# hila-chefer/Transformer-Explainability

Hardware: AMD Instinct MI355X
Metric: relevance maps/sec (ViT-B/16 224^2, batch 64 per GPU, generate_LRP transformer_attribution) (higher is better)
Workload: dtype f32 (3xbf16 split operands, 6 products, fp32 accumulate)

## Files before the change

include/te_relprop.h:

```cpp
#ifndef TE_RELPROP_H
#define TE_RELPROP_H

#include <stddef.h>
#include <stdint.h>

#ifdef __cplusplus
extern "C" {
#endif

typedef void* te_stream_t;
typedef uint16_t te_bf16_t;

enum {
  TE_OK = 0,
  TE_ERR_INVALID_ARG = -1,
  TE_ERR_WORKSPACE = -2,
  TE_ERR_UNSUPPORTED = -3,
  TE_ERR_NO_DEVICE = -4
};

enum { TE_VARIANT_OURS = 0, TE_VARIANT_LRP = 1, TE_IMPL_SIMPLE = 0x100 };

enum { TE_ROLLOUT_NORMALISE = 1, TE_ROLLOUT_CLS_FIXUP = 2, TE_ROLLOUT_ROW0 = 4 };

int te_version(void);
const char* te_status_string(int status);
int te_device_check(void);
const char* te_build_id(void);

size_t te_linear_relprop_workspace_bytes(int64_t T, int64_t in_f, int64_t out_f, int variant);
int te_linear_relprop_f32(const float* R, const float* X, const float* W, float* out,
                          int64_t T, int64_t in_f, int64_t out_f, float alpha, int variant,
                          void* ws, size_t ws_bytes, te_stream_t stream);

int te_linear_zpass_f32(const float* R, const float* X, const float* W, float* S,
                        int64_t T, int64_t in_f, int64_t out_f, te_stream_t stream);
int te_linear_cpass_f32(const float* S, const float* X, const float* W, float* out,
                        int64_t T, int64_t in_f, int64_t out_f, te_stream_t stream);

int te_linear_zpass_fwd_f32(const float* R, const float* r_scale, int64_t r_scale_stride,
                            int64_t rows_per_sample, const float* X, const float* W, const float* Y,
                            const float* bias, float* S, int64_t T, int64_t in_f, int64_t out_f,
                            te_stream_t stream);
int te_linear_relprop_fwd_f32(const float* R, const float* r_scale, int64_t r_scale_stride,
                              int64_t rows_per_sample, const float* X, const float* W, const float* Y,
                              const float* bias, float* out, int64_t T, int64_t in_f, int64_t out_f,
                              void* ws, size_t ws_bytes, te_stream_t stream);

size_t te_matmul_relprop_av_workspace_bytes(int64_t B, int64_t H, int64_t N, int64_t D);
int te_matmul_relprop_av_f32(const float* R, int64_t r_sb, int64_t r_sh, int64_t r_sn,
                             const float* attn,
                             const float* v, int64_t v_sb, int64_t v_sh, int64_t v_sn,
                             const float* Z, int64_t z_sb, int64_t z_sh, int64_t z_sn,
                             float* cam_attn,
                             float* cam_v, int64_t cv_sb, int64_t cv_sh, int64_t cv_sn,
                             int64_t B, int64_t H, int64_t N, int64_t D, float out_scale, int variant,
                             void* ws, size_t ws_bytes, te_stream_t stream);
size_t te_matmul_relprop_qk_workspace_bytes(int64_t B, int64_t H, int64_t N, int64_t D);
int te_matmul_relprop_qk_f32(const float* R_nn, const float* r_scale, int64_t r_scale_stride,
                             const float* q, int64_t q_sb, int64_t q_sh, int64_t q_sn,
                             const float* k, int64_t k_sb, int64_t k_sh, int64_t k_sn,
                             const float* Z,
                             float* cam_q, int64_t cq_sb, int64_t cq_sh, int64_t cq_sn,
                             float* cam_k, int64_t ck_sb, int64_t ck_sh, int64_t ck_sn,
                             int64_t B, int64_t H, int64_t N, int64_t D, float out_scale, int variant,
                             void* ws, size_t ws_bytes, te_stream_t stream);

size_t te_add_relprop_workspace_bytes(int64_t B, int64_t n);
int te_add_relprop_f32(const float* R, const float* X0, const float* X1, float* out0, float* out1,
                       int64_t B, int64_t n, int64_t x1_batch_stride, int variant,
                       void* ws, size_t ws_bytes, te_stream_t stream);

size_t te_add_relprop_deferred_workspace_bytes(int64_t B, int64_t n);
int te_add_relprop_deferred_f32(const float* R, const float* X0, const float* X1, float* a, float* b, float* fac,
                                int64_t B, int64_t n, int64_t x1_batch_stride,
                                void* ws, size_t ws_bytes, te_stream_t stream);

size_t te_add_bcast_relprop_workspace_bytes(int64_t B, int64_t H, int64_t N);
int te_add_bcast_relprop_f32(const float* R, const float* X0, const float* mask, float* out0,
                             float* out1, int64_t B, int64_t H, int64_t N, int variant,
                             void* ws, size_t ws_bytes, te_stream_t stream);

int te_add_bcast_relprop_deferred_f32(const float* R, const float* X0, const float* mask, float* a, float* out1,
                                      float* fac, int64_t B, int64_t H, int64_t N,
                                      void* ws, size_t ws_bytes, te_stream_t stream);

int te_clone_relprop_f32(const float* R0, const float* R1, const float* R2, const float* X,
                         float* out, int64_t n, te_stream_t stream);

int te_clone_relprop_scaled_f32(const float* R0, const float* s0, int64_t s0_stride,
                                const float* R1, const float* s1, int64_t s1_stride,
                                const float* R2, const float* s2, int64_t s2_stride,
                                const float* X, float* out, int64_t B, int64_t n, te_stream_t stream);

int te_index_select_relprop_f32(const float* R, const float* X, float* out,
                                int64_t B, int64_t N, int64_t C, int64_t index, te_stream_t stream);

int te_gradcam_headmean_f32(const float* grad, const float* cam, float* out,
                            int64_t B, int64_t H, int64_t N, te_stream_t stream);

size_t te_rollout_workspace_bytes(int64_t L, int64_t B, int64_t N);
size_t te_rollout_row0_workspace_bytes(int64_t B, int64_t N);
int te_rollout_f32(const float* cams, int64_t L, int64_t start_layer, int64_t B, int64_t N,
                   int flags, float* joint, void* ws, size_t ws_bytes, te_stream_t stream);

#define TE_X6_TILE_AUTO 0
#define TE_X6_TILE_128 1
#define TE_X6_TILE_256 2
#define TE_X6_TILE_128x128 3
#define TE_X6_TEST_DROP_HANDOVER 0x200
#define TE_X6_WHOLE_TILES 0x10000
#define TE_X6_TEST_SMALL_GRID 0x4000
#define TE_X6_X_PLANES_SIGNED 0x20000
#define TE_X6_TILE_Z_SHIFT 10
#define TE_X6_TILE_C_SHIFT 12
#define TE_X6_PHASE_SPLIT 4
#define TE_X6_PHASE_Z 8
#define TE_X6_PHASE_C 16
#define TE_X6_PHASE_MASK 28
int te_linear_relprop_x6_supported(int64_t T, int64_t in_f, int64_t out_f);
size_t te_linear_relprop_x6_workspace_bytes(int64_t T, int64_t in_f, int64_t out_f);
size_t te_linear_x6_weight_planes_bytes(int64_t in_f, int64_t out_f);
size_t te_linear_x6_planes_bytes(int64_t rows, int64_t K);
int te_linear_x6_prepare_weights_f32(const float* W, int64_t in_f, int64_t out_f, void* planes, size_t planes_bytes,
                                     te_stream_t stream);
int te_linear_x6_split_abs_f32(const float* X, int64_t rows, int64_t K, void* planes, size_t planes_bytes,
                               te_stream_t stream);
int te_linear_relprop_x6_f32(const float* R, const float* r_scale, int64_t r_scale_stride, int64_t rows_per_sample,
                             const float* X, const float* W, const void* w_planes, const void* x_planes,
                             const float* Y, const float* bias, float* out,
                             int64_t T, int64_t in_f, int64_t out_f, int flags, unsigned* status, void* ws,
                             size_t ws_bytes, te_stream_t stream);
int te_linear_relprop_x6_check(const void* ws, int64_t T, int64_t in_f, int64_t out_f, te_stream_t stream);

int te_linear_relprop_x6_general_supported(int64_t T, int64_t in_f, int64_t out_f, int variant);
size_t te_linear_x6_weight_planes_lrp_bytes(int64_t in_f, int64_t out_f);
int te_linear_x6_prepare_weights_lrp_f32(const float* W, int64_t in_f, int64_t out_f, void* planes, size_t planes_bytes,
                                         te_stream_t stream);
size_t te_linear_relprop_x6_general_workspace_bytes(int64_t T, int64_t in_f, int64_t out_f, int variant);
int te_linear_relprop_x6_general_f32(const float* R, const float* r_scale, int64_t r_scale_stride, int64_t rows_per_sample,
                                     const float* X, const float* W, const void* w_planes, const void* w_planes_lrp,
                                     const void* x_abs_planes, const float* Y, const float* bias, float* out,
                                     int64_t T, int64_t in_f, int64_t out_f, float alpha, int variant, int flags,
                                     unsigned* status, void* ws, size_t ws_bytes, te_stream_t stream);

int te_gemm_x6_supported(int64_t T, int64_t K, int64_t M);
size_t te_gemm_x6_workspace_bytes(int64_t T, int64_t K, int64_t M);
int te_linear_x6_split_matrix_f32(const float* A, int64_t rows, int64_t K, int transposed, void* planes,
                                  size_t planes_bytes, te_stream_t stream);
int te_gemm_x6_f32(const float* X, const void* x_planes, const void* w_planes, const float* bias, float* out,
                   int64_t T, int64_t K, int64_t M, int flags, unsigned* status, void* ws, size_t ws_bytes,
                   te_stream_t stream);
int te_linear_x6_split_dual_f32(const float* A, int64_t rows, int64_t K, void* planes, void* planes_abs,
                                size_t planes_bytes, te_stream_t stream);
int te_gelu_backward_x6_planes_f32(const float* dy, const float* x, int64_t rows, int64_t K, void* planes,
                                   size_t planes_bytes, te_stream_t stream);
int te_gelu_forward_x6_planes_f32(const float* x, float* y, int64_t rows, int64_t K, void* planes, void* planes_abs,
                                  size_t planes_bytes, te_stream_t stream);

int te_attention_forward_supported(int64_t N, int64_t D);
int te_attention_forward_f32(const float* qkv, float* z_qk, float* attn, float* out, void* out_planes,
                             void* out_abs_planes, size_t planes_bytes, int64_t B, int64_t H, int64_t N, int64_t D,
                             float scale, te_stream_t stream);
int te_attention_backward_f32(const float* d_out, const float* out, const float* qkv, const float* attn, float* d_attn,
                              float* d_qkv, int64_t B, int64_t H, int64_t N, int64_t D, float scale, int need_qk,
                              te_stream_t stream);

int te_attention_strided_supported(int64_t N, int64_t D);
size_t te_attention_backward_strided_workspace_bytes(int64_t B, int64_t H, int64_t N);
int te_attention_forward_strided_f32(const float* q, int64_t q_sb, int64_t q_sh, int64_t q_sn,
                                     const float* k, int64_t k_sb, int64_t k_sh, int64_t k_sn,
                                     const float* v, int64_t v_sb, int64_t v_sh, int64_t v_sn,
                                     const float* mask, float* z_qk, float* x_scaled, float* attn,
                                     float* out, int64_t o_sb, int64_t o_sh, int64_t o_sn,
                                     int64_t B, int64_t H, int64_t N, int64_t D, float scale, te_stream_t stream);
int te_attention_backward_strided_f32(const float* d_out, int64_t do_sb, int64_t do_sh, int64_t do_sn,
                                      const float* out, int64_t o_sb, int64_t o_sh, int64_t o_sn,
                                      const float* q, int64_t q_sb, int64_t q_sh, int64_t q_sn,
                                      const float* k, int64_t k_sb, int64_t k_sh, int64_t k_sn,
                                      const float* v, int64_t v_sb, int64_t v_sh, int64_t v_sn,
                                      const float* attn, float* d_attn,
                                      float* d_q, int64_t dq_sb, int64_t dq_sh, int64_t dq_sn,
                                      float* d_k, int64_t dk_sb, int64_t dk_sh, int64_t dk_sn,
                                      float* d_v, int64_t dv_sb, int64_t dv_sh, int64_t dv_sn,
                                      int64_t B, int64_t H, int64_t N, int64_t D, float scale, int need_qk,
                                      void* ws, size_t ws_bytes, te_stream_t stream);

int te_layernorm_supported(int64_t C);
int te_layernorm_forward_f32(const float* x, const float* weight, const float* bias, float* y, float* mean, float* rstd,
                             int64_t T, int64_t C, float eps, te_stream_t stream);
int te_layernorm_backward_f32(const float* dy, const float* x, const float* weight, const float* mean, const float* rstd,
                              const float* add, float* dx, int64_t T, int64_t C, te_stream_t stream);
int te_gelu_forward_f32(const float* x, float* y, int64_t n, te_stream_t stream);
int te_gelu_backward_f32(const float* dy, const float* x, float* dx, int64_t n, te_stream_t stream);

int te_heatmap_f32(const float* maps, float* heat, float* fg_mask, int64_t B, int64_t g, int64_t scale,
                   int normalise, te_stream_t stream);

size_t te_seg_metrics_workspace_bytes(int64_t B, int64_t H, int64_t W);
int te_seg_metrics_f32(const float* heat, const float* fg_mask, const int64_t* labels, int64_t* counts, double* ap,
                       double* f1, int64_t B, int64_t H, int64_t W, void* ws, size_t ws_bytes, te_stream_t stream);

#define TE_MAPSIM_SSIM 1
size_t te_map_similarity_workspace_bytes(int64_t B, int64_t n);
int te_map_similarity_f32(const float* a, const float* b, int64_t* rank_sums, double* sim, int64_t B, int64_t n, int64_t H,
                          int64_t W, int flags, double data_range, void* ws, size_t ws_bytes, te_stream_t stream);

#define TE_RATIONALE_MAX_KS 16
#define TE_RATIONALE_CLAMP 1
size_t te_rationale_metrics_workspace_bytes(int64_t B, int64_t N, int64_t Wmax);
int te_rationale_metrics_f32(const float* scores, const int32_t* word_ids, const uint8_t* truth, float* word_scores,
                             int32_t* n_words, int32_t* order, int32_t* counts, double* soft, int64_t B, int64_t N,
                             int64_t Wmax, const int64_t* ks, int64_t n_ks, int flags, void* ws, size_t ws_bytes,
                             te_stream_t stream);

#define TE_TOKEN_ERASE_MAX_FRACTIONS 8
int te_token_erase(const int64_t* input_ids, const int64_t* attention_mask, const int32_t* word_ids,
                   const int32_t* order, const int32_t* n_words, int64_t* ids_out, int64_t* mask_out,
                   int32_t* n_rationale, int64_t B, int64_t N, int64_t Wmax, const double* fractions, int64_t n_t,
                   int64_t pad_id, te_stream_t stream);

size_t te_conv2d_zb_relprop_workspace_bytes(int64_t B, int64_t C, int64_t H, int64_t W, int64_t E, int64_t p);
int te_conv2d_zb_relprop_f32(const float* R, int64_t r_bs, const float* X, const float* W, const float* Y,
                             const float* bias, float* out, int64_t B, int64_t C, int64_t H, int64_t W_, int64_t E,
                             int64_t p, int flags, void* ws, size_t ws_bytes, te_stream_t stream);

#define TE_PERTURB_MAX_STEPS 16
#define TE_PERTURB_MAX_CHANNELS 4
size_t te_perturb_workspace_bytes(int64_t B, int64_t n_steps);
int te_perturb_f32(const float* vis, const float* data, float* out, int64_t B, int64_t C, int64_t HW,
                   const int64_t* ks, int64_t n_steps, const float* mean, const float* std_, void* ws,
                   size_t ws_bytes, te_stream_t stream);

#define TE_BLUR_MAX_TAPS 63
int te_blur_normalised_f32(const float* data, float* out, int64_t B, int64_t C, int64_t H, int64_t W, const float* taps,
                           int64_t klen, const float* mean, const float* std_, te_stream_t stream);
size_t te_pixel_rank_workspace_bytes(int64_t B, int64_t n);
int te_pixel_rank_f32(const float* vis, int32_t* rank, int64_t B, int64_t n, void* ws, size_t ws_bytes, te_stream_t stream);
int te_curve_inputs_f32(const float* data, const float* substrate, const float* fill, const int32_t* rank, float* out,
                        int64_t B, int64_t C, int64_t HW, int64_t step, int64_t s0, int64_t n_s, int insertion,
                        const float* mean, const float* std_, te_stream_t stream);
int te_curve_inputs_bf16(const float* data, const float* substrate, const float* fill, const int32_t* rank, te_bf16_t* out,
                         int64_t B, int64_t C, int64_t HW, int64_t step, int64_t s0, int64_t n_s, int insertion,
                         const float* mean, const float* std_, te_stream_t stream);
int te_curve_scores_f32(const float* logits, const int64_t* target, double* prob, int64_t B, int64_t K, int64_t s0,
                        int64_t n_s, te_stream_t stream);
int te_curve_scores_bf16(const te_bf16_t* logits, const int64_t* target, double* prob, int64_t B, int64_t K, int64_t s0,
                         int64_t n_s, te_stream_t stream);
int te_curve_auc_f64(const double* prob, double* auc, int64_t S1, int64_t B, te_stream_t stream);

size_t te_localisation_workspace_bytes(int64_t P, int64_t H, int64_t W);
int te_localisation_f32(const float* heat, const int64_t* labels, const int64_t* image_index, const int64_t* target_id,
                        const int64_t* boxes, int64_t M, int64_t* stats, double* energy, int64_t P, int64_t B, int64_t H,
                        int64_t W, void* ws, size_t ws_bytes, te_stream_t stream);

int te_noise_inputs_f32(const float* x, float* out, int64_t B, int64_t n, int64_t d0, int64_t n_d, float radius, int64_t seed,
                        int64_t id0, te_stream_t stream);
int te_noise_inputs_bf16(const float* x, te_bf16_t* out, int64_t B, int64_t n, int64_t d0, int64_t n_d, float radius,
                         int64_t seed, int64_t id0, te_stream_t stream);
int te_map_distance_f32(const float* a, const float* b, double* sums, int64_t B, int64_t D, int64_t n, te_stream_t stream);
int te_map_distance_bf16(const float* a, const te_bf16_t* b, double* sums, int64_t B, int64_t D, int64_t n,
                         te_stream_t stream);
size_t te_map_complexity_workspace_bytes(int64_t B, int64_t n);
int te_map_complexity_f32(const float* maps, double* out, int64_t* counts, int64_t B, int64_t n, double eps, void* ws,
                          size_t ws_bytes, te_stream_t stream);

#define TE_SUBSET_MAX_CELLS 4096
int te_subset_inputs_f32(const float* x, const float* substrate, const float* fill, const float* attr, float* out,
                         uint8_t* member, double* attr_sum, int64_t B, int64_t C, int64_t g_h, int64_t g_w, int64_t p,
                         int64_t k, int64_t d0, int64_t n_d, int64_t seed, int64_t id0, te_stream_t stream);
int te_subset_inputs_bf16(const float* x, const float* substrate, const float* fill, const float* attr, te_bf16_t* out,
                          uint8_t* member, double* attr_sum, int64_t B, int64_t C, int64_t g_h, int64_t g_w, int64_t p,
                          int64_t k, int64_t d0, int64_t n_d, int64_t seed, int64_t id0, te_stream_t stream);
int te_perturbation_dot_f32(const float* x, const float* y, const float* w, double* sums, int64_t B, int64_t D, int64_t n,
                            int64_t m, te_stream_t stream);
int te_perturbation_dot_bf16(const float* x, const te_bf16_t* y, const float* w, double* sums, int64_t B, int64_t D, int64_t n,
                             int64_t m, te_stream_t stream);

int te_linear_relprop_bf16_supported(int64_t T, int64_t in_f, int64_t out_f);
size_t te_linear_relprop_bf16_workspace_bytes(int64_t T, int64_t in_f, int64_t out_f);
size_t te_linear_bf16_weight_planes_bytes(int64_t in_f, int64_t out_f);
int te_linear_bf16_prepare_weights(const te_bf16_t* W, int64_t in_f, int64_t out_f, void* planes, size_t planes_bytes,
                                   te_stream_t stream);
int te_linear_relprop_bf16(const float* R, int64_t r_ld, const float* r_scale, int64_t r_scale_stride,
                           int64_t rows_per_scale, const te_bf16_t* X, int64_t x_ld, const void* w_planes, float* out,
                           int64_t T, int64_t in_f, int64_t out_f, void* ws, size_t ws_bytes, te_stream_t stream);
int te_matmul_relprop_bf16_supported(int64_t N, int64_t D);
size_t te_matmul_relprop_av_bf16_workspace_bytes(int64_t B, int64_t H, int64_t N, int64_t D);
size_t te_matmul_relprop_qk_bf16_workspace_bytes(int64_t B, int64_t H, int64_t N, int64_t D);
int te_matmul_relprop_av_bf16(const float* R, int64_t r_sb, int64_t r_sh, int64_t r_sn,
                              const te_bf16_t* attn,
                              const te_bf16_t* v, int64_t v_sb, int64_t v_sh, int64_t v_sn,
                              const te_bf16_t* Z, int64_t z_sb, int64_t z_sh, int64_t z_sn,
                              float* cam_attn,
                              float* cam_v, int64_t cv_sb, int64_t cv_sh, int64_t cv_sn,
                              int64_t B, int64_t H, int64_t N, int64_t D, float out_scale, int variant,
                              void* ws, size_t ws_bytes, te_stream_t stream);
int te_matmul_relprop_qk_bf16(const float* R_nn, const float* r_scale, int64_t r_scale_stride,
                              const te_bf16_t* q, int64_t q_sb, int64_t q_sh, int64_t q_sn,
                              const te_bf16_t* k, int64_t k_sb, int64_t k_sh, int64_t k_sn,
                              const te_bf16_t* Z,
                              float* cam_q, int64_t cq_sb, int64_t cq_sh, int64_t cq_sn,
                              float* cam_k, int64_t ck_sb, int64_t ck_sh, int64_t ck_sn,
                              int64_t B, int64_t H, int64_t N, int64_t D, float out_scale, int variant,
                              void* ws, size_t ws_bytes, te_stream_t stream);
// ... 120 lines not shown
```

transformer-explainability_amd/bert.py:

```python
from __future__ import annotations

import math
from types import SimpleNamespace

import torch
import torch.nn as nn

from . import ops
from . import rules as R_ours

__all__ = ["BertConfigLite", "make_bert_module", "BertModel", "BertForSequenceClassification"]


def BertConfigLite(**kw):
    d = dict(vocab_size=30522, hidden_size=768, num_hidden_layers=12, num_attention_heads=12,
             intermediate_size=3072, hidden_act="gelu", hidden_dropout_prob=0.1,
             attention_probs_dropout_prob=0.1, max_position_embeddings=512, type_vocab_size=2,
             layer_norm_eps=1e-12, pad_token_id=0, num_labels=2)
    d.update(kw)
    return SimpleNamespace(**d)


class _FusedSelfAttention(torch.autograd.Function):

# ... 113 lines not shown
            if attention_mask is not None:
                scores = self.add([scores, attention_mask])
            probs = self.softmax(scores)
            self.save_attn(probs)
            if probs.requires_grad:
                probs.register_hook(self.save_attn_gradients)
            probs = self.dropout(probs)
            if head_mask is not None:
                probs = self.mul([probs, head_mask])
            ctx = self.matmul2([probs, v])
            ctx = ctx.permute(0, 2, 1, 3).contiguous()
            return (ctx.view(*ctx.shape[:-2], self.all_head_size),)

        def _forward_fused(self, h1, h2, h3, attention_mask):
            B, N, C = h1.shape
            H, D = self.num_attention_heads, self.attention_head_size
            ql, kl, vl = self.query(h1), self.key(h2), self.value(h3)
            ctx, probs, zqk, xsc = _FusedSelfAttention.apply(ql, kl, vl, attention_mask, H, 1.0 / math.sqrt(D), self)
            self._fused_anchor = ql if ql.requires_grad else None
            heads = lambda t: t.detach().view(B, N, H, D).permute(0, 2, 1, 3)
            q, k, v = heads(ql), heads(kl), heads(vl)
            self.save_attn(probs)
            caches = [(self.matmul1, [q, k.transpose(-1, -2)], zqk), (self.matmul2, [probs, v], heads(ctx))]
            if attention_mask is not None:
                caches.append((self.add, [xsc, attention_mask], None))
            for mod, X, Y in caches:
                mod.X, mod.Y = X, Y
                mod._y_version = Y._version if Y is not None else None
                mod._w_version = (None, None)
            return (ctx,)

        def relprop(self, cam, **kwargs):
            B, N, C = cam.shape
            H, D = self.num_attention_heads, self.attention_head_size
            var = self.matmul2.variant
            probs, v = self.matmul2.X
            q, kt = self.matmul1.X
            rq = torch.empty((B, N, C), dtype=cam.dtype, device=cam.device)
            rk, rv = torch.empty_like(rq), torch.empty_like(rq)
            as_heads = lambda t: t.view(B, N, H, D).permute(0, 2, 1, 3)
            if self.save_head_relevance:
                self.head_relevance = ops.head_relevance(as_heads(cam))
            cam1, _ = ops.matmul_relprop_av(as_heads(cam), probs, v, out_scale=0.5, cam_v_out=as_heads(rv), variant=var,
                                            z=R_ours._cached_y(self.matmul2))
            if self.head_mask is not None:
                cam1, _ = self.mul.relprop(cam1, **kwargs)
            self.save_attn_cam(cam1)
            if getattr(self, "_stop_after_attn_cam", False):
                raise L.StopRelprop()
            if self.attention_mask is not None:
                cam1, _ = self.add.relprop(cam1, deferred=True, **kwargs)
            ops.matmul_relprop_qk(cam1, q, kt.transpose(-1, -2), out_scale=0.5, cam_q_out=as_heads(rq),
                                  cam_k_out=as_heads(rk), variant=var, z=R_ours._cached_y(self.matmul1))
            rq = self.query.relprop(rq, **kwargs)
            rk = self.key.relprop(rk, **kwargs)
            rv = self.value.relprop(rv, **kwargs)
            return self.clone.relprop((rq, rk, rv), **kwargs)

        def attnlrp(self, G_o, eps):
            if self.head_mask is not None:
                raise ops._lib.TeError("BertSelfAttention.attnlrp: head_mask is not implemented for AttnLRP")
            q, k, v = self.query.Y.detach(), self.key.Y.detach(), self.value.Y.detach()
            d_q, d_k, d_v = torch.empty_like(q), torch.empty_like(k), torch.empty_like(v)
            R_ours.attention_attnlrp(G_o, q, k, v, self.get_attn().detach(), self.num_attention_heads,
                                     1.0 / math.sqrt(self.attention_head_size), d_q, d_k, d_v)
            ops.alrp_scale3(d_q, d_k, d_v)
            return self.clone.attnlrp((self.query.attnlrp(d_q, eps), self.key.attnlrp(d_k, eps),
                                       self.value.attnlrp(d_v, eps)), eps)

    class BertSelfOutput(nn.Module):
        def __init__(self, config):
            super().__init__()
            self.dense = L.Linear(config.hidden_size, config.hidden_size)
            self.LayerNorm = L.LayerNorm(config.hidden_size, eps=config.layer_norm_eps)
            self.dropout = L.Dropout(config.hidden_dropout_prob)
            self.add = L.Add()

        def forward(self, hidden_states, input_tensor):
            return self.LayerNorm(self.add([self.dropout(self.dense(hidden_states)), input_tensor]))

        def relprop(self, cam, **kwargs):
            cam1, cam2 = self.add.relprop(cam, deferred=True, **kwargs)
            return self.dense.relprop(cam1, **kwargs), cam2

        def attnlrp(self, G, eps):
            Gd = self.add.attnlrp(self.LayerNorm.attnlrp(G, eps), eps)
            return self.dense.attnlrp(Gd, eps), Gd

    class BertAttention(nn.Module):
        def __init__(self, config):
            super().__init__()
            self.self = BertSelfAttention(config)
            self.output = BertSelfOutput(config)
            self.clone = L.Clone()

        def forward(self, hidden_states, attention_mask=None, head_mask=None, **unused):
            h1, h2 = self.clone(hidden_states, 2)
            return (self.output(self.self(h1, attention_mask, head_mask)[0], h2),)

        def relprop(self, cam, **kwargs):
            cam1, cam2 = self.output.relprop(cam, **kwargs)
            cam1 = self.self.relprop(cam1, **kwargs)
            return self.clone.relprop((cam1, cam2), **kwargs)

        def attnlrp(self, G, eps):
            G1, G2 = self.output.attnlrp(G, eps)
            return self.clone.attnlrp((self.self.attnlrp(G1, eps), G2), eps)

    class BertIntermediate(nn.Module):
        def __init__(self, config):
            super().__init__()
            self.dense = L.Linear(config.hidden_size, config.intermediate_size)
            act = config.hidden_act
            self.intermediate_act_fn = ACT[act]() if isinstance(act, str) else act

        def forward(self, hidden_states):
            return self.intermediate_act_fn(self.dense(hidden_states))

        def relprop(self, cam, **kwargs):
            return self.dense.relprop(cam, **kwargs)

        def attnlrp(self, G, eps):
            return self.dense.attnlrp(self.intermediate_act_fn.attnlrp(G, eps), eps)

    class BertOutput(nn.Module):
        def __init__(self, config):
            super().__init__()
            self.dense = L.Linear(config.intermediate_size, config.hidden_size)
            self.LayerNorm = L.LayerNorm(config.hidden_size, eps=config.layer_norm_eps)
            self.dropout = L.Dropout(config.hidden_dropout_prob)
            self.add = L.Add()

        def forward(self, hidden_states, input_tensor):
            return self.LayerNorm(self.add([self.dropout(self.dense(hidden_states)), input_tensor]))

        def relprop(self, cam, **kwargs):
            cam1, cam2 = self.add.relprop(cam, deferred=True, **kwargs)
            return self.dense.relprop(cam1, **kwargs), cam2

        def attnlrp(self, G, eps):
            Gd = self.add.attnlrp(self.LayerNorm.attnlrp(G, eps), eps)
            return self.dense.attnlrp(Gd, eps), Gd

    class BertLayer(nn.Module):
        def __init__(self, config):
            super().__init__()
            self.attention = BertAttention(config)
            self.intermediate = BertIntermediate(config)
            self.output = BertOutput(config)
            self.clone = L.Clone()
            act = self.intermediate.intermediate_act_fn
            if hasattr(act, "feeds"):
                act.feeds(self.output.dense)

        def forward(self, hidden_states, attention_mask=None, head_mask=None, **unused):
            att = self.attention(hidden_states, attention_mask, head_mask)[0]
            a1, a2 = self.clone(att, 2)
            return (self.output(self.intermediate(a1), a2),)

        def relprop(self, cam, **kwargs):
            cam1, cam2 = self.output.relprop(cam, **kwargs)
            cam1 = self.intermediate.relprop(cam1, **kwargs)
            cam = self.clone.relprop((cam1, cam2), **kwargs)
            return self.attention.relprop(cam, **kwargs)

        def attnlrp(self, G, eps):
            G1, G2 = self.output.attnlrp(G, eps)
            G = self.clone.attnlrp((self.intermediate.attnlrp(G1, eps), G2), eps)
            return self.attention.attnlrp(G, eps)

        def relprop_cls_only(self, cam_cls, **kwargs):
            alpha = kwargs.get("alpha", 1)
            var = self.clone.variant
            cls = lambda t: t[:, :1]
            dfr = ops.USE_DEFERRED_ADD
            c1, c2 = ops.add_relprop(cam_cls, cls(self.output.add.X[0]), cls(self.output.add.X[1]), variant=var,
                                     deferred=dfr)
            c1 = R_ours.linear_rule(self.output.dense, c1, alpha, cls, var)
            c1 = R_ours.linear_rule(self.intermediate.dense, c1, alpha, cls, var)
            cam = ops.clone_relprop((c1, c2), cls(self.clone.X))
            att = self.attention
            a1, a2 = ops.add_relprop(cam, cls(att.output.add.X[0]), cls(att.output.add.X[1]), variant=var, deferred=dfr)
            a1 = R_ours.linear_rule(att.output.dense, a1, alpha, cls, var)
            B, N, C = att.clone.X.shape
            dense = torch.zeros((2, B, N, C), dtype=a1.dtype, device=a1.device)
            dense[0, :, 0] = a1[:, 0]
            if isinstance(a2, ops.Deferred):
                a2 = a2.materialise()
            dense[1, :, 0] = a2[:, 0]
            cam1 = att.self.relprop(dense[0], **kwargs)
            return att.clone.relprop((cam1, dense[1]), **kwargs)

    class BertEncoder(nn.Module):
        def __init__(self, config):
            super().__init__()
            self.config = config
            self.layer = nn.ModuleList([BertLayer(config) for _ in range(config.num_hidden_layers)])

        def forward(self, hidden_states, attention_mask=None, head_mask=None, **unused):
            for i, layer in enumerate(self.layer):
                hidden_states = layer(hidden_states, attention_mask, None if head_mask is None else head_mask[i])[0]
            return (hidden_states,)

        def relprop(self, cam, **kwargs):
            for layer in reversed(self.layer):
                cam = layer.relprop(cam, **kwargs)
            return cam

        def attnlrp(self, G, eps):
            for layer in reversed(self.layer):
                G = layer.attnlrp(G, eps)
            return G

    class BertPooler(nn.Module):
        def __init__(self, config):
            super().__init__()
            self.dense = L.Linear(config.hidden_size, config.hidden_size)
            self.activation = L.Tanh()
            self.pool = L.IndexSelect()
            self.register_buffer("_cls_index", torch.zeros((), dtype=torch.long), persistent=False)

        def forward(self, hidden_states):
            first = self.pool(hidden_states, 1, self._cls_index).squeeze(1)
            return self.activation(self.dense(first))

        def relprop(self, cam, **kwargs):
            cam = self.dense.relprop(cam, **kwargs)
            return self.pool.relprop(cam.unsqueeze(1), **kwargs)

        def attnlrp(self, G, eps):
            G = self.dense.attnlrp(self.activation.attnlrp(G, eps), eps)
            return self.pool.attnlrp(G, eps)

    class BertModel(nn.Module):
        def __init__(self, config):
            super().__init__()
            self.config = config
            self.embeddings = BertEmbeddings(config)
            self.encoder = BertEncoder(config)
            self.pooler = BertPooler(config)

        def get_input_embeddings(self):
            return self.embeddings.word_embeddings

        def get_head_mask(self, head_mask, num_hidden_layers, is_attention_chunked=False, batch_size=None):
            par = next(self.parameters())
            return R_ours.expand_head_mask(head_mask, num_hidden_layers, self.config.num_attention_heads, par.dtype,
                                           batch_size, par.device)

        def forward(self, input_ids=None, attention_mask=None, token_type_ids=None, position_ids=None,
                    head_mask=None, inputs_embeds=None, **unused):
            shape = input_ids.size() if input_ids is not None else inputs_embeds.size()[:-1]
            device = input_ids.device if input_ids is not None else inputs_embeds.device
            head_mask = self.get_head_mask(head_mask, self.config.num_hidden_layers, batch_size=shape[0])
            if attention_mask is None:
                attention_mask = torch.ones(shape, device=device)
            ext = (1.0 - attention_mask[:, None, None, :].to(next(self.parameters()).dtype)) * -10000.0
            with (ops.stock_forward() if torch.is_tensor(head_mask) else ops._NULL):
                emb = self.embeddings(input_ids=input_ids, position_ids=position_ids, token_type_ids=token_type_ids,
                                      inputs_embeds=inputs_embeds)
                seq = self.encoder(emb, attention_mask=ext, head_mask=head_mask)[0]
                return (seq, self.pooler(seq))

        exploit_cls_sparsity = True

        def relprop(self, cam, **kwargs):
            if not self.exploit_cls_sparsity:
                return self.encoder.relprop(self.pooler.relprop(cam, **kwargs), **kwargs)
            cam = self.pooler.dense.relprop(cam, **kwargs)
            cam = ops.index_select_relprop(cam.unsqueeze(1), self.pooler.pool.X[:, :1], 0)
            layers = list(self.encoder.layer)
            cam = layers[-1].relprop_cls_only(cam, **kwargs)
            for layer in reversed(layers[:-1]):
                cam = layer.relprop(cam, **kwargs)
            return cam

        def attnlrp(self, G, eps):
            G = self.encoder.attnlrp(self.pooler.attnlrp(G, eps), eps)
            norm = self.embeddings.LayerNorm
            return ops.alrp_token_relevance(norm.X, norm.attnlrp(G, eps), skip_first=False)

    class BertForSequenceClassification(nn.Module):
        def __init__(self, config):
            super().__init__()
            self.config = config
            self.num_labels = config.num_labels
            self.bert = BertModel(config)
            self.dropout = L.Dropout(config.hidden_dropout_prob)
            self.classifier = L.Linear(config.hidden_size, config.num_labels)
            self.apply(self._init_weights)

        def _init_weights(self, m):
            if isinstance(m, (nn.Linear, nn.Embedding)):
                m.weight.data.normal_(mean=0.0, std=getattr(self.config, "initializer_range", 0.02))
            elif isinstance(m, nn.LayerNorm):
                m.bias.data.zero_()
                m.weight.data.fill_(1.0)
            if isinstance(m, nn.Linear) and m.bias is not None:
                m.bias.data.zero_()

        def forward(self, input_ids=None, attention_mask=None, token_type_ids=None, position_ids=None,
                    head_mask=None, inputs_embeds=None, labels=None, **unused):
            pooled = self.bert(input_ids, attention_mask=attention_mask, token_type_ids=token_type_ids,
                               position_ids=position_ids, head_mask=head_mask, inputs_embeds=inputs_embeds)[1]
            logits = self.classifier(self.dropout(pooled))
            if labels is not None:
# ... 24 lines not shown
```

transformer-explainability_amd/csrc/te_api.hip:

```cpp
#include "te_common.h"

#include <string.h>

extern "C" int te_version(void) { return 800;  }

#ifndef TE_BUILD_ID
#define TE_BUILD_ID "unstamped"
#endif
extern "C" const char* te_build_id(void) { return TE_BUILD_ID; }

extern "C" const char* te_status_string(int status) {
  switch (status) {
    case TE_OK: return "ok";
    case TE_ERR_INVALID_ARG: return "invalid argument";
    case TE_ERR_WORKSPACE: return "workspace missing, misaligned or too small";
    case TE_ERR_UNSUPPORTED: return "shape not supported by the gfx950 kernels";
    case TE_ERR_NO_DEVICE: return "no gfx950 device visible";
    default: break;
  }
  if (status > 0) return hipGetErrorString((hipError_t)status);
  return "unknown status";
}

extern "C" int te_device_check(void) {
  int n = 0;
  if (hipGetDeviceCount(&n) != hipSuccess || n <= 0) return TE_ERR_NO_DEVICE;
  for (int d = 0; d < n; ++d) {
    hipDeviceProp_t p;
    if (hipGetDeviceProperties(&p, d) != hipSuccess) continue;
    if (strncmp(p.gcnArchName, "gfx950", 6) == 0) return TE_OK;
  }
  return TE_ERR_NO_DEVICE;
}
```

transformer-explainability_amd/csrc/te_linear_x6.hip:

```cpp
#include <algorithm>
#include <cmath>
#include <type_traits>

#include "te_x6.h"

namespace {

constexpr int kRB = 3 * kFrag;
constexpr int kMinFrag = 4;
constexpr int kSpinMillis = 250;
constexpr int kErrWord = 1023;


enum { MODE_Z = 0, MODE_C = 1, MODE_G = 2, MODE_ZI = 3, MODE_Z1 = 4, MODE_CI = 5, MODE_X = 6, MODE_ZS = 7 };

__device__ __forceinline__ float bf16_f32(unsigned b) { return __uint_as_float(b << 16); }

enum { OP_ABS = 0, OP_POS = 1, OP_NEG = 2, OP_ID = 3 };
template <int OP>
__device__ __forceinline__ float apply_op(float x) {
  if constexpr (OP == OP_ID) return x;
  if constexpr (OP == OP_ABS) return __int_as_float(__float_as_int(x) & 0x7fffffff);
  const int b = __float_as_int(x);
  if constexpr (OP == OP_POS) return __int_as_float(b > 0 ? b : 0);
  return __int_as_float(b < 0 ? b : 0);
}

template <int OP, bool TRANSPOSE>
__global__ __launch_bounds__(256) void split_kernel(const float* __restrict__ src, unsigned char* __restrict__ dst,
                                                    int64_t R, int64_t K, int group, int sign,
                                                    unsigned char* __restrict__ dst_abs = nullptr) {
  const int r = threadIdx.x & 31, sl = threadIdx.x >> 5;
  const int64_t rb = blockIdx.x;
  const int64_t ks = (int64_t)blockIdx.y * 8 + sl;
  const int64_t nks = K >> 4;
  if (ks >= nks) return;
  const int64_t row = rb * 32 + r;
  float v[16];
  if (row < R) {
    if constexpr (!TRANSPOSE) {
      const float* s = src + row * K + ks * 16;
#pragma unroll
      for (int c = 0; c < 4; ++c) {
        const f32x4 q = *reinterpret_cast<const f32x4*>(s + 4 * c);
#pragma unroll
        for (int e = 0; e < 4; ++e) v[4 * c + e] = q[e];
      }
    } else {
#pragma unroll
      for (int e = 0; e < 16; ++e) v[e] = src[(ks * 16 + e) * R + row];
    }
  } else {
#pragma unroll
    for (int e = 0; e < 16; ++e) v[e] = 0.0f;
  }
  unsigned p[8][3];
#pragma unroll
  for (int e = 0; e < 8; ++e) split3_pk(apply_op<OP>(v[2 * e]), apply_op<OP>(v[2 * e + 1]), p[e]);
  unsigned char* d = dst + ((rb * nks + ks) * group + sign * 3) * kFrag + r * 16;
#pragma unroll
  for (int q = 0; q < 3; ++q)
#pragma unroll
    for (int kh = 0; kh < 2; ++kh) {
      u32x4 w;
#pragma unroll
      for (int e = 0; e < 4; ++e) w[e] = p[4 * kh + e][q];
      *reinterpret_cast<u32x4*>(d + q * kFrag + kh * 512) = w;
    }
  if constexpr (OP == OP_ID) {
    if (dst_abs) {
#pragma unroll
      for (int e = 0; e < 8; ++e) {
        const unsigned m = p[e][0] & 0x80008000u;
        p[e][0] &= 0x7fff7fffu;
        p[e][1] ^= m & (((p[e][1] & 0x7fff7fffu) + 0x7fff7fffu) & 0x80008000u);
        p[e][2] ^= m & (((p[e][2] & 0x7fff7fffu) + 0x7fff7fffu) & 0x80008000u);
      }
      unsigned char* da = dst_abs + ((rb * nks + ks) * 3) * kFrag + r * 16;
#pragma unroll
      for (int q = 0; q < 3; ++q)
#pragma unroll
        for (int kh = 0; kh < 2; ++kh) {
          u32x4 w;
#pragma unroll
          for (int e = 0; e < 4; ++e) w[e] = p[4 * kh + e][q];
          *reinterpret_cast<u32x4*>(da + q * kFrag + kh * 512) = w;
        }
    }
  }
}

enum { SRC_GELU_BWD = 0, SRC_GELU_FWD = 1 };
constexpr int kGsPitch = 132;
template <int SRC>
__global__ __launch_bounds__(256) void gelu_split_lds_kernel(const float* __restrict__ g, const float* __restrict__ x,
                                                             float* __restrict__ y, unsigned char* __restrict__ dst,
                                                             unsigned char* __restrict__ dst_abs, int64_t R, int64_t K) {
  __shared__ __attribute__((aligned(16))) float tile[32 * kGsPitch];
  const int64_t rb = blockIdx.x;
  const int64_t k0 = (int64_t)blockIdx.y * 128;
#pragma unroll
  for (int j = 0; j < 4; ++j) {
    const int i = threadIdx.x + 256 * j;
    const int tr = i >> 5, c4 = i & 31;
    const int64_t row = rb * 32 + tr, col = k0 + 4 * c4;
    f32x4 o = {0.0f, 0.0f, 0.0f, 0.0f};
    if (row < R && col < K) {
      const int64_t at = row * K + col;
      const f32x4 xv = __builtin_nontemporal_load(reinterpret_cast<const f32x4*>(x + at));
      if constexpr (SRC == SRC_GELU_BWD) {
        const f32x4 gv = __builtin_nontemporal_load(reinterpret_cast<const f32x4*>(g + at));
#pragma unroll
        for (int e = 0; e < 4; ++e) o[e] = te_gelu_grad(gv[e], xv[e]);
      } else {
#pragma unroll
        for (int e = 0; e < 4; ++e) o[e] = te_gelu(xv[e]);
        *reinterpret_cast<f32x4*>(y + at) = o;
      }
    }
    *reinterpret_cast<f32x4*>(&tile[tr * kGsPitch + 4 * c4]) = o;
  }
  __syncthreads();
  const int r = threadIdx.x & 31, sl = threadIdx.x >> 5;
  const int64_t ks = (int64_t)blockIdx.y * 8 + sl;
  const int64_t nks = K >> 4;
  if (ks >= nks) return;
  float v[16];
#pragma unroll
  for (int c = 0; c < 4; ++c) {
    const f32x4 q = *reinterpret_cast<const f32x4*>(&tile[r * kGsPitch + sl * 16 + 4 * c]);
#pragma unroll
    for (int e = 0; e < 4; ++e) v[4 * c + e] = q[e];
  }
  unsigned p[8][3];
#pragma unroll
  for (int e = 0; e < 8; ++e) split3_pk(v[2 * e], v[2 * e + 1], p[e]);
  auto store = [&](unsigned char* d) __attribute__((always_inline)) {
#pragma unroll
    for (int q = 0; q < 3; ++q)
#pragma unroll
      for (int kh = 0; kh < 2; ++kh) {
        u32x4 w;
#pragma unroll
        for (int e = 0; e < 4; ++e) w[e] = p[4 * kh + e][q];
        *reinterpret_cast<u32x4*>(d + q * kFrag + kh * 512) = w;
      }
  };
  store(dst + ((rb * nks + ks) * 3) * kFrag + r * 16);
  if (SRC == SRC_GELU_FWD && dst_abs) {
#pragma unroll
    for (int e = 0; e < 8; ++e) {
      const unsigned m = p[e][0] & 0x80008000u;
      p[e][0] &= 0x7fff7fffu;
      p[e][1] ^= m & (((p[e][1] & 0x7fff7fffu) + 0x7fff7fffu) & 0x80008000u);
      p[e][2] ^= m & (((p[e][2] & 0x7fff7fffu) + 0x7fff7fffu) & 0x80008000u);
    }
    store(dst_abs + ((rb * nks + ks) * 3) * kFrag + r * 16);
  }
}

__global__ __launch_bounds__(256) void zero_words_kernel(u32x4* __restrict__ p) {
  p[(size_t)blockIdx.x * 256 + threadIdx.x] = u32x4{0u, 0u, 0u, 0u};
}

__device__ __forceinline__ float exact_z(const float* __restrict__ x, const float* __restrict__ w, int64_t K) {
  float z1 = 0.0f, z2 = 0.0f;
  for (int64_t k = 0; k < K; ++k) {
    const float xv = x[k], wv = w[k];
    z1 = fmaf(fmaxf(xv, 0.0f), fmaxf(wv, 0.0f), z1);
    z2 = fmaf(fminf(xv, 0.0f), fminf(wv, 0.0f), z2);
  }
  return z1 + z2;
}

__device__ __forceinline__ float exact_zi(const float* __restrict__ x, const float* __restrict__ w, int64_t K) {
  float z1 = 0.0f, z2 = 0.0f;
  for (int64_t k = 0; k < K; ++k) {
    const float xv = x[k], wv = w[k];
    z1 = fmaf(fmaxf(xv, 0.0f), fminf(wv, 0.0f), z1);
    z2 = fmaf(fminf(xv, 0.0f), fmaxf(wv, 0.0f), z2);
  }
  return z1 + z2;
}

struct X6Params {
  const unsigned char* A;
  const unsigned char* B;
  int64_t a_group_stride;
  int64_t b_rb_stride;
  int nks;
  unsigned char pad0_[20];
  int ntm, ntn;
  int rows_w;
  int t_fast;
  int whole_tiles;
  int pad1_;
  int ncb;
  int64_t T;
  int in_f, out_f;
  float* partial;
  unsigned* flags;
  unsigned* status;
  long long spin_ticks;
  int drop_handover;
  int small_grid;
  int prefer_whole;
  const float* R;
  const float* Y;
  const float* bias;
  const float* X;
  const float* W;
  unsigned char* S;
  const float* rs;
  int64_t rs_stride;
  int rps;
  float* out;
  float scale;
  int accum;
  int x_sign;
};

#if defined(__HIP_DEVICE_COMPILE__)
#define X6_PASS4(a, b, c, d) asm volatile("" : "+v"(a), "+v"(b), "+v"(c), "+v"(d))
#else
#define X6_PASS4(a, b, c, d) (void)0
#endif

__device__ __forceinline__ void glds16(const unsigned char* src, unsigned char* lds_wave_base) {
  __builtin_amdgcn_global_load_lds((const __attribute__((address_space(1))) void*)src,
                                   (__attribute__((address_space(3))) void*)lds_wave_base, 16, 0, 0);
}

constexpr int kStages = 2;
template <int WM>
struct X6Geo {
  static constexpr int NWM = (WM == 1) ? 1 : 2, NWN = (WM == 0) ? 2 : 4, MI = (WM == 0) ? 2 : 4;
  static constexpr int NW = NWM * NWN, THREADS = 64 * NW, WPS = (WM == 0) ? 3 : 2;
  static constexpr int TM = NWM * MI * 32, TT = NWN * 64;
  static constexpr int NPA = 3 * NWM * MI, NPB = 3 * NWN * 2;
  static constexpr int ACC = MI * 2 * 16;
  static constexpr int MAX_SPX = (WM == 2) ? 32 : (WM == 1) ? 64 : 96;
};

template <int WM, int MODE>
struct X6Lds {
  using GEO = X6Geo<WM>;
  static constexpr bool STAGED = (MODE == MODE_Z || MODE == MODE_ZS || MODE == MODE_ZI || MODE == MODE_Z1) && GEO::MI == 4;
  static constexpr int STAGES = kStages * (GEO::NPA + GEO::NPB) * kFrag;
  static constexpr int MAIN = (STAGED && GEO::NW * 16384 > STAGES) ? GEO::NW * 16384 : STAGES;
  static constexpr int TOTAL = MAIN + GEO::NW * 512 + 16;
};

template <int WM, int MODE>
__global__ __launch_bounds__(X6Geo<WM>::THREADS, X6Geo<WM>::WPS) void x6_kernel(const X6Params p) {
  using GEO = X6Geo<WM>;
  constexpr int NW = GEO::NW, NWM = GEO::NWM, NWN = GEO::NWN, MI = GEO::MI;
  constexpr bool SGN = MODE == MODE_ZS;
  constexpr bool Z_ABS = MODE == MODE_Z || SGN;
  constexpr bool IS_Z = (Z_ABS || MODE == MODE_ZI || MODE == MODE_Z1);
  constexpr bool IS_C = (MODE == MODE_C || MODE == MODE_CI);
  constexpr int G = IS_C ? 6 : 3;
  constexpr int NPA = GEO::NPA, NPB = GEO::NPB;
  constexpr int NP = NPA + NPB;
  static_assert(NPA / 3 == NW, "each wave stages one weight-side block");
  constexpr int PBW = NPB / 3 / NW;
  constexpr int STAGE = NP * kFrag;
  constexpr int GROUPS = NPA / G;
  constexpr int LDS_MAIN = X6Lds<WM, MODE>::MAIN;
  extern __shared__ __attribute__((aligned(16))) unsigned char smem[];

  const int lane = threadIdx.x & 63;
  const int wave = __builtin_amdgcn_readfirstlane(threadIdx.x >> 6);
  const int wm = wave / NWN, wn = wave % NWN;
  const int lane16 = lane * 16;

  const int bid = blockIdx.x, spx = gridDim.x >> 3;
  const int xcd = bid & 7, slot = bid >> 3;
  const int nks = p.nks;
  const int tiles = p.ntm * p.ntn;
  const int tx0 = (int)((int64_t)tiles * xcd / 8), tx1 = (int)((int64_t)tiles * (xcd + 1) / 8);
  const int ntx = tx1 - tx0;
  const int64_t iters = (int64_t)ntx * nks;
  auto cut = [&](int s) -> int64_t {
    int64_t b = iters * s / spx;
    const int r = (int)(b % nks);
    if (p.whole_tiles) return (2 * r < nks) ? b - r : b + (nks - r);
    if (r < kMinFrag) b -= r;
    else if (nks - r < kMinFrag) b += nks - r;
    return b;
  };
  const int64_t ib = cut(slot), ie = cut(slot + 1);
  if (ib >= ie) return;
  const int f_tile = (int)(ib / nks), kb = (int)(ib - (int64_t)f_tile * nks);
  const int l_tile = (int)((ie - 1) / nks), ke = (int)(ie - (int64_t)l_tile * nks);
  const bool tail = kb > 0;
  const bool head = (ke < nks) && !(f_tile == l_tile && tail);
  const int full0 = tail ? f_tile + 1 : f_tile, full1 = (ke < nks) ? l_tile - 1 : l_tile;
  const int nseq = (head ? 1 : 0) + (full1 >= full0 ? full1 - full0 + 1 : 0) + (tail ? 1 : 0);

  float* my_part = p.partial + (size_t)bid * GEO::THREADS * GEO::ACC;
  const float* in_part = p.partial + (size_t)(bid - 8) * GEO::THREADS * GEO::ACC;

  for (int seq = 0; seq < nseq; ++seq) {
    int tile, k0, k1;
    if (head && seq == 0) {
      tile = l_tile, k0 = 0, k1 = ke;
    } else if (tail && seq == nseq - 1) {
      tile = f_tile, k0 = kb, k1 = (f_tile == l_tile) ? ke : nks;
    } else {
      tile = full0 + seq - (head ? 1 : 0), k0 = 0, k1 = nks;
    }
    tile += tx0;
    int tn, tm;
    if (p.t_fast) {
      tm = tile / p.ntn, tn = tile - tm * p.ntn;
    } else {
      tn = tile / p.ntm, tm = tile - tn * p.ntm;
    }

    const unsigned char* srcA;
    if constexpr (!IS_C)
      srcA = p.A + (int64_t)(tm * GROUPS + wave) * p.a_group_stride + (int64_t)k0 * kRB;
    else
      srcA = p.A + (int64_t)(tm * GROUPS + (wave >> 1)) * p.a_group_stride + (int64_t)k0 * (2 * kRB) + (wave & 1) * kRB;
    const unsigned char* srcB[PBW];
#pragma unroll
    for (int u = 0; u < PBW; ++u) {
      const int cb = min(tn * (GEO::TT / 32) + wave * PBW + u, p.ncb - 1);
      srcB[u] = p.B + (int64_t)cb * p.b_rb_stride + (int64_t)k0 * kRB;
    }
    unsigned char* const ldsA = smem + wave * kRB;
    unsigned char* const ldsB = smem + NPA * kFrag + wave * (PBW * kRB);
    u32x4 breg[SGN ? PBW : 1][3];
    auto stage_in = [&](int stg, int adv) __attribute__((always_inline)) {
      srcA += adv * (G * kFrag);
#pragma unroll
      for (int u = 0; u < PBW; ++u) srcB[u] += adv * kRB;
#pragma unroll
      for (int q = 0; q < 3; ++q) glds16(srcA + q * kFrag + lane16, ldsA + stg * STAGE + q * kFrag);
#pragma unroll
      for (int u = 0; u < PBW; ++u)
#pragma unroll
        for (int q = 0; q < 3; ++q) {
          if constexpr (SGN) breg[u][q] = *reinterpret_cast<const u32x4*>(srcB[u] + q * kFrag + lane16);
          else glds16(srcB[u] + q * kFrag + lane16, ldsB + stg * STAGE + (u * 3 + q) * kFrag);
        }
    };
    auto sign_and_store = [&](int stg) __attribute__((always_inline)) {
#pragma unroll
      for (int u = 0; u < (SGN ? PBW : 0); ++u) {
#pragma unroll
        for (int e = 0; e < 4; ++e) {
          const unsigned m = breg[u][0][e] & 0x80008000u;
          breg[u][0][e] &= 0x7fff7fffu;
          breg[u][1][e] ^= m;
          breg[u][2][e] ^= m;
        }
#pragma unroll
        for (int q = 0; q < 3; ++q) *reinterpret_cast<u32x4*>(ldsB + stg * STAGE + (u * 3 + q) * kFrag + lane16) = breg[u][q];
      }
    };

    auto wait_for = [&](unsigned* flag) -> bool {
      unsigned* const ok_word = reinterpret_cast<unsigned*>(smem + LDS_MAIN + NW * 512);
      if (threadIdx.x == 0) {
        unsigned spins = 0, ok = 1u;
        const long long t_begin = wall_clock64();
        while (__hip_atomic_load(flag, __ATOMIC_RELAXED, __HIP_MEMORY_SCOPE_AGENT) == 0u) {
          __builtin_amdgcn_s_sleep(8);
          if ((++spins & 63u) == 0u &&
              (__hip_atomic_load(p.status, __ATOMIC_RELAXED, __HIP_MEMORY_SCOPE_AGENT) != 0u ||
               wall_clock64() - t_begin > p.spin_ticks)) {
            ok = 0u;
            break;
          }
        }
        if (!ok) {
          __hip_atomic_fetch_or(p.status, 1u, __ATOMIC_RELAXED, __HIP_MEMORY_SCOPE_AGENT);
          __hip_atomic_store(p.flags + kErrWord, 1u, __ATOMIC_RELAXED, __HIP_MEMORY_SCOPE_AGENT);
        }
        __builtin_amdgcn_fence(__ATOMIC_ACQUIRE, "agent");
        __hip_atomic_store(flag, 0u, __ATOMIC_RELAXED, __HIP_MEMORY_SCOPE_AGENT);
        *ok_word = ok;
// ... 62 lines not shown
        X6_WAIT(5); X6_MM(1, 0, 1);
        X6_WAIT(4); X6_MM(1, 1, 1); X6_MM(0, 1, 1);
        X6_WAIT(2); X6_MM(0, 0, 2);
        X6_WAIT(1); X6_MM(1, 0, 2);
        X6_WAIT(0); X6_MM(1, 1, 2); X6_MM(0, 1, 2);
        X6_SB;
#pragma unroll
        for (int q6 = 3; q6 < 6; ++q6) {
          X6_MM(0, 0, q6); X6_MM(1, 0, q6); X6_MM(1, 1, q6); X6_MM(0, 1, q6);
          X6_SB;
        }
#undef X6_RD4
      } else {
      X6_RD_HEAD(0);
      X6_RD_TAIL(0);
      stage_in((st + 1) % kStages, (ks + 1 < k1) ? 1 : 0);
      X6_WAIT(4); X6_MM(0, 0, 0);
      X6_WAIT(3); X6_MM(1, 0, 0);
      X6_WAIT(2); X6_MM(1, 1, 0); X6_MM(0, 1, 0);
      X6_RD_HEAD(1);
      X6_WAIT(4); X6_MM(2, 1, 0); X6_MM(2, 0, 0);
      X6_WAIT(3); X6_MM(3, 0, 0); X6_MM(3, 1, 0);
      X6_RD_TAIL(1);
      X6_WAIT(4); X6_MM(0, 0, 1);
      X6_WAIT(3); X6_MM(1, 0, 1);
      X6_WAIT(2); X6_MM(1, 1, 1); X6_MM(0, 1, 1);
      X6_RD_HEAD(2);
      X6_WAIT(4); X6_MM(2, 1, 1); X6_MM(2, 0, 1);
      X6_WAIT(3); X6_MM(3, 0, 1); X6_MM(3, 1, 1);
      X6_RD_TAIL(2);
      X6_WAIT(4); X6_MM(0, 0, 2);
      X6_WAIT(3); X6_MM(1, 0, 2);
      X6_WAIT(2); X6_MM(1, 1, 2); X6_MM(0, 1, 2);
      X6_WAIT(1); X6_MM(2, 1, 2); X6_MM(2, 0, 2);
      X6_WAIT(0); X6_MM(3, 0, 2); X6_MM(3, 1, 2);
      X6_SB;
#pragma unroll
      for (int q6 = 3; q6 < 6; ++q6) {
        X6_MM(0, 0, q6); X6_MM(1, 0, q6); X6_MM(1, 1, q6); X6_MM(0, 1, q6);
        X6_MM(2, 1, q6); X6_MM(2, 0, q6); X6_MM(3, 0, q6); X6_MM(3, 1, q6);
        X6_SB;
      }
      }
#undef X6_SB
#undef X6_RDB
#undef X6_RDA
#undef X6_WAIT
#undef X6_MM
#undef X6_RD_HEAD
#undef X6_RD_TAIL
      if constexpr (SGN) sign_and_store((st + 1) % kStages);
      st = (st + 1 == kStages) ? 0 : st + 1;
    }
    if constexpr (SGN) asm volatile("s_waitcnt lgkmcnt(0)" ::: "memory");

    auto publish = [&](float* dst, unsigned* flag) __attribute__((always_inline)) {
      f32x4* op = reinterpret_cast<f32x4*>(dst) + (size_t)wave * (GEO::ACC / 4) * 64 + lane;
#pragma unroll
      for (int mi = 0; mi < MI; ++mi)
#pragma unroll
        for (int ni = 0; ni < 2; ++ni) {
#pragma unroll
          for (int c = 0; c < 4; ++c) {
            f32x4 v;
#pragma unroll
            for (int e = 0; e < 4; ++e) v[e] = acc[mi][ni][4 * c + e];
            op[c * 64] = v;
          }
          op += 4 * 64;
          asm volatile("" : "+v"(op));
        }
      asm volatile("s_waitcnt vmcnt(0)" ::: "memory");
      __syncthreads();
      if (threadIdx.x == 0) {
        __builtin_amdgcn_fence(__ATOMIC_RELEASE, "agent");
        asm volatile("s_waitcnt vmcnt(0)" ::: "memory");
        if (!p.drop_handover) __hip_atomic_store(flag, 1u, __ATOMIC_RELAXED, __HIP_MEMORY_SCOPE_AGENT);
      }
    };
    if (k1 < nks) {
      publish(my_part, p.flags + bid);
      continue;
    }
    const int tc = lane & 31, h = lane >> 5;
    if constexpr (IS_Z) {
      const int nksS = p.out_f >> 4;
      int64_t tl[2];
      bool live[2], blk[2];
      float f[2];
#pragma unroll
      for (int ni = 0; ni < 2; ++ni) {
        const int cb = tn * (GEO::TT / 32) + wn * 2 + ni;
        const int64_t t = (int64_t)cb * 32 + tc;
        blk[ni] = cb < p.ncb;
        live[ni] = t < p.T;
        tl[ni] = live[ni] ? t : p.T - 1;
        f[ni] = p.rs ? p.rs[(tl[ni] / p.rps) * p.rs_stride] : 1.0f;
      }
      float* const bias_lds = reinterpret_cast<float*>(smem + LDS_MAIN) + wave * 128;
      if (lane < MI * 8) {
        f32x4 bv = {0.0f, 0.0f, 0.0f, 0.0f};
        if (p.bias) bv = *reinterpret_cast<const f32x4*>(p.bias + (tm * (NWM * MI) + wm * MI) * 32 + lane * 4);
        *reinterpret_cast<f32x4*>(bias_lds + lane * 4) = bv;
      }
      if constexpr (X6Lds<WM, MODE>::STAGED) {
        constexpr int NL = (MODE == MODE_Z1) ? 4 : 8;
        __builtin_amdgcn_s_barrier();
        unsigned char* const stg = smem + wave * 16384;
        unsigned rda[4];
#pragma unroll
        for (int g = 0; g < 4; ++g)
          rda[g] = (unsigned)(uintptr_t)stg + tc * 128 + (((2 * g + h) ^ ((tc >> 1) & 7)) << 4);
        const unsigned bia = (unsigned)(uintptr_t)bias_lds + h * 16;
        const int r8 = lane >> 3;
        auto request = [&](int bi, int buf) __attribute__((always_inline)) {
          const int ni = bi / MI, mi = bi % MI;
          const int cb = tn * (GEO::TT / 32) + wn * 2 + ni;
          const int j0 = (tm * (NWM * MI) + wm * MI + mi) * 32;
#pragma unroll
          for (int i = 0; i < 4; ++i) {
            const int row = 8 * i + r8;
            const int64_t t = min((int64_t)cb * 32 + row, p.T - 1);
            const int64_t off = t * p.out_f + j0 + (((lane & 7) ^ ((row >> 1) & 7)) << 2);
            glds16(reinterpret_cast<const unsigned char*>(p.R + off), stg + buf * 8192 + i * 1024);
            if constexpr (MODE != MODE_Z1)
              glds16(reinterpret_cast<const unsigned char*>(p.Y + off), stg + buf * 8192 + 4096 + i * 1024);
          }
        };
        const bool all_blk = blk[0] && blk[1];
        request(0, 0);
        request(1, 1);
#pragma unroll
        for (int bi = 0; bi < 2 * MI; ++bi) {
          const int ni = bi / MI, mi = bi % MI, buf = bi & 1;
          const int cb = tn * (GEO::TT / 32) + wn * 2 + ni;
          const int j0 = (tm * (NWM * MI) + wm * MI + mi) * 32;
          constexpr int kStore = 6;
          const int yl = (bi + 1 < 2 * MI) ? NL : 0, ys = (bi >= 2 ? kStore : 0) + (bi >= 1 ? kStore : 0);
          if (all_blk) asm volatile("s_waitcnt vmcnt(%0)" ::"n"(yl + ys) : "memory");
          else asm volatile("s_waitcnt vmcnt(%0)" ::"n"(yl) : "memory");
          f32x4 r4[4], y4[4], b4[4];
#pragma unroll
          for (int g = 0; g < 4; ++g) {
            asm volatile("ds_read_b128 %0, %1 offset:%2" : "=v"(r4[g]) : "v"(rda[g]), "i"(buf * 8192));
            if constexpr (MODE != MODE_Z1)
              asm volatile("ds_read_b128 %0, %1 offset:%2" : "=v"(y4[g]) : "v"(rda[g]), "i"(buf * 8192 + 4096));
            asm volatile("ds_read_b128 %0, %1 offset:%2" : "=v"(b4[g]) : "v"(bia), "i"((mi * 32 + 8 * g) * 4));
          }
          asm volatile("s_waitcnt lgkmcnt(0)" ::: "memory");
          if (bi + 2 < 2 * MI) request(bi + 2, buf);
          X6_PASS4(r4[0], r4[1], r4[2], r4[3]);
          if constexpr (MODE != MODE_Z1) X6_PASS4(y4[0], y4[1], y4[2], y4[3]);
          X6_PASS4(b4[0], b4[1], b4[2], b4[3]);
          unsigned w[4][3][2];
          unsigned long long any_cancel = 0;
          auto z_of = [&](int g, int c0, f32x2& z2, f32x2& a2) __attribute__((always_inline)) {
            a2 = f32x2{acc[mi][ni][4 * g + c0], acc[mi][ni][4 * g + c0 + 1]};
            if constexpr (Z_ABS)
              z2 = f32x2{0.5f, 0.5f} * ((f32x2{y4[g][c0], y4[g][c0 + 1]} - f32x2{b4[g][c0], b4[g][c0 + 1]}) + a2);
            else if constexpr (MODE == MODE_ZI)
              z2 = f32x2{0.5f, 0.5f} * ((f32x2{y4[g][c0], y4[g][c0 + 1]} - f32x2{b4[g][c0], b4[g][c0 + 1]}) - a2);
            else
              z2 = a2;
          };
          auto cancels = [&](float z, float a_abs, float b) __attribute__((always_inline)) -> bool {
            if constexpr (Z_ABS) return te_z_cancels(z, a_abs, b);
            else if constexpr (MODE == MODE_ZI) return te_z_cancels(-z, a_abs, b);
            else return false;
          };
#pragma unroll
          for (int g = 0; g < 4; ++g) {
            float sv4[4];
#pragma unroll
            for (int c0 = 0; c0 < 4; c0 += 2) {
              f32x2 z2, a2;
              z_of(g, c0, z2, a2);
              f32x2 rr = {r4[g][c0], r4[g][c0 + 1]};
              if (p.rs) rr = rr * f32x2{f[ni], f[ni]};
              const f32x2 sv = sd2(rr, z2);
#pragma unroll
              for (int e = 0; e < 2; ++e) {
                const bool cancel = cancels(z2[e], a2[e], b4[g][c0 + e]);
                if constexpr (MODE != MODE_Z1) any_cancel |= __builtin_amdgcn_ballot_w64(cancel);
                sv4[c0 + e] = (live[ni] && !cancel) ? sv[e] : 0.0f;
              }
            }
            unsigned lo[3], hi[3];
            split3_pk(sv4[0], sv4[1], lo);
            split3_pk(sv4[2], sv4[3], hi);
#pragma unroll
            for (int q = 0; q < 3; ++q) {
              w[g][q][0] = lo[q];
              w[g][q][1] = hi[q];
            }
          }
          unsigned bad = 0;
          if (any_cancel != 0) {
#pragma unroll
            for (int g = 0; g < 4; ++g)
#pragma unroll
              for (int c0 = 0; c0 < 4; c0 += 2) {
                f32x2 z2, a2;
                z_of(g, c0, z2, a2);
                bad |= (cancels(z2[0], a2[0], b4[g][c0]) ? 1u : 0u) << (4 * g + c0);
                bad |= (cancels(z2[1], a2[1], b4[g][c0 + 1]) ? 1u : 0u) << (4 * g + c0 + 1);
              }
          }
#pragma unroll
          for (int g = 0; g < 2; ++g)
#pragma unroll
            for (int q = 0; q < 3; ++q)
#pragma unroll
              for (int d = 0; d < 2; ++d) swap_halves(w[g][q][d], w[g + 2][q][d]);
          if (blk[ni]) {
            unsigned char* Srow = p.S + (int64_t)cb * nksS * kRB + tc * 16;
            unsigned char* sp = Srow + (int64_t)((j0 >> 4) + h) * kRB;
#pragma unroll
            for (int q = 0; q < 3; ++q)
#pragma unroll
              for (int c = 0; c < 2; ++c) {
                u32x4 v = {w[c][q][0], w[c][q][1], w[c + 2][q][0], w[c + 2][q][1]};
                *reinterpret_cast<u32x4*>(sp + q * kFrag + c * 512) = v;
              }
            if (!live[ni]) bad = 0;
            if (__builtin_amdgcn_ballot_w64(bad != 0) != 0) {
              asm volatile("s_waitcnt vmcnt(0)" ::: "memory");
              const float* Rrow = p.R + tl[ni] * p.out_f;
#pragma clang loop unroll(disable)
              for (int e = 0; e < 16; ++e) {
                if ((bad >> e) & 1u) {
                  const int jj = j0 + 8 * (e >> 2) + 4 * h + (e & 3);
                  const float z = (MODE == MODE_ZI) ? exact_zi(p.X + tl[ni] * p.in_f, p.W + (int64_t)jj * p.in_f, p.in_f)
                                                    : exact_z(p.X + tl[ni] * p.in_f, p.W + (int64_t)jj * p.in_f, p.in_f);
                  float rr = Rrow[jj];
                  if (p.rs) rr = rr * f[ni];
                  unsigned pl[3];
                  split3(te_sd(rr, z), pl);
                  unsigned short* d = reinterpret_cast<unsigned short*>(Srow + (int64_t)(jj >> 4) * kRB + ((jj >> 3) & 1) * 512) + (jj & 7);
                  d[0] = (unsigned short)pl[0];
                  d[kFrag / 2] = (unsigned short)pl[1];
                  d[kFrag] = (unsigned short)pl[2];
                }
              }
            }
          }
        }
      } else {
      constexpr int NBUF = (MI == 4) ? 2 : 1;
      f32x4 r4[NBUF][4], y4[NBUF][4];
      auto load_block = [&](int bi, int buf) __attribute__((always_inline)) {
        const int ni = bi / MI, mi = bi % MI;
        const int j0 = (tm * (NWM * MI) + wm * MI + mi) * 32;
        const float* Rrow = p.R + tl[ni] * p.out_f + j0 + 4 * h;
#pragma unroll
        for (int g = 0; g < 4; ++g) r4[buf][g] = *reinterpret_cast<const f32x4*>(Rrow + 8 * g);
        if constexpr (MODE != MODE_Z1) {
          const float* Yrow = p.Y + tl[ni] * p.out_f + j0 + 4 * h;
#pragma unroll
          for (int g = 0; g < 4; ++g) y4[buf][g] = *reinterpret_cast<const f32x4*>(Yrow + 8 * g);
        }
      };
      if constexpr (NBUF == 2) load_block(0, 0);
#pragma unroll
      for (int bi = 0; bi < 2 * MI; ++bi) {
        const int ni = bi / MI, mi = bi % MI, buf = bi % NBUF;
        const int cb = tn * (GEO::TT / 32) + wn * 2 + ni;
        const int j0 = (tm * (NWM * MI) + wm * MI + mi) * 32;
        if constexpr (NBUF == 2) {
          if (bi + 1 < 2 * MI) load_block(bi + 1, buf ^ 1);
        } else {
          load_block(bi, 0);
        }
        unsigned w[4][3][2];
        unsigned bad = 0;
#pragma unroll
        for (int g = 0; g < 4; ++g) {
          const f32x4 b4 = *reinterpret_cast<const f32x4*>(bias_lds + mi * 32 + 8 * g + 4 * h);
          float sv4[4];
#pragma unroll
          for (int c = 0; c < 4; ++c) {
            const float a_abs = acc[mi][ni][4 * g + c];
            float z;
            bool cancel;
            if constexpr (Z_ABS) {
              z = 0.5f * ((y4[buf][g][c] - b4[c]) + a_abs);
              cancel = te_z_cancels(z, a_abs, b4[c]);
            } else if constexpr (MODE == MODE_ZI) {
              z = 0.5f * ((y4[buf][g][c] - b4[c]) - a_abs);
              cancel = te_z_cancels(-z, a_abs, b4[c]);
            } else {
              z = a_abs;
              cancel = false;
            }
            bad |= (cancel ? 1u : 0u) << (4 * g + c);
            float rr = r4[buf][g][c];
            if (p.rs) rr = rr * f[ni];
            float sv = te_sd(rr, z);
            asm volatile("" : "+v"(sv));
            sv4[c] = (live[ni] && !cancel) ? sv : 0.0f;
          }
          unsigned lo[3], hi[3];
          split3_pk(sv4[0], sv4[1], lo);
          split3_pk(sv4[2], sv4[3], hi);
#pragma unroll
          for (int q = 0; q < 3; ++q) {
            w[g][q][0] = lo[q];
            w[g][q][1] = hi[q];
          }
        }
#pragma unroll
        for (int g = 0; g < 2; ++g)
#pragma unroll
          for (int q = 0; q < 3; ++q)
#pragma unroll
            for (int d = 0; d < 2; ++d) swap_halves(w[g][q][d], w[g + 2][q][d]);
        if (blk[ni]) {
          unsigned char* Srow = p.S + (int64_t)cb * nksS * kRB + tc * 16;
          unsigned char* sp = Srow + (int64_t)((j0 >> 4) + h) * kRB;
#pragma unroll
          for (int q = 0; q < 3; ++q)
#pragma unroll
            for (int c = 0; c < 2; ++c) {
              u32x4 v = {w[c][q][0], w[c][q][1], w[c + 2][q][0], w[c + 2][q][1]};
              *reinterpret_cast<u32x4*>(sp + q * kFrag + c * 512) = v;
            }
          if (!live[ni]) bad = 0;
          if (__builtin_amdgcn_ballot_w64(bad != 0) != 0) {
            asm volatile("s_waitcnt vmcnt(0)" ::: "memory");
            const float* Rrow = p.R + tl[ni] * p.out_f;
#pragma clang loop unroll(disable)
            for (int e = 0; e < 16; ++e) {
              if ((bad >> e) & 1u) {
                const int jj = j0 + 8 * (e >> 2) + 4 * h + (e & 3);
                const float z = (MODE == MODE_ZI) ? exact_zi(p.X + tl[ni] * p.in_f, p.W + (int64_t)jj * p.in_f, p.in_f)
                                                  : exact_z(p.X + tl[ni] * p.in_f, p.W + (int64_t)jj * p.in_f, p.in_f);
                float rr = Rrow[jj];
                if (p.rs) rr = rr * f[ni];
                unsigned pl[3];
                split3(te_sd(rr, z), pl);
                unsigned short* d = reinterpret_cast<unsigned short*>(Srow + (int64_t)(jj >> 4) * kRB + ((jj >> 3) & 1) * 512) + (jj & 7);
                d[0] = (unsigned short)pl[0];
                d[kFrag / 2] = (unsigned short)pl[1];
                d[kFrag] = (unsigned short)pl[2];
              }
            }
          }
        }
      }
      }
    } else if constexpr (MODE == MODE_G) {
      float* const bias_lds = reinterpret_cast<float*>(smem + LDS_MAIN) + wave * 128;
      if (lane < MI * 8) {
        f32x4 bv = {0.0f, 0.0f, 0.0f, 0.0f};
        if (p.bias) bv = *reinterpret_cast<const f32x4*>(p.bias + (tm * (NWM * MI) + wm * MI) * 32 + lane * 4);
        *reinterpret_cast<f32x4*>(bias_lds + lane * 4) = bv;
      }
#pragma unroll
      for (int ni = 0; ni < 2; ++ni) {
        const int64_t t = ((int64_t)tn * (GEO::TT / 32) + wn * 2 + ni) * 32 + tc;
        float* orow = p.out + (t < p.T ? t : 0) * p.out_f + (tm * (NWM * MI) + wm * MI) * 32 + 4 * h;
#pragma unroll
        for (int mi = 0; mi < MI; ++mi)
#pragma unroll
          for (int g = 0; g < 4; ++g) {
            const f32x4 b4 = *reinterpret_cast<const f32x4*>(bias_lds + mi * 32 + 8 * g + 4 * h);
            f32x4 o;
#pragma unroll
            for (int c = 0; c < 4; ++c) o[c] = acc[mi][ni][4 * g + c] + b4[c];
            if (t < p.T) *reinterpret_cast<f32x4*>(orow + mi * 32 + 8 * g) = o;
          }
      }
    } else if constexpr (MODE == MODE_X) {
#pragma unroll
      for (int ni = 0; ni < 2; ++ni) {
        const int64_t t = ((int64_t)tn * (GEO::TT / 32) + wn * 2 + ni) * 32 + tc;
        const int64_t off = (t < p.T ? t : 0) * p.out_f + (tm * (NWM * MI) + wm * MI) * 32 + 4 * h;
#pragma unroll
        for (int mi = 0; mi < MI; ++mi) {
          f32x4 xv[4], pv[4];
#pragma unroll
          for (int g = 0; g < 4; ++g) {
            xv[g] = *reinterpret_cast<const f32x4*>(p.X + off + mi * 32 + 8 * g);
            pv[g] = p.accum ? *reinterpret_cast<const f32x4*>(p.out + off + mi * 32 + 8 * g) : f32x4{0.0f, 0.0f, 0.0f, 0.0f};
          }
#pragma unroll
          for (int g = 0; g < 4; ++g) {
            f32x4 o;
#pragma unroll
            for (int c = 0; c < 4; ++c) {
              const float xm = (p.x_sign > 0) ? fmaxf(xv[g][c], 0.0f) : fminf(xv[g][c], 0.0f);
              const float v = p.scale * (xm * acc[mi][ni][4 * g + c]);
              o[c] = p.accum ? pv[g][c] + v : v;
            }
            if (t < p.T) *reinterpret_cast<f32x4*>(p.out + off + mi * 32 + 8 * g) = o;
          }
        }
      }
    } else {
      f32x4 x4[2][MI / 2][4];
      int64_t tt[2];
      bool live[2];
#pragma unroll
      for (int ni = 0; ni < 2; ++ni) {
        const int64_t t = ((int64_t)tn * (GEO::TT / 32) + wn * 2 + ni) * 32 + tc;
        live[ni] = t < p.T;
        tt[ni] = live[ni] ? t : p.T - 1;
#pragma unroll
        for (int il = 0; il < MI / 2; ++il) {
          const float* xr = p.X + tt[ni] * p.in_f + (tm * (NWM * MI / 2) + wm * (MI / 2) + il) * 32 + 4 * h;
#pragma unroll
          for (int g = 0; g < 4; ++g) x4[ni][il][g] = *reinterpret_cast<const f32x4*>(xr + 8 * g);
        }
      }
#pragma unroll
      for (int ni = 0; ni < 2; ++ni)
#pragma unroll
        for (int il = 0; il < MI / 2; ++il) {
          float* orow = p.out + tt[ni] * p.in_f + (tm * (NWM * MI / 2) + wm * (MI / 2) + il) * 32 + 4 * h;
#pragma unroll
          for (int g = 0; g < 4; ++g) {
            f32x4 o;
#pragma unroll
            for (int c = 0; c < 4; ++c) {
              const float xv = x4[ni][il][g][c];
              const float xp = fmaxf(xv, 0.0f), xn = fminf(xv, 0.0f);
              if constexpr (MODE == MODE_C)
                o[c] = p.scale * (xp * acc[2 * il][ni][4 * g + c] + xn * acc[2 * il + 1][ni][4 * g + c]);
              else
                o[c] = p.scale * (xp * acc[2 * il + 1][ni][4 * g + c] + xn * acc[2 * il][ni][4 * g + c]);
            }
            if constexpr (MODE == MODE_CI) {
              const f32x4 prev = *reinterpret_cast<const f32x4*>(orow + 8 * g);
#pragma unroll
              for (int c = 0; c < 4; ++c) o[c] = prev[c] + o[c];
            }
            if (live[ni]) *reinterpret_cast<f32x4*>(orow + 8 * g) = o;
          }
        }
    }
    __syncthreads();
  }
}

static_assert(sizeof(X6Params) == 248, "X6Params is the kernel-argument block of x6_kernel");
static_assert(offsetof(X6Params, ntm) == 56 && offsetof(X6Params, ncb) == 80 && offsetof(X6Params, T) == 88 &&
              offsetof(X6Params, partial) == 104 && offsetof(X6Params, R) == 152 && offsetof(X6Params, out) == 224,
              "a field of X6Params moved in the kernel arguments");

inline size_t planes_bytes(int64_t rows, int64_t K) {
  return (size_t)te_ceil_div(rows, 32) * 32 * (size_t)K * 6;
}
inline bool bad_k(int64_t K) { return K < 16 || K % 16; }
constexpr size_t kPartialBytes = (size_t)512 * 256 * 128 * 4;
constexpr double kWholeTileSlack = 1.15;
constexpr size_t kFlagBytes = 65536;
constexpr int kFlagWords = kFlagBytes / 4;
constexpr int kUsedFlagWords = kErrWord + 1;
constexpr int kRulePasses = 2;
constexpr int kGeneralPasses = 8;

struct X6Workspace {
  size_t x_stride, s, s_stride, partial, flags, total;
  unsigned char* x(void* ws, int set) const { return (unsigned char*)ws + set * x_stride; }
  unsigned char* sp(void* ws, int set) const { return (unsigned char*)ws + s + set * s_stride; }
  float* acc(void* ws) const { return (float*)((unsigned char*)ws + partial); }
  unsigned* flag_region(const void* ws, int pass) const { return (unsigned*)((unsigned char*)ws + flags) + (size_t)pass * kFlagWords; }
};
inline X6Workspace x6_workspace(int64_t T, int64_t K, int64_t M, int xsets, int ssets, int passes) {
  X6Workspace l;
  l.x_stride = te_align_up(planes_bytes(T, K), 256);
  l.s_stride = te_align_up(planes_bytes(T, M), 256);
  l.s = xsets * l.x_stride;
  l.partial = l.s + ssets * l.s_stride;
  l.flags = l.partial + kPartialBytes;
  l.total = l.flags + passes * kFlagBytes;
  return l;
}
inline X6Workspace gemm_workspace(int64_t T, int64_t K, int64_t M) { return x6_workspace(T, K, M, 1, 0, 1); }
inline X6Workspace rule_workspace(int64_t T, int64_t in_f, int64_t out_f) { return x6_workspace(T, in_f, out_f, 1, 1, kRulePasses); }
inline X6Workspace general_workspace(int64_t T, int64_t in_f, int64_t out_f) { return x6_workspace(T, in_f, out_f, 2, 2, kGeneralPasses); }

struct X6WeightPlanes { size_t c, total; };
inline X6WeightPlanes weight_planes(int64_t in_f, int64_t out_f) {
  const size_t c = te_align_up(planes_bytes(out_f, in_f), 256);
  return {c, c + te_align_up(2 * planes_bytes(in_f, out_f), 256)};
}
struct X6WeightPlanesLrp { size_t wn, wpT, wnT, total; };
inline X6WeightPlanesLrp weight_planes_lrp(int64_t in_f, int64_t out_f) {
  const size_t za = te_align_up(planes_bytes(out_f, in_f), 256), ca = te_align_up(planes_bytes(in_f, out_f), 256);
  return {za, 2 * za, 2 * za + ca, 2 * za + 2 * ca};
}

constexpr int kTileMask = TE_X6_TILE_128 | TE_X6_TILE_256 | TE_X6_TILE_128x128;
constexpr int kProductFlags = kTileMask | TE_X6_WHOLE_TILES | TE_X6_TEST_DROP_HANDOVER | TE_X6_TEST_SMALL_GRID;
constexpr int kRuleFlags = kProductFlags | TE_X6_PHASE_MASK | TE_X6_X_PLANES_SIGNED | (kTileMask << TE_X6_TILE_Z_SHIFT) | (kTileMask << TE_X6_TILE_C_SHIFT);

inline int pick_wm(int64_t in_f, int64_t out_f) {
  if (out_f % 256 == 0 && in_f % 128 == 0) return 2;
  if (out_f % 128 == 0 && in_f % 64 == 0) return 1;
  return 0;
}

inline long long spin_ticks_for_current_device() {
  static long long cached[64] = {};
  int dev = 0;
  if (hipGetDevice(&dev) != hipSuccess || dev < 0 || dev >= 64) dev = 0;
  if (cached[dev] == 0) {
    int khz = 0;
    if (hipDeviceGetAttribute(&khz, hipDeviceAttributeWallClockRate, dev) != hipSuccess || khz <= 0) khz = 100000;
    cached[dev] = (long long)khz * kSpinMillis;
  }
  return cached[dev];
}

template <int WM, int MODE>
int launch_x6(const X6Params& p, hipStream_t stream) {
  using GEO = X6Geo<WM>;
  constexpr int lds = X6Lds<WM, MODE>::TOTAL;
  static_assert(lds * (WM == 0 ? 3 : WM == 1 ? 2 : 1) <= 160 * 1024, "LDS of the workgroups of one CU");
  static_assert((size_t)8 * GEO::MAX_SPX * GEO::THREADS * GEO::ACC * 4 <= kPartialBytes && 8 * GEO::MAX_SPX < kErrWord, "workspace");
  auto kern = x6_kernel<WM, MODE>;
  hipError_t e = hipFuncSetAttribute(reinterpret_cast<const void*>(kern), hipFuncAttributeMaxDynamicSharedMemorySize, lds);
  if (e != hipSuccess) return (int)e;
  X6Params q = p;
  q.ntm = p.rows_w / GEO::TM;
  q.ntn = (int)te_ceil_div(p.T, GEO::TT);
  const int64_t tiles = (int64_t)q.ntm * q.ntn;
  const int max_spx = p.small_grid ? 2 : GEO::MAX_SPX;
  const int spx = (int)std::min<int64_t>(max_spx, std::max<int64_t>(1, te_ceil_div(tiles, 8)));
  const double r = (double)tiles / (8.0 * spx);
  q.whole_tiles = ((p.prefer_whole || std::ceil(r) <= kWholeTileSlack * r) && !p.small_grid) ? 1 : 0;
  if (!q.status) q.status = q.flags + kErrWord;
  q.spin_ticks = spin_ticks_for_current_device();
  kern<<<dim3(8 * spx), dim3(GEO::THREADS), lds, stream>>>(q);
  return TE_OK;
}

template <int MODE>
int launch_x6_mode(int wm, const X6Params& p, hipStream_t stream) {
  if (wm == 2) return launch_x6<2, MODE>(p, stream);
  if (wm == 1) return launch_x6<1, MODE>(p, stream);
  return launch_x6<0, MODE>(p, stream);
}

inline int choose_geo(int wm_max, int64_t T, int64_t rows_w, int pin, int min_tiles_256 = 256, bool small_ok = false) {
  if (pin == TE_X6_TILE_128) return 1;
  if (pin == TE_X6_TILE_256) return wm_max;
  if (pin == TE_X6_TILE_128x128) return 0;
  const int64_t t256 = te_ceil_div(T, 256);
  if (wm_max == 2 && t256 * (rows_w / 256) >= min_tiles_256) return 2;
  if (small_ok && t256 * (rows_w / 128) < 448) return 0;
  return 1;
}

inline X6Params call_params(int64_t T, float* partial, const float* bias, float* out, unsigned* status, int flags) {
  X6Params p{};
  p.T = T;
  p.ncb = (int)te_ceil_div(T, 32);
  p.partial = partial;
  p.bias = bias;
  p.out = out;
  p.status = status;
  p.drop_handover = (flags & TE_X6_TEST_DROP_HANDOVER) ? 1 : 0;
  p.small_grid = (flags & TE_X6_TEST_SMALL_GRID) ? 1 : 0;
  p.prefer_whole = (flags & TE_X6_WHOLE_TILES) ? 1 : 0;
  return p;
}
inline X6Params rule_params(X6Params p, const float* R, const float* r_scale, int64_t r_scale_stride, int64_t rows_per_sample,
                            const float* X, const float* W, const float* Y) {
  p.R = R;
  p.Y = Y;
  p.X = X;
  p.W = W;
  p.rs = r_scale;
  p.rs_stride = r_scale_stride;
  p.rps = (int)(r_scale ? rows_per_sample : 1);
  return p;
}
inline bool bad_r_scale(const float* r_scale, int64_t rows_per_sample, int64_t T) {
  return r_scale && (rows_per_sample <= 0 || rows_per_sample > 0x7fffffff || T % rows_per_sample);
}

template <int MODE>
int launch_pass(X6Params p, int wm, const unsigned char* A, const unsigned char* B, unsigned char* S, int64_t in_f,
                int64_t out_f, unsigned* flag_region, hipStream_t stream, float scale = 0.0f, int accum = 0, int x_sign = 0) {
  constexpr bool c_like = MODE == MODE_C || MODE == MODE_CI;
  constexpr bool over_out = c_like || MODE == MODE_X;
  p.A = A, p.B = B, p.S = S;
  p.nks = (int)((over_out ? out_f : in_f) / 16);
  p.a_group_stride = (int64_t)p.nks * (c_like ? 2 : 1) * kRB;
  p.b_rb_stride = (int64_t)p.nks * kRB;
  p.rows_w = (int)(c_like ? 2 * in_f : MODE == MODE_X ? in_f : out_f);
  p.in_f = (int)(MODE == MODE_X ? out_f : in_f);
  p.out_f = (int)(MODE == MODE_X ? in_f : out_f);
  p.scale = scale, p.accum = accum, p.x_sign = x_sign;
  p.flags = flag_region;
  return launch_x6_mode<MODE>(wm, p, stream);
}

inline void zero_flag_regions(unsigned* flag_words, int passes, hipStream_t stream) {
  zero_words_kernel<<<dim3(passes * kFlagBytes / 16 / 256), dim3(256), 0, stream>>>(reinterpret_cast<u32x4*>(flag_words));
}

inline int check_producer(bool have_all, bool f32_aligned, bool planes_aligned, int64_t rows, int64_t K, size_t planes_bytes_) {
  if (!have_all || rows < 1) return TE_ERR_INVALID_ARG;
  if (bad_k(K) || !f32_aligned || rows > ((int64_t)1 << 26)) return TE_ERR_UNSUPPORTED;
  if (planes_bytes_ < planes_bytes(rows, K) || !planes_aligned) return TE_ERR_WORKSPACE;
  return TE_OK;
}
inline dim3 producer_grid(int64_t rows, int64_t K) { return dim3((unsigned)te_ceil_div(rows, 32), (unsigned)te_ceil_div(K / 16, 8)); }

}

extern "C" int te_linear_relprop_x6_supported(int64_t T, int64_t in_f, int64_t out_f) {
  return (T >= 1 && in_f >= 128 && out_f >= 128 && pick_wm(in_f, out_f) != 0 && in_f <= (1 << 20) && out_f <= (1 << 20) &&
          T <= (int64_t)1 << 26) ? 1 : 0;
}

extern "C" size_t te_linear_x6_weight_planes_bytes(int64_t in_f, int64_t out_f) {
  return te_linear_relprop_x6_supported(1, in_f, out_f) ? weight_planes(in_f, out_f).total : 0;
}

extern "C" int te_linear_x6_prepare_weights_f32(const float* W, int64_t in_f, int64_t out_f, void* planes,
                                                size_t planes_bytes_, te_stream_t stream_) {
  if (!W || !planes) return TE_ERR_INVALID_ARG;
  if (!te_linear_relprop_x6_supported(1, in_f, out_f) || !te_aligned16(W)) return TE_ERR_UNSUPPORTED;
  if (planes_bytes_ < te_linear_x6_weight_planes_bytes(in_f, out_f) || !te_aligned16(planes)) return TE_ERR_WORKSPACE;
  hipStream_t stream = (hipStream_t)stream_;
  unsigned char* pz = (unsigned char*)planes;
  unsigned char* pc = pz + weight_planes(in_f, out_f).c;
  split_kernel<OP_ABS, false><<<producer_grid(out_f, in_f), dim3(256), 0, stream>>>(W, pz, out_f, in_f, 3, 0);
  const dim3 gc = producer_grid(in_f, out_f);
  split_kernel<OP_POS, true><<<gc, dim3(256), 0, stream>>>(W, pc, in_f, out_f, 6, 0);
  split_kernel<OP_NEG, true><<<gc, dim3(256), 0, stream>>>(W, pc, in_f, out_f, 6, 1);
  TE_RETURN_IF_LAUNCH_FAILED();
  return TE_OK;
}

extern "C" size_t te_linear_x6_planes_bytes(int64_t rows, int64_t K) {
  return (rows < 1 || bad_k(K)) ? 0 : planes_bytes(rows, K);
}

extern "C" int te_linear_x6_split_abs_f32(const float* X, int64_t rows, int64_t K, void* planes, size_t planes_bytes_,
                                          te_stream_t stream_) {
  const int rc = check_producer(X && planes, te_aligned16(X), te_aligned16(planes), rows, K, planes_bytes_);
  if (rc != TE_OK) return rc;
  split_kernel<OP_ABS, false><<<producer_grid(rows, K), dim3(256), 0, (hipStream_t)stream_>>>(X, (unsigned char*)planes, rows, K, 3, 0);
  TE_RETURN_IF_LAUNCH_FAILED();
  return TE_OK;
}

extern "C" int te_gemm_x6_supported(int64_t T, int64_t K, int64_t M) {
  return (T >= 1 && K >= 128 && M >= 128 && K % 16 == 0 && M % 128 == 0 && K <= (1 << 20) && M <= (1 << 20) &&
          T <= (int64_t)1 << 26) ? 1 : 0;
}

extern "C" int te_linear_x6_split_matrix_f32(const float* A, int64_t rows, int64_t K, int transposed, void* planes,
                                             size_t planes_bytes_, te_stream_t stream_) {
  const int rc = check_producer(A && planes, te_aligned16(A), te_aligned16(planes), rows, K, planes_bytes_);
  if (rc != TE_OK) return rc;
  const dim3 grid = producer_grid(rows, K);
  if (transposed)
    split_kernel<OP_ID, true><<<grid, dim3(256), 0, (hipStream_t)stream_>>>(A, (unsigned char*)planes, rows, K, 3, 0);
  else
    split_kernel<OP_ID, false><<<grid, dim3(256), 0, (hipStream_t)stream_>>>(A, (unsigned char*)planes, rows, K, 3, 0);
  TE_RETURN_IF_LAUNCH_FAILED();
  return TE_OK;
}

extern "C" int te_linear_x6_split_dual_f32(const float* A, int64_t rows, int64_t K, void* planes, void* planes_abs,
                                           size_t planes_bytes_, te_stream_t stream_) {
  const int rc = check_producer(A && planes && planes_abs, te_aligned16(A), te_aligned16(planes) && te_aligned16(planes_abs), rows, K, planes_bytes_);
  if (rc != TE_OK) return rc;
  split_kernel<OP_ID, false><<<producer_grid(rows, K), dim3(256), 0, (hipStream_t)stream_>>>(A, (unsigned char*)planes, rows, K, 3, 0,
                                                                                           (unsigned char*)planes_abs);
  TE_RETURN_IF_LAUNCH_FAILED();
  return TE_OK;
}

extern "C" int te_gelu_backward_x6_planes_f32(const float* dy, const float* x, int64_t rows, int64_t K, void* planes,
                                              size_t planes_bytes_, te_stream_t stream_) {
  const int rc = check_producer(dy && x && planes, te_aligned16(dy) && te_aligned16(x), te_aligned16(planes), rows, K, planes_bytes_);
  if (rc != TE_OK) return rc;
  gelu_split_lds_kernel<SRC_GELU_BWD><<<producer_grid(rows, K), dim3(256), 0, (hipStream_t)stream_>>>(
      dy, x, nullptr, (unsigned char*)planes, nullptr, rows, K);
  TE_RETURN_IF_LAUNCH_FAILED();
  return TE_OK;
}

extern "C" int te_gelu_forward_x6_planes_f32(const float* x, float* y, int64_t rows, int64_t K, void* planes, void* planes_abs,
                                             size_t planes_bytes_, te_stream_t stream_) {
  const int rc = check_producer(x && y && planes, te_aligned16(x) && te_aligned16(y),
                                te_aligned16(planes) && (!planes_abs || te_aligned16(planes_abs)), rows, K, planes_bytes_);
  if (rc != TE_OK) return rc;
  gelu_split_lds_kernel<SRC_GELU_FWD><<<producer_grid(rows, K), dim3(256), 0, (hipStream_t)stream_>>>(
      nullptr, x, y, (unsigned char*)planes, (unsigned char*)planes_abs, rows, K);
  TE_RETURN_IF_LAUNCH_FAILED();
  return TE_OK;
}

extern "C" size_t te_gemm_x6_workspace_bytes(int64_t T, int64_t K, int64_t M) {
  return te_gemm_x6_supported(T, K, M) ? gemm_workspace(T, K, M).total : 0;
}

extern "C" int te_gemm_x6_f32(const float* X, const void* x_planes, const void* w_planes, const float* bias, float* out,
                              int64_t T, int64_t K, int64_t M, int flags, unsigned* status, void* ws, size_t ws_bytes,
                              te_stream_t stream_) {
  if ((!X && !x_planes) || !w_planes || !out) return TE_ERR_INVALID_ARG;
  if ((flags & ~kProductFlags) != 0) return TE_ERR_INVALID_ARG;
  if (!te_gemm_x6_supported(T, K, M)) return TE_ERR_UNSUPPORTED;
  if (!ws || ws_bytes < te_gemm_x6_workspace_bytes(T, K, M) || !te_aligned16(ws)) return TE_ERR_WORKSPACE;
  if ((X && !te_aligned16(X)) || !te_aligned16(out) || !te_aligned16(w_planes) || (bias && !te_aligned16(bias)) ||
      (x_planes && !te_aligned16(x_planes)))
    return TE_ERR_UNSUPPORTED;
  hipStream_t stream = (hipStream_t)stream_;
  const X6Workspace l = gemm_workspace(T, K, M);
  zero_flag_regions(l.flag_region(ws, 0), 1, stream);
  if (!x_planes) {
    int rc = te_linear_x6_split_matrix_f32(X, T, K, 0, l.x(ws, 0), planes_bytes(T, K), stream_);
    if (rc != TE_OK) return rc;
    x_planes = l.x(ws, 0);
  }
  const int wm = choose_geo((M % 256 == 0) ? 2 : 1, T, M, flags & kTileMask, 192, true);
  const int rc = launch_pass<MODE_G>(call_params(T, l.acc(ws), bias, out, status, flags), wm, (const unsigned char*)w_planes,
                                     (const unsigned char*)x_planes, nullptr, K, M, l.flag_region(ws, 0), stream);
  if (rc != TE_OK) return rc;
  TE_RETURN_IF_LAUNCH_FAILED();
  return TE_OK;
}

extern "C" size_t te_linear_relprop_x6_workspace_bytes(int64_t T, int64_t in_f, int64_t out_f) {
  return te_linear_relprop_x6_supported(T, in_f, out_f) ? rule_workspace(T, in_f, out_f).total : 0;
}

extern "C" int te_linear_relprop_x6_f32(const float* R, const float* r_scale, int64_t r_scale_stride,
                                        int64_t rows_per_sample, const float* X, const float* W, const void* w_planes,
                                        const void* x_planes, const float* Y, const float* bias, float* out, int64_t T,
                                        int64_t in_f, int64_t out_f, int flags, unsigned* status, void* ws,
                                        size_t ws_bytes, te_stream_t stream_) {
  if (!R || !X || !W || !w_planes || !Y || !out || T <= 0) return TE_ERR_INVALID_ARG;
  if (!te_linear_relprop_x6_supported(T, in_f, out_f)) return TE_ERR_UNSUPPORTED;
  if (!ws || ws_bytes < te_linear_relprop_x6_workspace_bytes(T, in_f, out_f) || !te_aligned16(ws)) return TE_ERR_WORKSPACE;
  if (!te_aligned16(X) || !te_aligned16(W) || !te_aligned16(R) || !te_aligned16(Y) || !te_aligned16(out) ||
      !te_aligned16(w_planes) || (bias && !te_aligned16(bias)) || (x_planes && !te_aligned16(x_planes)))
    return TE_ERR_UNSUPPORTED;
  if (bad_r_scale(r_scale, rows_per_sample, T)) return TE_ERR_INVALID_ARG;
  if ((flags & ~kRuleFlags) != 0) return TE_ERR_INVALID_ARG;
  const int phases = (flags & TE_X6_PHASE_MASK) ? (flags & TE_X6_PHASE_MASK) : TE_X6_PHASE_MASK;
  hipStream_t stream = (hipStream_t)stream_;
  const X6Workspace l = rule_workspace(T, in_f, out_f);
  unsigned char* Ss = l.sp(ws, 0);
  const unsigned char* wz = (const unsigned char*)w_planes;
  const unsigned char* wc = wz + weight_planes(in_f, out_f).c;

  if (phases & TE_X6_PHASE_SPLIT) zero_flag_regions(l.flag_region(ws, 0), kRulePasses, stream);
  const bool x_signed = (flags & TE_X6_X_PLANES_SIGNED) != 0;
  if (!x_planes) {
    if (phases & TE_X6_PHASE_SPLIT) {
      int rc = x_signed ? te_linear_x6_split_matrix_f32(X, T, in_f, 0, l.x(ws, 0), planes_bytes(T, in_f), stream_)
                        : te_linear_x6_split_abs_f32(X, T, in_f, l.x(ws, 0), planes_bytes(T, in_f), stream_);
      if (rc != TE_OK) return rc;
    }
    x_planes = l.x(ws, 0);
  }
  const int wm_max = pick_wm(in_f, out_f);
  const int pz = (flags >> TE_X6_TILE_Z_SHIFT) & kTileMask, pc = (flags >> TE_X6_TILE_C_SHIFT) & kTileMask;
  const int wm_z = choose_geo(wm_max, T, out_f, pz ? pz : (flags & kTileMask), 256, true);
  const int wm_c = choose_geo(wm_max, T, 2 * in_f, pc ? pc : (flags & kTileMask));
  const X6Params p = rule_params(call_params(T, l.acc(ws), bias, out, status, flags), R, r_scale, r_scale_stride, rows_per_sample,
                                 X, W, Y);
  int rc;
  if (phases & TE_X6_PHASE_Z) {
    rc = x_signed ? launch_pass<MODE_ZS>(p, wm_z, wz, (const unsigned char*)x_planes, Ss, in_f, out_f, l.flag_region(ws, 0), stream, 1.0f)
                  : launch_pass<MODE_Z>(p, wm_z, wz, (const unsigned char*)x_planes, Ss, in_f, out_f, l.flag_region(ws, 0), stream, 1.0f);
    if (rc != TE_OK) return rc;
  }
  if (phases & TE_X6_PHASE_C) {
    rc = launch_pass<MODE_C>(p, wm_c, wc, Ss, Ss, in_f, out_f, l.flag_region(ws, 1), stream, 1.0f);
    if (rc != TE_OK) return rc;
  }
  TE_RETURN_IF_LAUNCH_FAILED();
  return TE_OK;
}

extern "C" int te_linear_relprop_x6_general_supported(int64_t T, int64_t in_f, int64_t out_f, int variant) {
  if (!te_linear_relprop_x6_supported(T, in_f, out_f)) return 0;
  if (variant == TE_VARIANT_LRP) return (in_f % 128 == 0) ? 1 : 0;
  return variant == TE_VARIANT_OURS ? 1 : 0;
}

extern "C" size_t te_linear_x6_weight_planes_lrp_bytes(int64_t in_f, int64_t out_f) {
  return te_linear_relprop_x6_general_supported(1, in_f, out_f, TE_VARIANT_LRP) ? weight_planes_lrp(in_f, out_f).total : 0;
}

extern "C" int te_linear_x6_prepare_weights_lrp_f32(const float* W, int64_t in_f, int64_t out_f, void* planes,
                                                    size_t planes_bytes_, te_stream_t stream_) {
  if (!W || !planes) return TE_ERR_INVALID_ARG;
  if (!te_linear_relprop_x6_general_supported(1, in_f, out_f, TE_VARIANT_LRP) || !te_aligned16(W)) return TE_ERR_UNSUPPORTED;
  if (planes_bytes_ < te_linear_x6_weight_planes_lrp_bytes(in_f, out_f) || !te_aligned16(planes)) return TE_ERR_WORKSPACE;
  hipStream_t stream = (hipStream_t)stream_;
  unsigned char* q = (unsigned char*)planes;
  const X6WeightPlanesLrp wl = weight_planes_lrp(in_f, out_f);
  const dim3 gz = producer_grid(out_f, in_f), gc = producer_grid(in_f, out_f);
  split_kernel<OP_POS, false><<<gz, dim3(256), 0, stream>>>(W, q, out_f, in_f, 3, 0);
  split_kernel<OP_NEG, false><<<gz, dim3(256), 0, stream>>>(W, q + wl.wn, out_f, in_f, 3, 0);
  split_kernel<OP_POS, true><<<gc, dim3(256), 0, stream>>>(W, q + wl.wpT, in_f, out_f, 3, 0);
  split_kernel<OP_NEG, true><<<gc, dim3(256), 0, stream>>>(W, q + wl.wnT, in_f, out_f, 3, 0);
  TE_RETURN_IF_LAUNCH_FAILED();
  return TE_OK;
}

extern "C" size_t te_linear_relprop_x6_general_workspace_bytes(int64_t T, int64_t in_f, int64_t out_f, int variant) {
  return te_linear_relprop_x6_general_supported(T, in_f, out_f, variant) ? general_workspace(T, in_f, out_f).total : 0;
}

extern "C" int te_linear_relprop_x6_general_f32(const float* R, const float* r_scale, int64_t r_scale_stride,
                                                int64_t rows_per_sample, const float* X, const float* W,
                                                const void* w_planes, const void* w_planes_lrp, const void* x_abs_planes,
                                                const float* Y, const float* bias, float* out, int64_t T, int64_t in_f,
                                                int64_t out_f, float alpha, int variant, int flags, unsigned* status,
                                                void* ws, size_t ws_bytes, te_stream_t stream_) {
  if (!R || !X || !W || !out || T <= 0) return TE_ERR_INVALID_ARG;
  if (!te_linear_relprop_x6_general_supported(T, in_f, out_f, variant)) return TE_ERR_UNSUPPORTED;
  const bool lrp = variant == TE_VARIANT_LRP;
  if (lrp ? !w_planes_lrp : (!w_planes || !Y)) return TE_ERR_INVALID_ARG;
  if (!ws || ws_bytes < te_linear_relprop_x6_general_workspace_bytes(T, in_f, out_f, variant) || !te_aligned16(ws))
    return TE_ERR_WORKSPACE;
  if (!te_aligned16(X) || !te_aligned16(W) || !te_aligned16(R) || (Y && !te_aligned16(Y)) || !te_aligned16(out) ||
      (w_planes && !te_aligned16(w_planes)) || (w_planes_lrp && !te_aligned16(w_planes_lrp)) ||
      (bias && !te_aligned16(bias)) || (x_abs_planes && !te_aligned16(x_abs_planes)))
    return TE_ERR_UNSUPPORTED;
  if (bad_r_scale(r_scale, rows_per_sample, T)) return TE_ERR_INVALID_ARG;
  if ((flags & ~kProductFlags) != 0) return TE_ERR_INVALID_ARG;
  hipStream_t stream = (hipStream_t)stream_;
  const float beta = alpha - 1.0f;
  const X6Workspace l = general_workspace(T, in_f, out_f);
  unsigned char* Xa = l.x(ws, 0), *Xb = l.x(ws, 1);
  unsigned char* Sa = l.sp(ws, 0), *Sb = l.sp(ws, 1);
  zero_flag_regions(l.flag_region(ws, 0), kGeneralPasses, stream);

  const X6Params p = rule_params(call_params(T, l.acc(ws), bias, out, status ? status : l.flag_region(ws, kGeneralPasses - 1) + kErrWord, flags),
                                 R, r_scale, r_scale_stride, rows_per_sample, X, W, Y);
  const int pin = flags & kTileMask;
  const int wm_z = choose_geo(pick_wm(in_f, out_f), T, out_f, pin, 256, true);
  int pass = 0;
  int rc;
  if (!lrp) {
    const unsigned char* wz = (const unsigned char*)w_planes;
    const unsigned char* wc = wz + weight_planes(in_f, out_f).c;
    if (!x_abs_planes) {
      rc = te_linear_x6_split_abs_f32(X, T, in_f, Xa, planes_bytes(T, in_f), stream_);
      if (rc != TE_OK) return rc;
      x_abs_planes = Xa;
    }
    const int wm_c = choose_geo(pick_wm(in_f, out_f), T, 2 * in_f, pin);
    rc = launch_pass<MODE_Z>(p, wm_z, wz, (const unsigned char*)x_abs_planes, Sa, in_f, out_f, l.flag_region(ws, pass++), stream);
    if (rc != TE_OK) return rc;
    rc = launch_pass<MODE_C>(p, wm_c, wc, Sa, nullptr, in_f, out_f, l.flag_region(ws, pass++), stream, alpha);
    if (rc != TE_OK) return rc;
    if (beta != 0.0f) {
      rc = launch_pass<MODE_ZI>(p, wm_z, wz, (const unsigned char*)x_abs_planes, Sa, in_f, out_f, l.flag_region(ws, pass++), stream);
      if (rc != TE_OK) return rc;
      rc = launch_pass<MODE_CI>(p, wm_c, wc, Sa, nullptr, in_f, out_f, l.flag_region(ws, pass++), stream, -beta);
      if (rc != TE_OK) return rc;
    }
  } else {
    const X6WeightPlanesLrp wl = weight_planes_lrp(in_f, out_f);
    const unsigned char* Wp = (const unsigned char*)w_planes_lrp;
    const unsigned char* Wn = Wp + wl.wn, *WpT = Wp + wl.wpT, *WnT = Wp + wl.wnT;
    split_kernel<OP_POS, false><<<producer_grid(T, in_f), dim3(256), 0, stream>>>(X, Xa, T, in_f, 3, 0);
    split_kernel<OP_NEG, false><<<producer_grid(T, in_f), dim3(256), 0, stream>>>(X, Xb, T, in_f, 3, 0);
    const int wm_x = choose_geo((in_f % 256 == 0) ? 2 : 1, T, in_f, pin, 192, true);
    auto x_pass = [&](const unsigned char* AT, const unsigned char* S, int sign, float scale, int accum) -> int {
      return launch_pass<MODE_X>(p, wm_x, AT, S, nullptr, in_f, out_f, l.flag_region(ws, pass++), stream, scale, accum, sign);
    };
    for (int half = 0; half < (beta != 0.0f ? 2 : 1); ++half) {
      const unsigned char* w1 = half ? Wn : Wp, *w2 = half ? Wp : Wn, *w1T = half ? WnT : WpT, *w2T = half ? WpT : WnT;
      const float sc = half ? -beta : alpha;
      if (half) {
        pass = 0;
        static_assert(kGeneralPasses >= 5, "four passes per half + the region of the per-call error word");
// ... 31 lines not shown
```

transformer-explainability_amd/ops.py:

```python
from __future__ import annotations

import contextlib
import os
from typing import Optional, Sequence, Tuple

import torch

from . import _lib
from ._lib import (TE_HEADMEAN_CLAMP, TE_HEADMEAN_ROW0, TE_IMPL_SIMPLE, TE_RATIONALE_CLAMP, TE_ROLLOUT_CLS_FIXUP,
                   TE_ROLLOUT_NORMALISE, TE_ROLLOUT_ROW0, TE_VARIANT_LRP, TE_VARIANT_OURS)
from ._lib import (TE_X6_PHASE_C, TE_X6_PHASE_SPLIT, TE_X6_PHASE_Z, TE_X6_TEST_DROP_HANDOVER,
                   TE_X6_TEST_SMALL_GRID, TE_X6_TILE_C_SHIFT, TE_X6_TILE_Z_SHIFT, TE_X6_WHOLE_TILES, TE_X6_X_PLANES_SIGNED)

Tensor = torch.Tensor
_VARIANTS = {"ours": TE_VARIANT_OURS, "lrp": TE_VARIANT_LRP}

FORCE_SIMPLE = False
KERNEL_TIMER = None
_NULL = contextlib.nullcontext()


def _timed(name: str, flops: float = 0.0, nbytes: float = 0.0):
    return _NULL if KERNEL_TIMER is None else KERNEL_TIMER(name, float(flops), float(nbytes))

# ... 160 lines not shown
    return bad


def x6_failed(device=None) -> bool:
    return bool(_x6_failed_words(device))


def x6_raise_if_failed(device=None, reset: bool = True):
    bad = _x6_failed_words(device)
    if bad:
        if reset:
            for t in bad:
                t.zero_()
        raise _lib.TeError("an x6 Linear kernel waited in vain for the accumulators of a tile it shares with another "
                           "workgroup (bounded stream-K hand-over expired): the affected outputs were poisoned with NaN and "
                           "every map computed since the last check is invalid.  Typical causes: several persistent x6 "
                           "launches competing for the CUs (more than one step in flight), a profiler or another process "
                           "holding CUs.  Re-run the step; set TE_LINEAR_X6=0 to use the fp32-MFMA kernels instead")


_x6_posted = {}


def x6_post(device):
    if not torch.cuda.is_available() or torch.cuda.is_current_stream_capturing():
        return
    idx = _x6_device_index(device)
    t = _x6_status.get(idx)
    if t is None:
        return
    ent = _x6_posted.get(idx)
    if ent is None:
        ent = _x6_posted[idx] = [torch.zeros(4, dtype=torch.int32).pin_memory(), torch.cuda.Event(), False]
    elif ent[2] and not ent[1].query():
        return
    with torch.cuda.device(idx):
        ent[0].copy_(t, non_blocking=True)
        ent[1].record()
    ent[2] = True


def x6_poll(device):
    if not _x6_posted or torch.cuda.is_current_stream_capturing():
        return
    ent = _x6_posted.get(_x6_device_index(device))
    if ent is None or not ent[2] or not ent[1].query():
        return
    ent[2] = False
    if int(ent[0][0]) != 0:
        x6_raise_if_failed(device)


def _weight_key(W: Tensor):
    return (W.data_ptr(), W._version, tuple(W.shape), tuple(W.stride()), str(W.device))


def x6_invalidate(obj) -> int:
    mods = obj.modules() if hasattr(obj, "modules") else [obj]
    n = 0
    for m in mods:
        c = getattr(m, "__dict__", {}).get("_te_cache")
        if c:
            c.clear()
            n += 1
    return n


def _cached_planes(W: Tensor, cache: Optional[dict], name: str, build) -> tuple:
    key = _weight_key(W)
    hit = None if cache is None else cache.get(name)
    if hit is None or hit[0] != key:
        hit = (key, *build(W.detach()))
        if cache is not None:
            cache[name] = hit
    return hit[1:]


def _prepare_planes(Wc: Tensor, bytes_fn: str, prepare_fn: str, dims: tuple, *extra) -> Tensor:
    with _on_device(Wc) as lib:
        planes = _ws(getattr(lib, bytes_fn)(*dims), Wc)
        _lib.check(getattr(lib, prepare_fn)(_ptr(Wc), *dims, *extra, _ptr(planes), planes.numel(), _stream(Wc)), prepare_fn)
    return planes


def x6_weight_planes(W: Tensor, cache: Optional[dict] = None) -> Tensor:
    out_f, in_f = W.shape
    return _cached_planes(W, cache, "x6_planes", lambda Wd: (_prepare_planes(
        _c(Wd), "te_linear_x6_weight_planes_bytes", "te_linear_x6_prepare_weights_f32", (in_f, out_f)),))[0]


X6_GEMM = {"": "all", "1": "all", "0": "off"}.get(os.environ.get("TE_X6_GEMM", "all"), os.environ.get("TE_X6_GEMM", "all"))
if X6_GEMM not in ("all", "auto", "off"):
    raise ValueError(f"TE_X6_GEMM={X6_GEMM!r}: expected all / auto / off (or 1 / 0)")


def gemm_x6_wanted(T: int, K: int, M: int) -> bool:
    if X6_GEMM == "off" or T < 256 or not gemm_x6_supported(T, K, M):
        return False
    return X6_GEMM == "all" or (K <= 1024 and M >= 2 * K)


def x6_weight_planes_lrp(W: Tensor, cache: Optional[dict] = None) -> Tensor:
    out_f, in_f = W.shape
    return _cached_planes(W, cache, "x6_planes_lrp", lambda Wd: (_prepare_planes(
        _c(Wd), "te_linear_x6_weight_planes_lrp_bytes", "te_linear_x6_prepare_weights_lrp_f32", (in_f, out_f)),))[0]


def x6_matrix_planes(W: Tensor, transposed: bool, cache: Optional[dict] = None) -> Tensor:
    out_f, in_f = W.shape
    dims = (in_f, out_f) if transposed else (out_f, in_f)
    return _cached_planes(W, cache, "x6_gemm_planes_T" if transposed else "x6_gemm_planes", lambda Wd: (_prepare_planes(
        _c(Wd), "te_linear_x6_planes_bytes", "te_linear_x6_split_matrix_f32", dims, int(transposed)),))[0]


def linear_relprop_x6_supported(T: int, in_f: int, out_f: int) -> bool:
    return bool(_lib.load().te_linear_relprop_x6_supported(int(T), int(in_f), int(out_f)))


def gemm_x6_supported(T: int, K: int, M: int) -> bool:
    return bool(_lib.load().te_gemm_x6_supported(int(T), int(K), int(M)))


X6_KEEP_ABS = os.environ.get("TE_X6_KEEP_ABS", "1") not in ("", "0")
X6_SIGNED_PLANES = True


def _signed(planes: Tensor) -> Tensor:
    planes._te_signed_planes = True
    return planes


def planes_are_signed(planes: Optional[Tensor]) -> bool:
    return planes is not None and getattr(planes, "_te_signed_planes", False)


def _x_abs_key(X: Tensor, T: int, K: int):
    return (X.data_ptr(), X._version, T, K, str(X.device))


def post_x_planes(cache: dict, X: Tensor, xs: Tensor, xa: Optional[Tensor] = None):
    K = X.shape[-1]
    cache["x_planes_from_producer"] = (_x_abs_key(X, X.numel() // K, K), xs, xa, X)


def take_x_planes(cache: dict, X: Tensor, T: int, K: int):
    hit = cache.pop("x_planes_from_producer", None)
    if hit is not None and hit[0] == _x_abs_key(X, T, K) and hit[3].data_ptr() == X.data_ptr():
        return hit[1], hit[2]
    return None


def drop_x_planes(cache: dict, with_abs: bool = False):
    cache.pop("x_planes_from_producer", None)
    if with_abs:
        cache.pop("x_abs_planes", None)


def post_x_abs_planes(cache: dict, X: Tensor, T: int, K: int, xa: Tensor):
    cache["x_abs_planes"] = (_x_abs_key(X, T, K), xa)


def take_x_abs_planes(cache: dict, X: Tensor, T: int, K: int) -> Optional[Tensor]:
    keep = _X_ABS_KEPT
    hit = cache.get("x_abs_planes") if keep is not None and not keep.last else cache.pop("x_abs_planes", None)
    return hit[1] if hit is not None and hit[0] == _x_abs_key(X, T, K) else None


_X_ABS_KEPT = None


class x_abs_planes_kept:

    def __init__(self, caches):
        self.caches, self.last = list(caches), False

    def __enter__(self):
        global _X_ABS_KEPT
        self._outer, _X_ABS_KEPT = _X_ABS_KEPT, self
        return self

    def __exit__(self, *exc):
        global _X_ABS_KEPT
        _X_ABS_KEPT = self._outer
        for c in self.caches:
            c.pop("x_abs_planes", None)
        return False


def post_dy_planes(cache: dict, planes: Tensor, like: Tensor) -> Tensor:
    base = torch.full((1,), float("nan"), dtype=like.dtype, device=like.device)
    cache["dy_planes_from_consumer"] = (base, tuple(like.shape), planes)
    return base.expand(like.shape)


def take_dy_planes(cache: dict, dy: Tensor) -> Optional[Tensor]:
    hit = cache.pop("dy_planes_from_consumer", None)
    if hit is not None and dy.data_ptr() == hit[0].data_ptr() and tuple(dy.shape) == hit[1] and not any(dy.stride()):
        return hit[2]
    return None


def rule_takes_abs_planes(T: int, in_f: int, out_f: int) -> bool:
    return bool(USE_LINEAR_X6 and X6_KEEP_ABS and linear_relprop_x6_supported(T, in_f, out_f))


def gemm_x6(X: Tensor, w_planes: Tensor, bias: Optional[Tensor], M: int, timer_name: str = "gemm_x6",
            keep_abs: Optional[dict] = None, x_planes: Optional[Tensor] = None) -> Tensor:
    K = X.shape[-1]
    lead = X.shape[:-1]
    T = X.numel() // K
    Xc = None if x_planes is not None else _c(X).reshape(-1, K)
    like = X if Xc is None else Xc
    out = torch.empty((T, M), dtype=torch.float32, device=X.device)
    bc = None if bias is None else _c(bias.detach())
    with _on_device(like) as lib:
        ws = _ws(lib.te_gemm_x6_workspace_bytes(T, K, M), like)
        x_bytes = (6.0 if x_planes is not None else 10.0) * T * K
        xs = x_planes
        if xs is None and keep_abs is not None:
            got = take_x_planes(keep_abs, X, T, K)
            if got is not None:
                xs, x_bytes = got[0], 6.0 * T * K
                post_x_abs_planes(keep_abs, X, T, K, got[1] if got[1] is not None else _signed(xs))
        if xs is not None and xs.numel() * xs.element_size() < lib.te_linear_x6_planes_bytes(T, K):
            raise _lib.TeError(f"gemm_x6: the operand planes handed in hold {xs.numel() * xs.element_size()} bytes, "
                               f"[{T}, {K}] needs {lib.te_linear_x6_planes_bytes(T, K)}")
        for_rule = xs is None and keep_abs is not None and rule_takes_abs_planes(T, K, M)
        if for_rule and not X6_SIGNED_PLANES:
            x_bytes += 6.0 * T * K
        with _timed(timer_name, 12.0 * T * K * M, x_bytes + 6.0 * K * M + 4.0 * T * M):
            if for_rule:
                nb = lib.te_linear_x6_planes_bytes(T, K)
                if X6_SIGNED_PLANES:
                    xs = _signed(_ws(nb, Xc))
                    _lib.check(lib.te_linear_x6_split_matrix_f32(_ptr(Xc), T, K, 0, _ptr(xs), nb, _stream(Xc)),
                               "te_linear_x6_split_matrix_f32")
                    post_x_abs_planes(keep_abs, X, T, K, xs)
                else:
                    xs, xa = _ws(nb, Xc), _ws(nb, Xc)
                    _lib.check(lib.te_linear_x6_split_dual_f32(_ptr(Xc), T, K, _ptr(xs), _ptr(xa), nb, _stream(Xc)),
                               "te_linear_x6_split_dual_f32")
                    post_x_abs_planes(keep_abs, X, T, K, xa)
            _lib.check(lib.te_gemm_x6_f32(_ptr(Xc) if Xc is not None else None, _ptr(xs), _ptr(w_planes), _ptr(bc), _ptr(out),
                                          T, K, M, (X6_TILE | X6_FLAGS) & ~0x3c00, _ptr(x6_status(X.device)), _ptr(ws),
                                          ws.numel(), _stream(like)), "te_gemm_x6_f32")
    return out.reshape(*lead, M)


def linear_relprop(R: Tensor, X: Tensor, W: Tensor, alpha: float = 1.0, variant="ours",
                   Y: Optional[Tensor] = None, bias: Optional[Tensor] = None, cache: Optional[dict] = None) -> Tensor:
    if _any_f64(R, X, W):
        return linear_relprop_f64(R, X, W, alpha=alpha, variant=variant)
    if _is_bf16(X) or _is_bf16(W):
        return linear_relprop_bf16(R, X, W, alpha=alpha, variant=variant, cache=cache)
    out_f, in_f = W.shape
    lead = X.shape[:-1]
    R, r_scale = _split_deferred(R)
    Rc, Xc, Wc = _c(R).reshape(-1, out_f), _c(X).reshape(-1, in_f), _c(W)
    T = Xc.shape[0]
    if Rc.shape[0] != T:
        raise _lib.TeError(f"Linear.relprop: R has {Rc.shape[0]} rows, X has {T}")
    out = torch.empty((T, in_f), dtype=torch.float32, device=X.device)
    var = _variant(variant)
    fast_ok = (var == TE_VARIANT_OURS and alpha == 1 and in_f % 4 == 0 and out_f % 4 == 0 and
               all(t.data_ptr() % 16 == 0 for t in (Rc, Xc, Wc)))
    fwd = fast_ok and USE_FORWARD_OUTPUT and Y is not None
    if r_scale is not None and not fwd:
        Rc = _c(Deferred(R, r_scale).materialise()).reshape(-1, out_f)
        r_scale = None
    rs_ptr, rs_stride, rps = None, 0, 1
    if r_scale is not None:
        rs_ptr, rs_stride, rps = r_scale.data_ptr(), r_scale.stride(0), T // r_scale.shape[0]
    var_code = var & 0xff
    general = (USE_LINEAR_X6 and not (var & TE_IMPL_SIMPLE) and not (var_code == TE_VARIANT_OURS and alpha == 1)
               and all(t.data_ptr() % 16 == 0 for t in (Rc, Xc, Wc))
               and (var_code == TE_VARIANT_LRP or (USE_FORWARD_OUTPUT and Y is not None))
               and bool(_lib.load().te_linear_relprop_x6_general_supported(T, in_f, out_f, var_code)))
    if general:
        Yg = bg = None
        if var_code == TE_VARIANT_OURS:
            Yg = _c(Y.detach()).reshape(-1, out_f)
            bg = None if bias is None else _c(bias.detach())
            general = Yg.shape[0] == T and Yg.data_ptr() % 16 == 0 and (bg is None or bg.data_ptr() % 16 == 0)
    if general:
        wp = x6_weight_planes(W, cache) if var_code == TE_VARIANT_OURS else None
        wpl = x6_weight_planes_lrp(W, cache) if var_code == TE_VARIANT_LRP else None
        xa = take_x_abs_planes(cache, X, T, in_f) if cache is not None and var_code == TE_VARIANT_OURS else None
        if planes_are_signed(xa):
            xa = None
        gemm = 2.0 * T * in_f * out_f
        halves = 2 if alpha != 1 else 1
        units = (18.0 if var_code == TE_VARIANT_OURS else 24.0) * halves
        with _on_device(Xc) as lib, _timed("linear_x6_general", units * gemm,
                                           halves * (6.0 * (2 * T * in_f + 3 * in_f * out_f + 2 * T * out_f) + 16.0 * T * in_f)):
            ws = _ws(lib.te_linear_relprop_x6_general_workspace_bytes(T, in_f, out_f, var_code), Xc)
            _lib.check(lib.te_linear_relprop_x6_general_f32(_ptr(Rc), rs_ptr, rs_stride, rps, _ptr(Xc), _ptr(Wc), _ptr(wp),
                                                            _ptr(wpl), _ptr(xa), _ptr(Yg), _ptr(bg), _ptr(out), T, in_f,
                                                            out_f, float(alpha), var_code, (X6_TILE | X6_FLAGS) & ~0x3c00,
                                                            _ptr(x6_status(Xc.device)), _ptr(ws), ws.numel(), _stream(Xc)),
                       "te_linear_relprop_x6_general_f32")
            if X6_CHECK:
                x6_raise_if_failed(Xc.device)
        return out.reshape(*lead, in_f)
    if fwd:
        Yc = _c(Y.detach()).reshape(-1, out_f)
        bc = None if bias is None else _c(bias.detach())
        if Yc.shape[0] != T:
            raise _lib.TeError(f"Linear.relprop: Y has {Yc.shape[0]} rows, X has {T}")
    if (fwd and USE_LINEAR_X6 and Yc.data_ptr() % 16 == 0 and (bc is None or bc.data_ptr() % 16 == 0)
            and _lib.load().te_linear_relprop_x6_supported(T, in_f, out_f)):
        planes = x6_weight_planes(W, cache)
        xa = take_x_abs_planes(cache, X, T, in_f) if cache is not None else None
        x_signed = TE_X6_X_PLANES_SIGNED if planes_are_signed(xa) else 0
        with _on_device(Xc) as lib:
            ws = _ws(lib.te_linear_relprop_x6_workspace_bytes(T, in_f, out_f), Xc)
            status = x6_status(Xc.device)

            def call(flags):
                _lib.check(lib.te_linear_relprop_x6_f32(_ptr(Rc), rs_ptr, rs_stride, rps, _ptr(Xc), _ptr(Wc), _ptr(planes),
                                                        _ptr(xa), _ptr(Yc), _ptr(bc), _ptr(out), T, in_f, out_f,
                                                        X6_TILE | X6_FLAGS | x_signed | flags, _ptr(status), _ptr(ws), ws.numel(),
                                                        _stream(Xc)),
                           "te_linear_relprop_x6_f32")
            if KERNEL_TIMER is None:
                call(0)
            else:
                gemm = 2.0 * T * in_f * out_f
                if xa is None:
                    with _timed("linear_x6_split", 0.0, 10.0 * T * in_f):
                        call(TE_X6_PHASE_SPLIT)
                else:
                    call(TE_X6_PHASE_SPLIT)
                with _timed("linear_x6_zpass", 6.0 * gemm, 6.0 * (T * in_f + in_f * out_f + T * out_f) + 8.0 * T * out_f):
                    call(TE_X6_PHASE_Z)
                with _timed("linear_x6_cpass", 12.0 * gemm, 6.0 * (T * out_f + 2 * in_f * out_f) + 8.0 * T * in_f):
                    call(TE_X6_PHASE_C)
            if X6_CHECK:
                rc = lib.te_linear_relprop_x6_check(_ptr(ws), T, in_f, out_f, _stream(Xc))
                if rc != 0:
                    status.zero_()
                    raise _lib.TeError(f"te_linear_relprop_x6_f32({T},{in_f},{out_f}): a workgroup waited in vain for the "
                                       f"accumulators of a shared tile (status {rc}); the result is invalid")
                x6_raise_if_failed(Xc.device)
        return out.reshape(*lead, in_f)
    if KERNEL_TIMER is not None and fast_ok:
        with _on_device(Xc) as lib:
            S = torch.empty((T, out_f), dtype=torch.float32, device=X.device)
            st = _stream(Xc)
            if fwd:
                with _timed("linear_zpass_fwd", 2.0 * T * in_f * out_f, 4.0 * (T * in_f + 3 * T * out_f + in_f * out_f)):
                    _lib.check(lib.te_linear_zpass_fwd_f32(_ptr(Rc), rs_ptr, rs_stride, rps, _ptr(Xc), _ptr(Wc),
                                                           _ptr(Yc), _ptr(bc), _ptr(S), T, in_f, out_f, st),
                               "te_linear_zpass_fwd_f32")
            else:
                with _timed("linear_zpass", 2.0 * T * (2 * in_f) * out_f, 4.0 * (T * in_f + 2 * T * out_f + in_f * out_f)):
                    _lib.check(lib.te_linear_zpass_f32(_ptr(Rc), _ptr(Xc), _ptr(Wc), _ptr(S), T, in_f, out_f, st),
                               "te_linear_zpass_f32")
            with _timed("linear_cpass", 2.0 * T * (2 * in_f) * out_f, 4.0 * (T * out_f + 2 * T * in_f + in_f * out_f)):
                _lib.check(lib.te_linear_cpass_f32(_ptr(S), _ptr(Xc), _ptr(Wc), _ptr(out), T, in_f, out_f, st),
                           "te_linear_cpass_f32")
        return out.reshape(*lead, in_f)
    with _on_device(Xc) as lib:
        ws = _ws(lib.te_linear_relprop_workspace_bytes(T, in_f, out_f, var), Xc)
        if fwd:
            _lib.check(lib.te_linear_relprop_fwd_f32(_ptr(Rc), rs_ptr, rs_stride, rps, _ptr(Xc), _ptr(Wc),
                                                     _ptr(Yc), _ptr(bc), _ptr(out), T, in_f, out_f, _ptr(ws),
                                                     ws.numel(), _stream(Xc)),
                       "te_linear_relprop_fwd_f32")
        else:
            _lib.check(lib.te_linear_relprop_f32(_ptr(Rc), _ptr(Xc), _ptr(Wc), _ptr(out), T, in_f, out_f, float(alpha),
                                                 var, _ptr(ws), ws.numel(), _stream(Xc)), "te_linear_relprop_f32")
    return out.reshape(*lead, in_f)


def _bhnd(t: Tensor) -> Tuple[Tensor, int, int, int]:
    t = _prep(t)
    if t.stride(-1) != 1 or min(t.stride()[:3]) < 0:
        t = t.contiguous()
    sb, sh, sn, _ = t.stride()
    return t, sb, sh, sn


def _cached_z(z: Optional[Tensor], shape) -> Optional[Tensor]:
    if z is None or not USE_FORWARD_PRODUCTS or tuple(z.shape) != tuple(shape):
        return None
    return _c(z.detach())


def matmul_relprop_av(R: Tensor, attn: Tensor, v: Tensor, out_scale: float = 1.0,
                      cam_v_out: Optional[Tensor] = None, variant="ours", z: Optional[Tensor] = None
                      ) -> Tuple[Tensor, Tensor]:
    if _any_f64(R, attn, v):
        return matmul_relprop_av_f64(R, attn, v, out_scale, cam_v_out, variant, z)
    if _is_bf16(attn) or _is_bf16(v):
        return matmul_relprop_av_bf16(R, attn, v, out_scale, cam_v_out, variant, z)
    B, H, N, D = v.shape
    zc = None
    z_str = (H * N * D, N * D, D)
# ... 164 lines not shown
    hd = lambda t: (None, 0, 0, 0) if t is None else _heads(_prep(t), H)
    (q, qb, qh, qn), (k, kb, kh, kn), (v, vb, vh, vn) = hd(q), hd(k), hd(v)
    (dq, dqb, dqh, dqn), (dk, dkb, dkh, dkn), (dv, dvb, dvh, dvn) = hd(d_q), hd(d_k), hd(d_v)
    with _on_device(d_out) as lib, _timed("attention_backward", (8.0 if need_qk else 4.0) * B * H * N * N * D,
                                          4.0 * B * ((4 if need_qk else 2) * H * N * N + 8 * N * C)):
        ws = _ws(lib.te_attention_backward_strided_workspace_bytes(B, H, N), d_out)
        if not (out is not None and tuple(out.shape) == (B, N, C) and out.dtype == d_out.dtype and out.stride(-1) == 1):
            out = None
        (o, ob, oh, on) = hd(out)
        _lib.check(lib.te_attention_backward_strided_f32(_ptr(d_out), N * C, 64, C, _ptr(o), ob, oh, on, _ptr(q), qb, qh, qn,
                                                         _ptr(k), kb, kh, kn, _ptr(v), vb, vh, vn, _ptr(attn), _ptr(d_attn),
                                                         _ptr(dq), dqb, dqh, dqn, _ptr(dk), dkb, dkh, dkn, _ptr(dv), dvb, dvh,
                                                         dvn, B, H, N, D, float(scale), int(bool(need_qk)), _ptr(ws),
                                                         ws.numel(), _stream(d_out)), "te_attention_backward_strided_f32")
    return d_attn


def attention_forward_planes_supported(qkv: Tensor, num_heads: int) -> bool:
    B, N, C3 = qkv.shape
    C = C3 // 3
    return (qkv.is_cuda and qkv.dtype == torch.float32 and C % num_heads == 0 and C // num_heads == 64 and N <= 224
            and bool(_lib.load().te_attention_forward_supported(N, 64)))


def attention_forward(qkv: Tensor, num_heads: int, scale: float, planes: bool = False, planes_abs: bool = True):
    if _is_bf16(qkv):
        if planes:
            raise _lib.TeError("attention_forward(planes=True): operand planes are emitted from float32 activations only")
        qkv = _c16(qkv)
        C = qkv.shape[-1] // 3
        out, attn, zqk, _ = attention_forward_qkv_bf16(qkv[..., :C], qkv[..., C:2 * C], qkv[..., 2 * C:], num_heads, scale)
        return out, attn, zqk
    qkv = _c(qkv)
    B, N, C3 = qkv.shape
    C = C3 // 3
    H, D = num_heads, C // num_heads
    if not _lib.load().te_attention_forward_supported(N, D):
        if planes:
            raise _lib.TeError("attention_forward(planes=True): shape not served by te_attention_forward_f32")
        out, attn, zqk, _ = attention_forward_qkv(qkv[..., :C], qkv[..., C:2 * C], qkv[..., 2 * C:], num_heads, scale)
        return out, attn, zqk
    out = torch.empty((B, N, C), dtype=torch.float32, device=qkv.device)
    attn = torch.empty((B, H, N, N), dtype=torch.float32, device=qkv.device)
    zqk = torch.empty((B, H, N, N), dtype=torch.float32, device=qkv.device)
    extra = (12.0 if planes_abs else 6.0) * B * N * C if planes else 0.0
    with _on_device(qkv) as lib, _timed("attention_forward", 4.0 * B * H * N * N * D, 4.0 * B * (2 * H * N * N + 4 * N * C) + extra):
        nb, xs, xa = 0, None, None
        if planes:
            nb = lib.te_linear_x6_planes_bytes(B * N, C)
            xs, xa = _ws(nb, qkv), _ws(nb, qkv) if planes_abs else None
        _lib.check(lib.te_attention_forward_f32(_ptr(qkv), _ptr(zqk), _ptr(attn), _ptr(out), _ptr(xs), _ptr(xa), nb, B, H, N,
                                                D, float(scale), _stream(qkv)), "te_attention_forward_f32")
    return (out, attn, zqk, xs, xa) if planes else (out, attn, zqk)


def attention_backward(d_out: Tensor, qkv: Tensor, attn: Tensor, num_heads: int, scale: float,
                       need_qk: bool = True, out: Optional[Tensor] = None) -> Tuple[Tensor, Optional[Tensor]]:
    if _is_bf16(d_out) or _is_bf16(qkv) or _is_bf16(attn):
        qkv = _c16(qkv)
        C = qkv.shape[-1] // 3
        d_qkv = torch.empty_like(qkv)
        th = lambda t, i: t[..., i * C:(i + 1) * C]
        d_attn = attention_backward_qkv_bf16(d_out, th(qkv, 0), th(qkv, 1), th(qkv, 2), attn, num_heads, scale,
                                             th(d_qkv, 0), th(d_qkv, 1), th(d_qkv, 2), need_qk=need_qk)
        return d_attn, d_qkv
    d_out, qkv, attn = _c(d_out), _c(qkv), _c(attn)
    B, N, C3 = qkv.shape
    C = C3 // 3
    H, D = num_heads, C // num_heads
    d_qkv = torch.empty_like(qkv)
    if not _lib.load().te_attention_forward_supported(N, D):
        th = lambda t, i: t[..., i * C:(i + 1) * C]
        d_attn = attention_backward_qkv(d_out, th(qkv, 0), th(qkv, 1), th(qkv, 2), attn, num_heads, scale,
                                        th(d_qkv, 0), th(d_qkv, 1), th(d_qkv, 2), need_qk=need_qk, out=out)
        return d_attn, d_qkv
    d_attn = torch.empty_like(attn)
    with _on_device(qkv) as lib, _timed("attention_backward", (8.0 if need_qk else 4.0) * B * H * N * N * D,
                                        4.0 * B * ((4 if need_qk else 2) * H * N * N + 8 * N * C)):
        if not (out is not None and need_qk and tuple(out.shape) == tuple(d_out.shape) and out.is_contiguous()
                and out.dtype == d_out.dtype):
            out = None
        _lib.check(lib.te_attention_backward_f32(_ptr(d_out), _ptr(out), _ptr(qkv), _ptr(attn), _ptr(d_attn), _ptr(d_qkv), B,
                                                 H, N, D, float(scale), int(bool(need_qk)), _stream(qkv)),
                   "te_attention_backward_f32")
    return d_attn, d_qkv


def layernorm_supported(x: Tensor) -> bool:
    return (x.is_cuda and x.dtype == torch.float32 and x.dim() >= 2
            and bool(_lib.load().te_layernorm_supported(int(x.shape[-1]))))


def layernorm_forward(x: Tensor, weight: Tensor, bias: Optional[Tensor], eps: float) -> Tuple[Tensor, Tensor, Tensor]:
    x = _c(x)
    C = x.shape[-1]
    T = x.numel() // C
    y = torch.empty_like(x)
    mean = torch.empty((T,), dtype=torch.float32, device=x.device)
    rstd = torch.empty((T,), dtype=torch.float32, device=x.device)
    with _on_device(x) as lib, _timed("layernorm_forward", 0.0, 4.0 * 2 * T * C):
        _lib.check(lib.te_layernorm_forward_f32(_ptr(x), _ptr(_c(weight)), _ptr(_c(bias)) if bias is not None else None,
                                                _ptr(y), _ptr(mean), _ptr(rstd), T, C, float(eps), _stream(x)),
                   "te_layernorm_forward_f32")
    return y, mean, rstd


def layernorm_backward(dy: Tensor, x: Tensor, weight: Tensor, mean: Tensor, rstd: Tensor,
                       add: Optional[Tensor] = None) -> Tensor:
    dy, x = _c(dy), _c(x)
    C = x.shape[-1]
    T = x.numel() // C
    dx = torch.empty_like(x)
    with _on_device(x) as lib, _timed("layernorm_backward", 0.0, 4.0 * (3 + (add is not None)) * T * C):
        _lib.check(lib.te_layernorm_backward_f32(_ptr(dy), _ptr(x), _ptr(_c(weight)), _ptr(mean), _ptr(rstd),
                                                 _ptr(_c(add)) if add is not None else None, _ptr(dx), T, C, _stream(x)),
                   "te_layernorm_backward_f32")
    return dx


def gelu_forward(x: Tensor) -> Tensor:
    x = _c(x)
    y = torch.empty_like(x)
    with _on_device(x) as lib, _timed("gelu_forward", 0.0, 4.0 * 2 * x.numel()):
        _lib.check(lib.te_gelu_forward_f32(_ptr(x), _ptr(y), x.numel(), _stream(x)), "te_gelu_forward_f32")
    return y


X6_FUSE_GELU = os.environ.get("TE_X6_FUSE_GELU", "1") not in ("", "0")


_GELU_BWD_HANDOFF = 0


class gelu_backward_plane_handoff:

    def __enter__(self):
        global _GELU_BWD_HANDOFF
        _GELU_BWD_HANDOFF += 1
        return self

    def __exit__(self, *exc):
        global _GELU_BWD_HANDOFF
        _GELU_BWD_HANDOFF -= 1


def gelu_backward_handoff_active() -> bool:
    return _GELU_BWD_HANDOFF > 0


def gelu_planes_supported(x: Tensor) -> bool:
    return bool(X6_FUSE_GELU and x.dim() >= 2 and x.shape[-1] >= 16 and x.shape[-1] % 16 == 0)


def gelu_forward_planes(x: Tensor, planes_abs: bool = True):
    x = _c(x)
    K = x.shape[-1]
    T = x.numel() // K
    y = torch.empty_like(x)
    with _on_device(x) as lib, _timed("gelu_forward", 0.0, (4.0 * 2 + (12.0 if planes_abs else 6.0)) * x.numel()):
        nb = lib.te_linear_x6_planes_bytes(T, K)
        xs, xa = _ws(nb, x), _ws(nb, x) if planes_abs else None
        _lib.check(lib.te_gelu_forward_x6_planes_f32(_ptr(x), _ptr(y), T, K, _ptr(xs), _ptr(xa), nb, _stream(x)),
                   "te_gelu_forward_x6_planes_f32")
    return y, xs, xa


def gelu_backward_planes(dy: Tensor, x: Tensor) -> Tensor:
    dy, x = _c(dy), _c(x)
    K = x.shape[-1]
    T = x.numel() // K
    with _on_device(x) as lib, _timed("gelu_backward", 0.0, (4.0 * 2 + 6.0) * x.numel()):
        nb = lib.te_linear_x6_planes_bytes(T, K)
        planes = _ws(nb, x)
        _lib.check(lib.te_gelu_backward_x6_planes_f32(_ptr(dy), _ptr(x), T, K, _ptr(planes), nb, _stream(x)),
                   "te_gelu_backward_x6_planes_f32")
    return planes


def gelu_backward(dy: Tensor, x: Tensor) -> Tensor:
    dy, x = _c(dy), _c(x)
    dx = torch.empty_like(x)
    with _on_device(x) as lib, _timed("gelu_backward", 0.0, 4.0 * 3 * x.numel()):
        _lib.check(lib.te_gelu_backward_f32(_ptr(dy), _ptr(x), _ptr(dx), x.numel(), _stream(x)), "te_gelu_backward_f32")
    return dx


USE_DEFERRED_ADD = True


def _is_bcast_mask(X0: Tensor, X1: Tensor) -> bool:
    return X1.dim() == 4 and X0.dim() == 4 and X1.shape[1] == 1 and X1.shape[2] == 1 and X0.shape[1] * X0.shape[2] != 1


def add_relprop(R: Tensor, X0: Tensor, X1: Tensor, variant="ours", deferred: bool = False):
    if _any_f64(R, X0, X1):
        return add_relprop_f64(R, X0, X1, variant, deferred)
    if _is_bf16(X0) or _is_bf16(X1):
        return add_relprop_bf16(R, X0, X1, variant, deferred)
    B = X0.shape[0]
    R, X0 = _c(R), _c(X0)
    n = X0[0].numel()
    if _is_bcast_mask(X0, X1):
        H, N = X0.shape[1], X0.shape[3]
        mask = _c(X1).reshape(X1.shape[0], N)
        if mask.shape[0] == 1 and B > 1:
            mask = mask.expand(B, N).contiguous()
        out0 = torch.empty_like(X0)
        out1 = torch.empty((B, 1, 1, N), dtype=torch.float32, device=X0.device)
        if deferred and _variant(variant) == TE_VARIANT_OURS:
            fac = torch.empty((B, 2), dtype=torch.float32, device=X0.device)
            with _on_device(X0) as lib, _timed("add_bcast_mask_deferred", 0.0, 4.0 * B * (3 * H * N * N + 2 * N)):
                ws = _ws(lib.te_add_bcast_relprop_workspace_bytes(B, H, N), X0)
                _lib.check(lib.te_add_bcast_relprop_deferred_f32(_ptr(R), _ptr(X0), _ptr(mask), _ptr(out0), _ptr(out1),
                                                                 _ptr(fac), B, H, N, _ptr(ws), ws.numel(), _stream(X0)),
                           "te_add_bcast_relprop_deferred_f32")
            return Deferred(out0, fac[:, 0]), out1
        with _on_device(X0) as lib, _timed("add_bcast_mask", 0.0, 4.0 * B * (3 * H * N * N + 2 * N)):
            ws = _ws(lib.te_add_bcast_relprop_workspace_bytes(B, H, N), X0)
            _lib.check(lib.te_add_bcast_relprop_f32(_ptr(R), _ptr(X0), _ptr(mask), _ptr(out0), _ptr(out1), B, H, N,
                                                    _variant(variant), _ptr(ws), ws.numel(), _stream(X0)),
                       "te_add_bcast_relprop_f32")
        return out0, out1
    X1 = _c(X1)
    if X1.shape == X0.shape:
        x1_bs = n
    elif X1.shape[0] == 1 and X1.shape[1:] == X0.shape[1:]:
        x1_bs = 0
    else:
        raise _lib.TeError(f"Add.relprop: unsupported operand shapes {tuple(X0.shape)} + {tuple(X1.shape)}")
    out0, out1 = torch.empty_like(X0), torch.empty_like(X0)
    var = _variant(variant)
    x1_elems = n if x1_bs else n / B
    if deferred and var == TE_VARIANT_OURS:
        fac = torch.empty((B, 2), dtype=torch.float32, device=X0.device)
        with _on_device(X0) as lib, _timed("add_deferred", 0.0, 4.0 * B * (4 * n + x1_elems)):
            ws = _ws(lib.te_add_relprop_deferred_workspace_bytes(B, n), X0)
            _lib.check(lib.te_add_relprop_deferred_f32(_ptr(R), _ptr(X0), _ptr(X1), _ptr(out0), _ptr(out1), _ptr(fac), B,
                                                       n, x1_bs, _ptr(ws), ws.numel(), _stream(X0)),
                       "te_add_relprop_deferred_f32")
        return Deferred(out0, fac[:, 0]), Deferred(out1, fac[:, 1])
    with _on_device(X0) as lib, _timed("add", 0.0, 4.0 * B * (4 * n + x1_elems)):
        ws = _ws(lib.te_add_relprop_workspace_bytes(B, n), X0)
        _lib.check(lib.te_add_relprop_f32(_ptr(R), _ptr(X0), _ptr(X1), _ptr(out0), _ptr(out1), B, n, x1_bs,
                                          var, _ptr(ws), ws.numel(), _stream(X0)), "te_add_relprop_f32")
    return out0, out1


def clone_relprop(Rs: Sequence, X: Tensor) -> Tensor:
    if len(Rs) not in (2, 3):
        raise _lib.TeError(f"Clone.relprop supports 2 or 3 aliases, got {len(Rs)}")
    if _any_f64(X, *Rs):
        return clone_relprop_f64(Rs, X)
    bf = _is_bf16(X)
    X = _c16(X) if bf else _c(X)
    sfx = "bf16" if bf else "f32"
    pairs = [_split_deferred(r) for r in Rs]
    Rs = [_c(r) for r, _ in pairs]
    scales = [sc for _, sc in pairs]
    for r in Rs:
        if r.numel() != X.numel():
            raise _lib.TeError("Clone.relprop: relevance / input size mismatch")
    out = torch.empty(X.shape, dtype=torch.float32, device=X.device)
    nb = 4.0 * X.numel() * (len(Rs) + 1) + X.element_size() * X.numel()
    if any(sc is not None for sc in scales):
        B = X.shape[0]
        sp = [(None, 0) if sc is None else (sc.data_ptr(), sc.stride(0)) for sc in scales] + [(None, 0)]
        with _on_device(X) as lib, _timed("clone", 0.0, nb):
            _lib.check(getattr(lib, "te_clone_relprop_scaled_" + sfx)(
                _ptr(Rs[0]), sp[0][0], sp[0][1], _ptr(Rs[1]), sp[1][0], sp[1][1], _ptr(Rs[2]) if len(Rs) == 3 else None,
                sp[2][0], sp[2][1], _ptr(X), _ptr(out), B, X.numel() // B, _stream(X)), "te_clone_relprop_scaled_" + sfx)
        return out
    with _on_device(X) as lib, _timed("clone", 0.0, nb):
        _lib.check(getattr(lib, "te_clone_relprop_" + sfx)(_ptr(Rs[0]), _ptr(Rs[1]), _ptr(Rs[2]) if len(Rs) == 3 else None,
                                                           _ptr(X), _ptr(out), X.numel(), _stream(X)),
                   "te_clone_relprop_" + sfx)
    return out


def index_select_relprop(R: Tensor, X: Tensor, index: int) -> Tensor:
    if _any_f64(R, X):
        return index_select_relprop_f64(R, X, index)
    bf = _is_bf16(X)
    X = _c16(X) if bf else _c(X)
    B, N, C = X.shape
    R = _c(R).reshape(B, C)
    out = torch.empty(X.shape, dtype=torch.float32, device=X.device)
    sfx = "bf16" if bf else "f32"
    with _on_device(X) as lib:
        _lib.check(getattr(lib, "te_index_select_relprop_" + sfx)(_ptr(R), _ptr(X), _ptr(out), B, N, C, int(index),
                                                                   _stream(X)), "te_index_select_relprop_" + sfx)
    return out


def gradcam_headmean(grad: Tensor, cam: Tensor, out: Optional[Tensor] = None) -> Tensor:
    if _any_f64(grad, cam, out):
        return gradcam_headmean_f64(grad, cam, out)
    bf = _is_bf16(grad)
    grad, cam = (_c16(grad) if bf else _c(grad)), _c(cam)
    B, H, N, _ = cam.shape
    if out is None:
        out = torch.empty((B, N, N), dtype=torch.float32, device=cam.device)
    sfx = "bf16" if bf else "f32"
    with _on_device(cam) as lib, _timed("headmean", 0.0, (grad.element_size() + 4.0) * B * H * N * N + 4.0 * B * N * N):
        _lib.check(getattr(lib, "te_gradcam_headmean_" + sfx)(_ptr(grad), _ptr(cam), _ptr(out), B, H, N, _stream(cam)),
                   "te_gradcam_headmean_" + sfx)
    return out


def attn_headmean(attn: Tensor, out: Optional[Tensor] = None, clamp: bool = False, row0: bool = False) -> Tensor:
    attn = _prep_bf16(attn)
    if attn.dim() != 4 or attn.shape[2] != attn.shape[3]:
        raise _lib.TeError(f"attn_headmean: expected [B,H,N,N] attention probabilities, got {tuple(attn.shape)}")
    B, H, N, _ = attn.shape
    if attn.stride(3) != 1 or attn.stride(2) != N:
        attn = attn.contiguous()
    shape = (B, N) if row0 else (B, N, N)
    if out is None:
        out = torch.empty(shape, dtype=torch.float32, device=attn.device)
    elif tuple(out.shape) != shape or out.dtype != torch.float32 or not out.is_contiguous() or out.device != attn.device:
        raise _lib.TeError(f"attn_headmean: out must be a contiguous float32 {shape} on {attn.device}")
# ... 1268 lines not shown
```

transformer-explainability_amd/producers.py:

```python
from __future__ import annotations

import torch

from . import ops


def usable(x: torch.Tensor) -> bool:
    return ops.USE_FUSED_PRODUCERS and torch.is_tensor(x) and ops.layernorm_supported(x)


def gelu_usable(x: torch.Tensor) -> bool:
    return (ops.USE_FUSED_PRODUCERS and torch.is_tensor(x) and x.is_cuda and x.dtype == torch.float32
            and x.numel() > 0 and x.numel() % 4 == 0)


def norm_usable(x: torch.Tensor, norm) -> bool:
    return (usable(x) and not norm.training and getattr(norm, "weight", None) is not None
            and tuple(norm.normalized_shape) == (x.shape[-1],))


class _LayerNorm(torch.autograd.Function):
    @staticmethod
    def forward(ctx, x, weight, bias, eps):
        y, mean, rstd = ops.layernorm_forward(x, weight, bias, eps)
        ctx.save_for_backward(x, weight, mean, rstd)
        return y

    @staticmethod
    def backward(ctx, dy):
        x, weight, mean, rstd = ctx.saved_tensors
        return ops.layernorm_backward(dy, x, weight, mean, rstd), None, None, None


class _ResidualLayerNorm(torch.autograd.Function):

    @staticmethod
    def forward(ctx, x, weight, bias, eps):
        y, mean, rstd = ops.layernorm_forward(x, weight, bias, eps)
        ctx.save_for_backward(x, weight, mean, rstd)
        return x.view_as(x), y

    @staticmethod
    def backward(ctx, d_bypass, dy):
        x, weight, mean, rstd = ctx.saved_tensors
        if dy is None:
            return d_bypass, None, None, None
        return ops.layernorm_backward(dy, x, weight, mean, rstd, add=d_bypass), None, None, None


class _Gelu(torch.autograd.Function):

    @staticmethod
    def forward(ctx, x, feeds, source):
        ctx.save_for_backward(x)
        ctx.source = source
        if feeds is not None:
            y, xs, xa = ops.gelu_forward_planes(x, not ops.X6_SIGNED_PLANES)
            ops.post_x_planes(feeds, y, xs, xa)
            return y
        return ops.gelu_forward(x)

    @staticmethod
    def backward(ctx, dy):
        (x,) = ctx.saved_tensors
        if ctx.source is not None:
            return ops.post_dy_planes(ctx.source, ops.gelu_backward_planes(dy, x), x), None, None
        return ops.gelu_backward(dy, x), None, None


class _Linear(torch.autograd.Function):

    @staticmethod
    def forward(ctx, x, weight, bias, cache, fwd_x6, bwd_x6):
        ctx.weight, ctx.cache, ctx.bwd_x6 = weight, cache, bwd_x6
        if fwd_x6:
            return ops.gemm_x6(x, ops.x6_matrix_planes(weight, False, cache), bias, weight.shape[0], "linear_forward_x6",
                               keep_abs=cache)
        return torch.nn.functional.linear(x, weight, bias)

    @staticmethod
    def backward(ctx, dy):
        w = ctx.weight
        if ctx.bwd_x6:
            dx = ops.gemm_x6(dy, ops.x6_matrix_planes(w, True, ctx.cache), None, w.shape[1], "linear_backward_x6",
                             x_planes=ops.take_dy_planes(ctx.cache, dy))
        else:
            dx = torch.matmul(dy, w)
        return dx, None, None, None, None, None


def linear_plan(x: torch.Tensor, lin):
    if not (ops.USE_FUSED_PRODUCERS and ops.X6_GEMM != "off" and torch.is_tensor(x) and x.is_cuda
            and x.dtype == torch.float32 and not lin.training and x.dim() >= 2):
        return False, False
    out_f, in_f = lin.weight.shape
    T = x.numel() // in_f
    return ops.gemm_x6_wanted(T, in_f, out_f), ops.gemm_x6_wanted(T, out_f, in_f)


def takes_producer_planes(lin, T: int, K: int) -> bool:
    out_f, in_f = lin.weight.shape
    return bool(K == in_f and ops.USE_FUSED_PRODUCERS and ops.X6_GEMM != "off" and not lin.training
                and ops.gemm_x6_wanted(T, in_f, out_f) and ops.rule_takes_abs_planes(T, in_f, out_f))


def _d(t):
    return None if t is None else t.detach()


def linear(x, lin, cache, plan):
    out = _Linear.apply(x, _d(lin.weight), _d(lin.bias), cache, plan[0], plan[1])
    if plan[1]:
        out._te_bwd_x6_cache = cache
    return out


def layer_norm(x, norm):
    return _LayerNorm.apply(x, _d(norm.weight), _d(norm.bias), norm.eps)


def residual_layer_norm(x, norm):
    return _ResidualLayerNorm.apply(x, _d(norm.weight), _d(norm.bias), norm.eps)


def gelu(x, consumer=None, consumer_cache=None):
    feeds = source = None
    if ops.gelu_planes_supported(x):
        K = x.shape[-1]
        if consumer is not None and takes_producer_planes(consumer, x.numel() // K, K):
            feeds = consumer_cache
        if ops.gelu_backward_handoff_active():
            source = getattr(x, "_te_bwd_x6_cache", None)
    if feeds is None and consumer_cache is not None:
        ops.drop_x_planes(consumer_cache)
    return _Gelu.apply(x, feeds, source)
```

transformer-explainability_amd/rules.py:

```python
from __future__ import annotations

import contextlib

import torch
import torch.nn as nn

from . import ops

__all__ = ['forward_hook', 'Clone', 'Add', 'Cat', 'ReLU', 'GELU', 'Dropout', 'BatchNorm2d', 'Linear', 'MaxPool2d',
           'AdaptiveAvgPool2d', 'AvgPool2d', 'Conv2d', 'Sequential', 'safe_divide', 'einsum', 'Softmax',
           'IndexSelect', 'LayerNorm', 'AddEye', 'Tanh', 'MatMul', 'Mul']


def safe_divide(a, b):
    den = b.clamp(min=1e-9) + b.clamp(max=1e-9)
    den = den + den.eq(0).type(den.type()) * 1e-9
    return a / den * b.ne(0).type(b.type())


def forward_hook(self, input, output):
    if type(input[0]) in (list, tuple):
        self.X = [i.detach() for i in input[0]]
    else:
        self.X = input[0].detach()
    self.Y = output
    self._y_version = output._version if torch.is_tensor(output) else None
    w = getattr(self, "weight", None)
    b = getattr(self, "bias", None)
    self._w_version = (w._version if torch.is_tensor(w) else None, b._version if torch.is_tensor(b) else None)


class StopRelprop(Exception):
    """Raised by an attention module whose ``_stop_after_attn_cam`` flag is set, right after it stored its attn_cam:
    the model-level relprop loop catches it (extension: ``prune_below_start_layer``, see vit.VisionTransformer)."""


@contextlib.contextmanager
def stop_after_attn_cam(attn_module):
    if attn_module is not None:
        attn_module._stop_after_attn_cam = True
    try:
        yield
    finally:
        if attn_module is not None:
            attn_module._stop_after_attn_cam = False


def _cached_y(module):
    y = getattr(module, "Y", None)
    if not torch.is_tensor(y) or getattr(module, "_y_version", None) != y._version:
        return None
    w = getattr(module, "weight", None)
    b = getattr(module, "bias", None)
    now = (w._version if torch.is_tensor(w) else None, b._version if torch.is_tensor(b) else None)
    if getattr(module, "_w_version", now) != now:
        return None
    return y


class RelProp(nn.Module):
    variant = "ours"

    def __init__(self):
        super(RelProp, self).__init__()
        self.register_forward_hook(forward_hook)

    def relprop(self, R, alpha):
        return R

    def attnlrp(self, G, eps):
        raise NotImplementedError(f"{type(self).__name__}.attnlrp: AttnLRP has no rule for this module")


class _Identity(RelProp):
    """Rules that pass relevance through unchanged (layers_ours.py:67-80,86-87) need no cached input."""


def _no_cache_hook(self, input, output):
    self.Y = output


class ReLU(nn.ReLU, RelProp):
    pass


class GELU(nn.GELU, RelProp):
    def feeds(self, linear):
        self.__dict__["_te_feeds"] = (linear,)
        return self

    def forward(self, x):
        from . import producers
        if getattr(self, "approximate", "none") == "none" and not self.training and producers.gelu_usable(x):
            nxt = self.__dict__.get("_te_feeds", (None,))[0]
            return producers.gelu(x, nxt, x6_cache(nxt) if isinstance(nxt, Linear) else None)
        return super().forward(x)

    def attnlrp(self, G, eps):
        if getattr(self, "approximate", "none") != "none":
            raise NotImplementedError("GELU.attnlrp: the identity rule is implemented for the exact (erf) GELU")
        return ops.alrp_act(G, self.X, "gelu")


class Softmax(nn.Softmax, RelProp):
    pass


class LayerNorm(nn.LayerNorm, RelProp):
    def forward(self, x):
        from . import producers
        if producers.norm_usable(x, self):
            return producers.layer_norm(x, self)
        return super().forward(x)

    def attnlrp(self, G, eps):
        if len(self.normalized_shape) != 1:
            raise NotImplementedError("LayerNorm.attnlrp: normalisation over the last dimension only")
        gamma = self.weight if self.weight is not None else torch.ones(self.normalized_shape, device=G.device)
        return ops.alrp_layernorm(G, gamma, ops.alrp_row_rstd(self.X, self.eps))


class Dropout(nn.Dropout, RelProp):
    pass


class Tanh(nn.Tanh, RelProp):
    def attnlrp(self, G, eps):
        return ops.alrp_act(G, self.X, "tanh")


def x6_cache(module) -> dict:
    c = module.__dict__.get("_te_cache")
    if c is None:
        c = module.__dict__["_te_cache"] = {}
    return c


class _ScratchCache:

    def __getstate__(self):
        state = self.__dict__.copy()
        state.pop("_te_cache", None)
        return state

    def _load_from_state_dict(self, *args, **kwargs):
        super()._load_from_state_dict(*args, **kwargs)
        ops.x6_invalidate(self)

    def _apply(self, fn, *args, **kwargs):
        ops.x6_invalidate(self)
        return super()._apply(fn, *args, **kwargs)


class Linear(_ScratchCache, nn.Linear, RelProp):

    def forward(self, x):
        from . import producers
        plan = producers.linear_plan(x, self)
        if not plan[0]:
            ops.drop_x_planes(x6_cache(self), with_abs=True)
        if plan[0] or plan[1]:
            return producers.linear(x, self, x6_cache(self), plan)
        return super().forward(x)

    def relprop(self, R, alpha):
        return linear_rule(self, R, alpha)

    def attnlrp(self, G, eps):
        Y = self.Y.detach()
        if Y.shape != G.shape:
            raise ops._lib.TeError(f"Linear.attnlrp: G {tuple(G.shape)} does not have the shape of the cached output "
                                   f"{tuple(Y.shape)}")
        return ops.alrp_linear(ops.alrp_damp(G, Y, eps), self.weight, x6_cache(self))


def linear_rule(m, R, alpha, rows=None, variant=None):
    X, Y = m.X, _cached_y(m)
    if Y is not None and Y.shape[:-1] != X.shape[:-1]:
        Y = None
    if rows is not None:
        X, Y = rows(X), None if Y is None else rows(Y)
    return ops.linear_relprop(R, X, m.weight.detach(), alpha=alpha, variant=variant or m.variant, Y=Y, bias=m.bias,
                              cache=x6_cache(m))


class Add(RelProp):

    def forward(self, inputs):
        return torch.add(*inputs)

    def relprop(self, R, alpha, deferred=False):
        x0, x1 = self.X
        bcast_mask = x0.dim() == 4 and x1.dim() == 4 and x1.shape[1] == 1 and x1.shape[2] == 1
        a, b = ops.add_relprop(R, x0, x1, variant=self.variant,
                               deferred=deferred and ops.USE_DEFERRED_ADD and (x0.shape == x1.shape or bcast_mask))
        return [a, b]

    def attnlrp(self, G, eps):
        return ops.alrp_damp(G, self.Y.detach(), eps)


class einsum(RelProp):

    def __init__(self, equation):
        super().__init__()
        self.equation = equation

    def forward(self, *operands):
        ops_ = operands[0] if (len(operands) == 1 and isinstance(operands[0], (list, tuple))) else operands
        eq = self.equation.replace(" ", "")
        if eq == 'bhid,bhjd->bhij' and len(ops_) == 2:
            return torch.matmul(ops_[0], ops_[1].transpose(-1, -2))
        if eq == 'bhij,bhjd->bhid' and len(ops_) == 2:
            return torch.matmul(ops_[0], ops_[1])
        return torch.einsum(self.equation, *operands)

    def relprop(self, R, alpha):
        eq = self.equation.replace(" ", "")
        if eq == 'bhij,bhjd->bhid':
            cam_attn, cam_v = ops.matmul_relprop_av(R, self.X[0], self.X[1], variant=self.variant, z=_cached_y(self))
            return [cam_attn, cam_v]
        if eq == 'bhid,bhjd->bhij':
            cam_q, cam_k = ops.matmul_relprop_qk(R, self.X[0], self.X[1], variant=self.variant, z=_cached_y(self))
            return [cam_q, cam_k]
        raise NotImplementedError(f"einsum.relprop: equation {self.equation!r} is not on the accelerated path")


class MatMul(RelProp):

    def forward(self, inputs):
        return torch.matmul(*inputs)

    def relprop(self, R, alpha):
        x0, x1 = self.X
        if x0.dim() != 4 or x1.dim() != 4:
            raise NotImplementedError("MatMul.relprop: only [B,H,.,.] attention products are accelerated")
        if x1.stride(-1) != 1 and x1.stride(-2) == 1:
            k = x1.transpose(-1, -2)
            cam_q, cam_k = ops.matmul_relprop_qk(R, x0, k, variant=self.variant, z=_cached_y(self))
            return [cam_q, cam_k.transpose(-1, -2)]
        if x0.shape[-1] == x0.shape[-2] == x1.shape[-2]:
            cam_attn, cam_v = ops.matmul_relprop_av(R, x0, x1, variant=self.variant, z=_cached_y(self))
            return [cam_attn, cam_v]
        if x0.shape[-1] == x1.shape[-2]:
            k = x1.transpose(-1, -2).contiguous()
            cam_q, cam_k = ops.matmul_relprop_qk(R, x0, k, variant=self.variant, z=_cached_y(self))
            return [cam_q, cam_k.transpose(-1, -2)]
        raise NotImplementedError("MatMul.relprop: operand shapes are not an attention product")


def attention_attnlrp(G_o, q, k, v, attn, num_heads, scale, d_q, d_k, d_v):
    B, N, C = G_o.shape
    H, D = num_heads, C // num_heads
    if ops._lib.load().te_attention_strided_supported(N, D):
        ops.attention_backward_qkv(G_o, q, k, v, attn, H, scale, d_q, d_k, d_v, need_qk=True)
        return
    heads = lambda t: t.view(B, N, H, D).permute(0, 2, 1, 3)
    go = heads(ops._c(G_o))
    d_attn = torch.matmul(go, heads(v).transpose(-1, -2))
    heads(d_v).copy_(torch.matmul(attn.transpose(-1, -2), go))
    d_s = attn * (d_attn - (d_attn * attn).sum(dim=-1, keepdim=True))
    heads(d_q).copy_(torch.matmul(d_s, heads(k)) * scale)
    heads(d_k).copy_(torch.matmul(d_s.transpose(-1, -2), heads(q)) * scale)


class Clone(RelProp):

    def forward(self, input, num):
        self.__setattr__('num', num)
        return [input for _ in range(num)]

    def relprop(self, R, alpha):
        return ops.clone_relprop(list(R), self.X)

    def attnlrp(self, G, eps):
        G = list(G)
        out = G[0] + G[1]
        for g in G[2:]:
            out += g
        return out


class IndexSelect(RelProp):

    def forward(self, inputs, dim, indices):
        self.__setattr__('dim', dim)
        self.__setattr__('indices', indices)
        if not torch.is_tensor(indices):
            self._index_host = int(indices)
        elif indices.numel() == 1 and (not indices.is_cuda or getattr(self, "_index_src", None) is not indices
                                       or getattr(self, "_index_version", None) != indices._version):
            if not (indices.is_cuda and torch.cuda.is_current_stream_capturing()):
                self._index_host = int(indices)
                self._index_src = indices
                self._index_version = indices._version
        return torch.index_select(inputs, dim, indices.reshape(-1) if torch.is_tensor(indices) else indices)

    def relprop(self, R, alpha):
        idx = self.indices
        if self.dim != 1 or self.X.dim() != 3 or (torch.is_tensor(idx) and idx.numel() != 1):
            raise NotImplementedError("IndexSelect.relprop: only dim=1 with a single index is accelerated")
        host = getattr(self, "_index_host", None)
        if host is None or (torch.is_tensor(idx) and (getattr(self, "_index_src", idx) is not idx
                                                      or getattr(self, "_index_version", idx._version) != idx._version)):
            host = int(idx)
        return ops.index_select_relprop(R, self.X, host)

    def attnlrp(self, G, eps):
        idx = self.indices
        if self.dim != 1 or self.X.dim() != 3 or (torch.is_tensor(idx) and idx.numel() != 1):
            raise NotImplementedError("IndexSelect.attnlrp: only dim=1 with a single index")
        out = torch.zeros(self.X.shape, dtype=G.dtype, device=G.device)
        out.index_copy_(1, idx.reshape(1) if torch.is_tensor(idx) else torch.tensor([int(idx)], device=G.device),
                        G.reshape(G.shape[0], 1, -1))
        return out
# ... 93 lines not shown
```

transformer-explainability_amd/vit.py:

```python
from __future__ import annotations

import torch
import torch.nn as nn

from . import methods, ops, producers
from . import rules as R_ours

__all__ = ["VisionTransformer", "vit_base_patch16_224", "vit_large_patch16_224", "deit_base_patch16_224",
           "compute_rollout_attention", "make_vit_module"]


def compute_rollout_attention(all_layer_matrices, start_layer=0):
    return ops.rollout(torch.stack(list(all_layer_matrices), 0), start_layer=start_layer, normalise=False)


def tail_full(model, cam, **kwargs):
    cam, _ = model.add.relprop(cam, **kwargs)
    cam = model.patch_embed.relprop(cam[:, 1:], **kwargs)
    return cam.sum(dim=1)


def tail_rollout(model, start_layer=0):
    mats = [blk.attn.get_attn_cam().clamp(min=0).mean(dim=1) for blk in model.blocks]
    return compute_rollout_attention(mats, start_layer=start_layer)[:, 0, 1:]


def tail_attribution(model, start_layer=0, pruned=False):
    first = model.blocks[-1].attn.get_attn_cam()
    Bn, _, N, _ = first.shape
    stack = torch.empty((len(model.blocks), Bn, N, N), dtype=first.dtype, device=first.device)
    for i, blk in enumerate(model.blocks):
        if i >= start_layer or not pruned:
            ops.gradcam_headmean(blk.attn.get_attn_gradients(), blk.attn.get_attn_cam(), out=stack[i])
    return ops.rollout(stack, start_layer=start_layer, normalise=False, row0_only=True)[:, 1:]


def tail_layer(model, method, is_ablation=False):
    blk = model.blocks[-1] if method == "last_layer" else model.blocks[1]
    c = blk.attn.get_attn_cam()
    if is_ablation:
        c = blk.attn.get_attn_gradients() * c
    return c.clamp(min=0).mean(dim=1)[:, 0, 1:]


def tail_last_layer_attn(model):
    attn = model.blocks[-1].attn.get_attn()
    if ops._is_bf16(attn):
        return ops.attn_headmean(attn.detach(), clamp=True, row0=True)[:, 1:]
    return attn.clamp(min=0).mean(dim=1)[:, 0, 1:]


def relprop_tail(model, method, cam=None, is_ablation=False, start_layer=0, pruned=False, **kwargs):
    if method == "full":
        return tail_full(model, cam, **kwargs)
    if method == "rollout":
        return tail_rollout(model, start_layer)
    if method in ("transformer_attribution", "grad"):
        return tail_attribution(model, start_layer, pruned)
    if method in ("last_layer", "second_layer"):
        return tail_layer(model, method, is_ablation)
    if method == "last_layer_attn":
        return tail_last_layer_attn(model)
    return None


def _trunc_normal_(t, std=.02):
    with torch.no_grad():
        return nn.init.trunc_normal_(t, mean=0., std=std, a=-2., b=2.)


class _SplitQKV(torch.autograd.Function):

    @staticmethod
    def forward(ctx, qkv, num_heads):
        B, N, C3 = qkv.shape
        parts = qkv.view(B, N, 3, num_heads, C3 // (3 * num_heads)).permute(2, 0, 3, 1, 4)
        return parts[0].contiguous(), parts[1].contiguous(), parts[2].contiguous()

    @staticmethod
    def backward(ctx, dq, dk, dv):
        ref = next(g for g in (dq, dk, dv) if g is not None)
        B, H, N, D = ref.shape
        grad = torch.empty((B, N, 3, H, D), dtype=ref.dtype, device=ref.device)
        slots = grad.permute(2, 0, 3, 1, 4)
        for slot, g in zip(slots, (dq, dk, dv)):
            if g is None:
                slot.zero_()
            else:
                slot.copy_(g)
        return grad.view(B, N, 3 * H * D), None


def split_qkv(qkv, num_heads):
    return _SplitQKV.apply(qkv, num_heads)


class _FusedAttention(torch.autograd.Function):

    @staticmethod
    def forward(ctx, qkv, num_heads, scale, module, feeds=None):
        if feeds is not None:
            out, attn, zqk, xs, xa = ops.attention_forward(qkv, num_heads, scale, planes=True, planes_abs=not ops.X6_SIGNED_PLANES)
            ops.post_x_planes(feeds, out, xs, xa)
        else:
            out, attn, zqk = ops.attention_forward(qkv, num_heads, scale)
        ctx.save_for_backward(qkv, attn, out)
        ctx.num_heads, ctx.scale, ctx.module = num_heads, scale, module
        ctx.mark_non_differentiable(attn, zqk)
        ctx.set_materialize_grads(False)
        return out, attn, zqk

    @staticmethod
    def backward(ctx, d_out, _d_attn_unused, _d_zqk_unused):
        qkv, attn, out = ctx.saved_tensors
        if d_out is None:
            return None, None, None, None, None
        stop = bool(getattr(ctx.module, "_fused_stop_backward", False))
        d_attn, d_qkv = ops.attention_backward(d_out, qkv, attn, ctx.num_heads, ctx.scale, need_qk=not stop, out=out)
        ctx.module.save_attn_gradients(d_attn)
        return (None if stop else d_qkv), None, None, None, None


PRETRAINED_URLS = {
    "vit_base_patch16_224": "https://github.com/rwightman/pytorch-image-models/releases/download/v0.1-vitjx/"
                            "jx_vit_base_p16_224-80ecf9dd.pth",
    "vit_large_patch16_224": "https://github.com/rwightman/pytorch-image-models/releases/download/v0.1-vitjx/"
                             "jx_vit_large_p16_224-4ee7a4dc.pth",
    "deit_base_patch16_224": "https://dl.fbaipublicfiles.com/deit/deit_base_patch16_224-b5f2ef4d.pth",
}


def load_pretrained_weights(model, url, patch_size=16, key=None):
    import os
    name = os.path.basename(url)
    try:
        state = torch.hub.load_state_dict_from_url(url, map_location="cpu", progress=False)
    except Exception as exc:
        where = os.path.join(torch.hub.get_dir(), "checkpoints", name)
        raise RuntimeError(f"pretrained=True: {name} is not in the torch hub cache and could not be downloaded "
                           f"({type(exc).__name__}: {exc}); place the checkpoint at {where}") from exc
    if key is not None:
        state = state[key]
    state = dict(state)
    w = state.get("patch_embed.proj.weight")
    if w is not None and w.dim() == 2:
        state["patch_embed.proj.weight"] = w.reshape(w.shape[0], 3, patch_size, patch_size)
    strict = True
    if "head.weight" in state and state["head.weight"].shape[0] != model.head.weight.shape[0]:
        del state["head.weight"], state["head.bias"]
        strict = False
    model.load_state_dict(state, strict=strict)
    return model


def make_vit_module(L):

    class Mlp(nn.Module):
        def __init__(self, in_features, hidden_features=None, out_features=None, drop=0.):
            super().__init__()
            out_features = out_features or in_features
            hidden_features = hidden_features or in_features
            self.fc1 = L.Linear(in_features, hidden_features)
            self.act = L.GELU()
            self.fc2 = L.Linear(hidden_features, out_features)
            self.drop = L.Dropout(drop)
            if hasattr(self.act, "feeds"):
                self.act.feeds(self.fc2)

        def forward(self, x):
            return self.drop(self.fc2(self.drop(self.act(self.fc1(x)))))

        def relprop(self, cam, **kwargs):
            cam = self.fc2.relprop(cam, **kwargs)
            return self.fc1.relprop(cam, **kwargs)

        def attnlrp(self, G, eps):
            G = self.act.attnlrp(self.fc2.attnlrp(G, eps), eps)
            return self.fc1.attnlrp(G, eps)

    class Attention(nn.Module):
        def __init__(self, dim, num_heads=8, qkv_bias=False, attn_drop=0., proj_drop=0.):
            super().__init__()
            self.num_heads = num_heads
            self.scale = (dim // num_heads) ** -0.5
            self.matmul1 = L.einsum('bhid,bhjd->bhij')
            self.matmul2 = L.einsum('bhij,bhjd->bhid')
            self.qkv = L.Linear(dim, dim * 3, bias=qkv_bias)
            self.attn_drop = L.Dropout(attn_drop)
            self.proj = L.Linear(dim, dim)
            self.proj_drop = L.Dropout(proj_drop)
            self.softmax = L.Softmax(dim=-1)
            self.mul = L.Mul()
            self.attn_cam = self.attn = self.v = self.v_cam = self.attn_gradients = None
            self.head_mask = None
            self.save_head_relevance = False
            self.head_relevance = None

        def get_attn(self): return self.attn
        def save_attn(self, attn): self.attn = attn
        def get_attention_map(self): return self.attn
        def save_attention_map(self, attn): self.attn = attn
        def save_attn_cam(self, cam): self.attn_cam = cam
        def get_attn_cam(self): return self.attn_cam
        def get_v(self): return self.v
        def save_v(self, v): self.v = v
        def save_v_cam(self, cam): self.v_cam = cam
        def get_v_cam(self): return self.v_cam
        def save_attn_gradients(self, g): self.attn_gradients = g
        def get_attn_gradients(self): return self.attn_gradients

        def forward(self, x, head_mask=None):
            B, N, C = x.shape
            H = self.num_heads
            self._fused_anchor = None
            self.head_mask = head_mask
            if head_mask is None and ops.USE_FUSED_PRODUCERS and x.is_cuda and not self.training and (
                    (x.dtype == torch.float32 and ops.attention_forward_supported(N, C // H))
                    or (x.dtype == torch.bfloat16 and ops.attention_forward_bf16_supported(N, C // H))):
                return self._forward_fused(x)
            q, k, v = split_qkv(self.qkv(x), H)
            self.save_v(v)
            attn = self.attn_drop(self.softmax(self.matmul1([q, k]) * self.scale))
            self.save_attn(attn)
            if attn.requires_grad:
                attn.register_hook(self.save_attn_gradients)
            if head_mask is not None:
                attn = self.mul([attn, head_mask])
            out = self.matmul2([attn, v]).permute(0, 2, 1, 3).reshape(B, N, C)
            return self.proj_drop(self.proj(out))

        def _forward_fused(self, x):
            B, N, C = x.shape
            H, D = self.num_heads, C // self.num_heads
            qkv = self.qkv(x)
            feeds = None
            if (isinstance(self.proj, L.Linear) and ops.attention_forward_planes_supported(qkv, H)
                    and producers.takes_producer_planes(self.proj, B * N, C)):
                feeds = R_ours.x6_cache(self.proj)
            out, attn, zqk = _FusedAttention.apply(qkv, H, self.scale, self, feeds)
            self._fused_anchor = qkv if qkv.requires_grad else None
            q, k, v = qkv.detach().view(B, N, 3, H, D).permute(2, 0, 3, 1, 4)
            self.save_v(v)
            self.save_attn(attn)
            zav = out.detach().view(B, N, H, D).permute(0, 2, 1, 3)
            for mod, X, Y in ((self.matmul1, [q, k], zqk), (self.matmul2, [attn, v], zav)):
                mod.X, mod.Y = X, Y
                mod._y_version, mod._w_version = Y._version, (None, None)
            return self.proj_drop(self.proj(out))

        def relprop(self, cam, **kwargs):
            return self.relprop_after_proj(self.proj.relprop(cam, **kwargs), **kwargs)

        def relprop_after_proj(self, cam, **kwargs):
            B, N, C = cam.shape
            H = self.num_heads
            D = C // H
            r_heads = cam.view(B, N, H, D).permute(0, 2, 1, 3)
            if self.save_head_relevance:
                self.head_relevance = ops.head_relevance(r_heads)
            attn, v = self.matmul2.X
            q, k = self.matmul1.X
            cam_qkv = torch.empty((B, N, 3 * C), dtype=cam.dtype, device=cam.device)
            slots = cam_qkv.view(B, N, 3, H, D).permute(2, 0, 3, 1, 4)
            var = self.matmul2.variant
            cam1, cam_v = ops.matmul_relprop_av(r_heads, attn, v, out_scale=0.5, cam_v_out=slots[2], variant=var,
                                                z=R_ours._cached_y(self.matmul2))
            self.save_v_cam(cam_v)
            if self.head_mask is not None:
                cam1, _ = self.mul.relprop(cam1, **kwargs)
            self.save_attn_cam(cam1)
            if getattr(self, "_stop_after_attn_cam", False):
                raise L.StopRelprop()
            ops.matmul_relprop_qk(cam1, q, k, out_scale=0.5, cam_q_out=slots[0], cam_k_out=slots[1], variant=var,
                                  z=R_ours._cached_y(self.matmul1))
            return self.qkv.relprop(cam_qkv, **kwargs)

        def attnlrp(self, G, eps):
            if self.head_mask is not None:
                raise ops._lib.TeError("Attention.attnlrp: head_mask is not implemented for AttnLRP")
            G_o = self.proj.attnlrp(G, eps)
            B, N, C = G_o.shape
            qkv = self.qkv.Y.detach()
            d_qkv = torch.empty_like(qkv)
            third = lambda t, i: t[..., i * C:(i + 1) * C]
            R_ours.attention_attnlrp(G_o, third(qkv, 0), third(qkv, 1), third(qkv, 2), self.get_attn().detach(),
                                     self.num_heads, self.scale, third(d_qkv, 0), third(d_qkv, 1), third(d_qkv, 2))
            return self.qkv.attnlrp(ops.alrp_scale3(d_qkv), eps)

    class Block(nn.Module):
        def __init__(self, dim, num_heads, mlp_ratio=4., qkv_bias=False, drop=0., attn_drop=0., norm_eps=1e-6):
            super().__init__()
            self.norm1 = L.LayerNorm(dim, eps=norm_eps)
            self.attn = Attention(dim, num_heads=num_heads, qkv_bias=qkv_bias, attn_drop=attn_drop, proj_drop=drop)
            self.norm2 = L.LayerNorm(dim, eps=norm_eps)
            self.mlp = Mlp(in_features=dim, hidden_features=int(dim * mlp_ratio), drop=drop)
            self.add1 = L.Add()
            self.add2 = L.Add()
            self.clone1 = L.Clone()
            self.clone2 = L.Clone()

        def forward(self, x, head_mask=None):
            x1, n = self._clone_norm(self.clone1, self.norm1, x)
            x = self.add1([x1, self.attn(n) if head_mask is None else self.attn(n, head_mask)])
            x1, n = self._clone_norm(self.clone2, self.norm2, x)
            return self.add2([x1, self.mlp(n)])

        @staticmethod
        def _clone_norm(clone, norm, x):
            if producers.norm_usable(x, norm):
                x1, n = producers.residual_layer_norm(x, norm)
                clone.X, clone.num = x.detach(), 2
                norm.X, norm.Y = clone.X, n
                return x1, n
            x1, x2 = clone(x, 2)
            return x1, norm(x2)

        def relprop(self, cam, **kwargs):
            cam1, cam2 = self.add2.relprop(cam, deferred=True, **kwargs)
            cam2 = self.mlp.relprop(cam2, **kwargs)
            cam = self.clone2.relprop((cam1, cam2), **kwargs)
# ... 189 lines not shown
```

Before: 1025.

## Fuse GELU forward and backward into the fc1 x6 GEMM epilogue

Adds GEMM epilogue modes that apply GELU to fc1's output and write both the pre-activation, the activation and its split bf16 planes in the forward pass. In the backward pass the same epilogue computes the GELU gradient and emits split planes for the next GEMM. This removes the separate GELU forward and backward plane kernels and their extra passes over the 3072-wide hidden activations. The cost is a more complex mailbox protocol between modules, with cache keys that could miss and silently fall back to the unfused path.

```diff
diff --git a/include/te_relprop.h b/include/te_relprop.h
--- a/include/te_relprop.h
+++ b/include/te_relprop.h
@@ -151,6 +151,10 @@
 int te_gemm_x6_f32(const float* X, const void* x_planes, const void* w_planes, const float* bias, float* out,
                    int64_t T, int64_t K, int64_t M, int flags, unsigned* status, void* ws, size_t ws_bytes,
                    te_stream_t stream);
+int te_gemm_x6_act_f32(const float* X, const void* x_planes, const void* w_planes, const float* bias, float* out,
+                       float* act_out, void* act_planes, size_t act_planes_bytes, const float* act_grad_h,
+                       int64_t T, int64_t K, int64_t M, int flags, unsigned* status, void* ws, size_t ws_bytes,
+                       te_stream_t stream);
 int te_linear_x6_split_dual_f32(const float* A, int64_t rows, int64_t K, void* planes, void* planes_abs,
                                 size_t planes_bytes, te_stream_t stream);
 int te_gelu_backward_x6_planes_f32(const float* dy, const float* x, int64_t rows, int64_t K, void* planes,
diff --git a/transformer-explainability_amd/bert.py b/transformer-explainability_amd/bert.py
--- a/transformer-explainability_amd/bert.py
+++ b/transformer-explainability_amd/bert.py
@@ -289,6 +289,8 @@
             act = self.intermediate.intermediate_act_fn
             if hasattr(act, "feeds"):
                 act.feeds(self.output.dense)
+            if hasattr(act, "follows"):
+                act.follows(self.intermediate.dense)
 
         def forward(self, hidden_states, attention_mask=None, head_mask=None, **unused):
             att = self.attention(hidden_states, attention_mask, head_mask)[0]
diff --git a/transformer-explainability_amd/csrc/te_api.hip b/transformer-explainability_amd/csrc/te_api.hip
--- a/transformer-explainability_amd/csrc/te_api.hip
+++ b/transformer-explainability_amd/csrc/te_api.hip
@@ -2,7 +2,7 @@
 
 #include <string.h>
 
-extern "C" int te_version(void) { return 800;  }
+extern "C" int te_version(void) { return 801;  }
 
 #ifndef TE_BUILD_ID
 #define TE_BUILD_ID "unstamped"
diff --git a/transformer-explainability_amd/csrc/te_linear_x6.hip b/transformer-explainability_amd/csrc/te_linear_x6.hip
--- a/transformer-explainability_amd/csrc/te_linear_x6.hip
+++ b/transformer-explainability_amd/csrc/te_linear_x6.hip
@@ -12,7 +12,7 @@
 constexpr int kErrWord = 1023;
 
 
-enum { MODE_Z = 0, MODE_C = 1, MODE_G = 2, MODE_ZI = 3, MODE_Z1 = 4, MODE_CI = 5, MODE_X = 6, MODE_ZS = 7 };
+enum { MODE_Z = 0, MODE_C = 1, MODE_G = 2, MODE_ZI = 3, MODE_Z1 = 4, MODE_CI = 5, MODE_X = 6, MODE_ZS = 7, MODE_GA = 8, MODE_GD = 9 };
 
 __device__ __forceinline__ float bf16_f32(unsigned b) { return __uint_as_float(b << 16); }
 
@@ -189,7 +189,9 @@
   int64_t a_group_stride;
   int64_t b_rb_stride;
   int nks;
-  unsigned char pad0_[20];
+  unsigned char pad0_[4];
+  float* act_out;
+  unsigned char pad0b_[8];
   int ntm, ntn;
   int rows_w;
   int t_fast;
@@ -229,6 +231,29 @@
 __device__ __forceinline__ void glds16(const unsigned char* src, unsigned char* lds_wave_base) {
   __builtin_amdgcn_global_load_lds((const __attribute__((address_space(1))) void*)src,
                                    (__attribute__((address_space(3))) void*)lds_wave_base, 16, 0, 0);
+}
+
+struct X6BlockPlanes { unsigned w[4][3][2]; };
+__device__ __forceinline__ void exchange_store_planes(X6BlockPlanes b, bool store, unsigned char* S, int cb, int nksS, int j0, int tc,
+                                                      int h) {
+  auto& w = b.w;
+#pragma unroll
+  for (int g = 0; g < 2; ++g)
+#pragma unroll
+    for (int q = 0; q < 3; ++q)
+#pragma unroll
+      for (int d = 0; d < 2; ++d) swap_halves(w[g][q][d], w[g + 2][q][d]);
+  if (store) {
+    unsigned char* Srow = S + (int64_t)cb * nksS * kRB + tc * 16;
+    unsigned char* sp = Srow + (int64_t)((j0 >> 4) + h) * kRB;
+#pragma unroll
+    for (int q = 0; q < 3; ++q)
+#pragma unroll
+      for (int c = 0; c < 2; ++c) {
+        u32x4 v = {w[c][q][0], w[c][q][1], w[c + 2][q][0], w[c + 2][q][1]};
+        *reinterpret_cast<u32x4*>(sp + q * kFrag + c * 512) = v;
+      }
+  }
 }
 
 constexpr int kStages = 2;
@@ -597,7 +622,8 @@
           X6_PASS4(r4[0], r4[1], r4[2], r4[3]);
           if constexpr (MODE != MODE_Z1) X6_PASS4(y4[0], y4[1], y4[2], y4[3]);
           X6_PASS4(b4[0], b4[1], b4[2], b4[3]);
-          unsigned w[4][3][2];
+          X6BlockPlanes bp;
+          auto& w = bp.w;
           unsigned long long any_cancel = 0;
           auto z_of = [&](int g, int c0, f32x2& z2, f32x2& a2) __attribute__((always_inline)) {
             a2 = f32x2{acc[mi][ni][4 * g + c0], acc[mi][ni][4 * g + c0 + 1]};
@@ -651,22 +677,9 @@
                 bad |= (cancels(z2[1], a2[1], b4[g][c0 + 1]) ? 1u : 0u) << (4 * g + c0 + 1);
               }
           }
-#pragma unroll
-          for (int g = 0; g < 2; ++g)
-#pragma unroll
-            for (int q = 0; q < 3; ++q)
-#pragma unroll
-              for (int d = 0; d < 2; ++d) swap_halves(w[g][q][d], w[g + 2][q][d]);
+          exchange_store_planes(bp, blk[ni], p.S, cb, nksS, j0, tc, h);
           if (blk[ni]) {
             unsigned char* Srow = p.S + (int64_t)cb * nksS * kRB + tc * 16;
-            unsigned char* sp = Srow + (int64_t)((j0 >> 4) + h) * kRB;
-#pragma unroll
-            for (int q = 0; q < 3; ++q)
-#pragma unroll
-              for (int c = 0; c < 2; ++c) {
-                u32x4 v = {w[c][q][0], w[c][q][1], w[c + 2][q][0], w[c + 2][q][1]};
-                *reinterpret_cast<u32x4*>(sp + q * kFrag + c * 512) = v;
-              }
             if (!live[ni]) bad = 0;
             if (__builtin_amdgcn_ballot_w64(bad != 0) != 0) {
               asm volatile("s_waitcnt vmcnt(0)" ::: "memory");
@@ -716,7 +729,8 @@
         } else {
           load_block(bi, 0);
         }
-        unsigned w[4][3][2];
+        X6BlockPlanes bp;
+        auto& w = bp.w;
         unsigned bad = 0;
 #pragma unroll
         for (int g = 0; g < 4; ++g) {
@@ -753,22 +767,9 @@
             w[g][q][1] = hi[q];
           }
         }
-#pragma unroll
-        for (int g = 0; g < 2; ++g)
-#pragma unroll
-          for (int q = 0; q < 3; ++q)
-#pragma unroll
-            for (int d = 0; d < 2; ++d) swap_halves(w[g][q][d], w[g + 2][q][d]);
+        exchange_store_planes(bp, blk[ni], p.S, cb, nksS, j0, tc, h);
         if (blk[ni]) {
           unsigned char* Srow = p.S + (int64_t)cb * nksS * kRB + tc * 16;
-          unsigned char* sp = Srow + (int64_t)((j0 >> 4) + h) * kRB;
-#pragma unroll
-          for (int q = 0; q < 3; ++q)
-#pragma unroll
-            for (int c = 0; c < 2; ++c) {
-              u32x4 v = {w[c][q][0], w[c][q][1], w[c + 2][q][0], w[c + 2][q][1]};
-              *reinterpret_cast<u32x4*>(sp + q * kFrag + c * 512) = v;
-            }
           if (!live[ni]) bad = 0;
           if (__builtin_amdgcn_ballot_w64(bad != 0) != 0) {
             asm volatile("s_waitcnt vmcnt(0)" ::: "memory");
@@ -815,6 +816,78 @@
             if (t < p.T) *reinterpret_cast<f32x4*>(orow + mi * 32 + 8 * g) = o;
           }
       }
+    } else if constexpr (MODE == MODE_GA || MODE == MODE_GD) {
+      constexpr bool FWD = MODE == MODE_GA;
+      float* const bias_lds = reinterpret_cast<float*>(smem + LDS_MAIN) + wave * 128;
+      if constexpr (FWD) {
+        if (lane < MI * 8) {
+          f32x4 bv = {0.0f, 0.0f, 0.0f, 0.0f};
+          if (p.bias) bv = *reinterpret_cast<const f32x4*>(p.bias + (tm * (NWM * MI) + wm * MI) * 32 + lane * 4);
+          *reinterpret_cast<f32x4*>(bias_lds + lane * 4) = bv;
+        }
+      }
+      const int nksS = p.out_f >> 4;
+      constexpr int NBUF = (!FWD && MI == 4) ? 2 : 1;
+      f32x4 h4[NBUF][4];
+      auto load_block = [&](int bi, int buf) __attribute__((always_inline)) {
+        const int ni = bi / MI, mi = bi % MI;
+        const int64_t t = ((int64_t)tn * (GEO::TT / 32) + wn * 2 + ni) * 32 + tc;
+        const float* hrow = p.Y + (t < p.T ? t : p.T - 1) * p.out_f + (tm * (NWM * MI) + wm * MI + mi) * 32 + 4 * h;
+#pragma unroll
+        for (int g = 0; g < 4; ++g) h4[buf][g] = *reinterpret_cast<const f32x4*>(hrow + 8 * g);
+      };
+      if constexpr (!FWD && NBUF == 2) load_block(0, 0);
+#pragma unroll
+      for (int bi = 0; bi < 2 * MI; ++bi) {
+        const int ni = bi / MI, mi = bi % MI, buf = bi % NBUF;
+        const int cb = tn * (GEO::TT / 32) + wn * 2 + ni;
+        const int64_t t = (int64_t)cb * 32 + tc;
+        const bool live = t < p.T;
+        const int j0 = (tm * (NWM * MI) + wm * MI + mi) * 32;
+        if constexpr (!FWD) {
+          if constexpr (NBUF == 2) {
+            if (bi + 1 < 2 * MI) load_block(bi + 1, buf ^ 1);
+          } else {
+            load_block(bi, 0);
+          }
+        }
+        X6BlockPlanes bp;
+        auto& w = bp.w;
+#pragma unroll
+        for (int g = 0; g < 4; ++g) {
+          float sv4[4];
+          if constexpr (FWD) {
+            const f32x4 b4 = *reinterpret_cast<const f32x4*>(bias_lds + mi * 32 + 8 * g + 4 * h);
+            f32x4 o, a;
+#pragma unroll
+            for (int c = 0; c < 4; ++c) {
+              o[c] = acc[mi][ni][4 * g + c] + b4[c];
+              a[c] = te_gelu(o[c]);
+              sv4[c] = live ? a[c] : 0.0f;
+            }
+            if (live) {
+              const int64_t at = t * p.out_f + j0 + 8 * g + 4 * h;
+              *reinterpret_cast<f32x4*>(p.out + at) = o;
+              *reinterpret_cast<f32x4*>(p.act_out + at) = a;
+            }
+          } else {
+#pragma unroll
+            for (int c = 0; c < 4; ++c) {
+              const float d = te_gelu_grad(acc[mi][ni][4 * g + c], h4[buf][g][c]);
+              sv4[c] = live ? d : 0.0f;
+            }
+          }
+          unsigned lo[3], hi[3];
+          split3_pk(sv4[0], sv4[1], lo);
+          split3_pk(sv4[2], sv4[3], hi);
+#pragma unroll
+          for (int q = 0; q < 3; ++q) {
+            w[g][q][0] = lo[q];
+            w[g][q][1] = hi[q];
+          }
+        }
+        exchange_store_planes(bp, cb < p.ncb, p.S, cb, nksS, j0, tc, h);
+      }
     } else if constexpr (MODE == MODE_X) {
 #pragma unroll
       for (int ni = 0; ni < 2; ++ni) {
@@ -888,7 +961,7 @@
 }
 
 static_assert(sizeof(X6Params) == 248, "X6Params is the kernel-argument block of x6_kernel");
-static_assert(offsetof(X6Params, ntm) == 56 && offsetof(X6Params, ncb) == 80 && offsetof(X6Params, T) == 88 &&
+static_assert(offsetof(X6Params, act_out) == 40 && offsetof(X6Params, ntm) == 56 && offsetof(X6Params, ncb) == 80 && offsetof(X6Params, T) == 88 &&
               offsetof(X6Params, partial) == 104 && offsetof(X6Params, R) == 152 && offsetof(X6Params, out) == 224,
               "a field of X6Params moved in the kernel arguments");
 
@@ -1148,15 +1221,19 @@
   return te_gemm_x6_supported(T, K, M) ? gemm_workspace(T, K, M).total : 0;
 }
 
-extern "C" int te_gemm_x6_f32(const float* X, const void* x_planes, const void* w_planes, const float* bias, float* out,
-                              int64_t T, int64_t K, int64_t M, int flags, unsigned* status, void* ws, size_t ws_bytes,
-                              te_stream_t stream_) {
-  if ((!X && !x_planes) || !w_planes || !out) return TE_ERR_INVALID_ARG;
+extern "C" int te_gemm_x6_act_f32(const float* X, const void* x_planes, const void* w_planes, const float* bias, float* out,
+                                  float* act_out, void* act_planes, size_t act_planes_bytes, const float* act_grad_h,
+                                  int64_t T, int64_t K, int64_t M, int flags, unsigned* status, void* ws, size_t ws_bytes,
+                                  te_stream_t stream_) {
+  const bool act_fwd = act_out != nullptr, act_bwd = act_grad_h != nullptr;
+  if ((!X && !x_planes) || !w_planes || (!out && !act_bwd)) return TE_ERR_INVALID_ARG;
+  if ((act_fwd && act_bwd) || (act_fwd || act_bwd) != (act_planes != nullptr) || (act_bwd && bias)) return TE_ERR_INVALID_ARG;
   if ((flags & ~kProductFlags) != 0) return TE_ERR_INVALID_ARG;
   if (!te_gemm_x6_supported(T, K, M)) return TE_ERR_UNSUPPORTED;
   if (!ws || ws_bytes < te_gemm_x6_workspace_bytes(T, K, M) || !te_aligned16(ws)) return TE_ERR_WORKSPACE;
-  if ((X && !te_aligned16(X)) || !te_aligned16(out) || !te_aligned16(w_planes) || (bias && !te_aligned16(bias)) ||
-      (x_planes && !te_aligned16(x_planes)))
+  if (act_planes && (act_planes_bytes < planes_bytes(T, M) || !te_aligned16(act_planes))) return TE_ERR_WORKSPACE;
+  if ((X && !te_aligned16(X)) || (out && !te_aligned16(out)) || !te_aligned16(w_planes) || (bias && !te_aligned16(bias)) ||
+      (x_planes && !te_aligned16(x_planes)) || !te_aligned16(act_out) || !te_aligned16(act_grad_h))
     return TE_ERR_UNSUPPORTED;
   hipStream_t stream = (hipStream_t)stream_;
   const X6Workspace l = gemm_workspace(T, K, M);
@@ -1167,11 +1244,25 @@
     x_planes = l.x(ws, 0);
   }
   const int wm = choose_geo((M % 256 == 0) ? 2 : 1, T, M, flags & kTileMask, 192, true);
-  const int rc = launch_pass<MODE_G>(call_params(T, l.acc(ws), bias, out, status, flags), wm, (const unsigned char*)w_planes,
-                                     (const unsigned char*)x_planes, nullptr, K, M, l.flag_region(ws, 0), stream);
+  X6Params p = call_params(T, l.acc(ws), bias, out, status, flags);
+  p.act_out = act_out;
+  p.Y = act_grad_h;
+  const unsigned char* wp = (const unsigned char*)w_planes;
+  const unsigned char* xp = (const unsigned char*)x_planes;
+  unsigned char* ap = (unsigned char*)act_planes;
+  const int rc = act_fwd   ? launch_pass<MODE_GA>(p, wm, wp, xp, ap, K, M, l.flag_region(ws, 0), stream)
+                 : act_bwd ? launch_pass<MODE_GD>(p, wm, wp, xp, ap, K, M, l.flag_region(ws, 0), stream)
+                           : launch_pass<MODE_G>(p, wm, wp, xp, nullptr, K, M, l.flag_region(ws, 0), stream);
   if (rc != TE_OK) return rc;
   TE_RETURN_IF_LAUNCH_FAILED();
   return TE_OK;
+}
+
+extern "C" int te_gemm_x6_f32(const float* X, const void* x_planes, const void* w_planes, const float* bias, float* out,
+                              int64_t T, int64_t K, int64_t M, int flags, unsigned* status, void* ws, size_t ws_bytes,
+                              te_stream_t stream_) {
+  return te_gemm_x6_act_f32(X, x_planes, w_planes, bias, out, nullptr, nullptr, 0, nullptr, T, K, M, flags, status, ws, ws_bytes,
+                            stream_);
 }
 
 extern "C" size_t te_linear_relprop_x6_workspace_bytes(int64_t T, int64_t in_f, int64_t out_f) {
diff --git a/transformer-explainability_amd/ops.py b/transformer-explainability_amd/ops.py
--- a/transformer-explainability_amd/ops.py
+++ b/transformer-explainability_amd/ops.py
@@ -336,6 +336,7 @@
 
 def drop_x_planes(cache: dict, with_abs: bool = False):
     cache.pop("x_planes_from_producer", None)
+    cache.pop("act_grad_from_producer", None)
     if with_abs:
         cache.pop("x_abs_planes", None)
 
@@ -371,10 +372,18 @@
         return False
 
 
-def post_dy_planes(cache: dict, planes: Tensor, like: Tensor) -> Tensor:
+def post_dy_planes(cache: dict, planes: Tensor, like: Tensor, placeholder: Optional[Tensor] = None) -> Tensor:
+    if placeholder is not None and tuple(placeholder.shape) == tuple(like.shape) and not any(placeholder.stride()):
+        cache["dy_planes_from_consumer"] = (placeholder, tuple(like.shape), planes)
+        return placeholder
     base = torch.full((1,), float("nan"), dtype=like.dtype, device=like.device)
     cache["dy_planes_from_consumer"] = (base, tuple(like.shape), planes)
     return base.expand(like.shape)
+
+
+def dy_planes_posted(cache: Optional[dict], dy: Tensor) -> bool:
+    hit = None if cache is None else cache.get("dy_planes_from_consumer")
+    return bool(hit is not None and dy.data_ptr() == hit[0].data_ptr() and tuple(dy.shape) == hit[1] and not any(dy.stride()))
 
 
 def take_dy_planes(cache: dict, dy: Tensor) -> Optional[Tensor]:
@@ -384,19 +393,62 @@
     return None
 
 
+X6_ACT_EPILOGUE = True
+X6_ACT_EPILOGUE_DIRS = {"": "both", "1": "both", "0": "off"}.get(os.environ.get("TE_X6_ACT_EPILOGUE", "both"),
+                                                                 os.environ.get("TE_X6_ACT_EPILOGUE", "both"))
+if X6_ACT_EPILOGUE_DIRS not in ("both", "fwd", "bwd", "off"):
+    raise ValueError(f"TE_X6_ACT_EPILOGUE={X6_ACT_EPILOGUE_DIRS!r}: expected both / fwd / bwd / off (or 1 / 0)")
+
+
+def act_epilogue_on(direction: str) -> bool:
+    return bool(X6_ACT_EPILOGUE and X6_ACT_EPILOGUE_DIRS in ("both", direction))
+
+
+def post_act(cache: dict, h: Tensor, a: Tensor, planes: Tensor):
+    K = h.shape[-1]
+    cache["act_from_product"] = (_x_abs_key(h, h.numel() // K, K), a, planes, h)
+
+
+def take_act(cache: dict, h: Tensor):
+    hit = cache.pop("act_from_product", None)
+    K = h.shape[-1]
+    if hit is not None and hit[0] == _x_abs_key(h, h.numel() // K, K) and tuple(hit[3].shape) == tuple(h.shape):
+        return hit[1], hit[2]
+    return None
+
+
+def post_act_grad(cache: dict, a: Tensor, h: Tensor, act_cache: dict):
+    K = a.shape[-1]
+    cache["act_grad_from_producer"] = (_x_abs_key(a, a.numel() // K, K), h, act_cache, a)
+
+
+def take_act_grad(cache: dict, a: Tensor):
+    hit = cache.pop("act_grad_from_producer", None)
+    K = a.shape[-1]
+    if hit is not None and hit[0] == _x_abs_key(a, a.numel() // K, K) and hit[3].data_ptr() == a.data_ptr():
+        return hit[1], hit[2]
+    return None
+
+
 def rule_takes_abs_planes(T: int, in_f: int, out_f: int) -> bool:
     return bool(USE_LINEAR_X6 and X6_KEEP_ABS and linear_relprop_x6_supported(T, in_f, out_f))
 
 
 def gemm_x6(X: Tensor, w_planes: Tensor, bias: Optional[Tensor], M: int, timer_name: str = "gemm_x6",
-            keep_abs: Optional[dict] = None, x_planes: Optional[Tensor] = None) -> Tensor:
+            keep_abs: Optional[dict] = None, x_planes: Optional[Tensor] = None, act_forward: bool = False,
+            act_grad_h: Optional[Tensor] = None):
     K = X.shape[-1]
     lead = X.shape[:-1]
     T = X.numel() // K
+    if act_grad_h is not None and (act_forward or bias is not None or act_grad_h.numel() != T * M):
+        raise _lib.TeError("gemm_x6: act_grad_h takes [T, M] values, no bias, and excludes act_forward")
     Xc = None if x_planes is not None else _c(X).reshape(-1, K)
     like = X if Xc is None else Xc
-    out = torch.empty((T, M), dtype=torch.float32, device=X.device)
+    out = None if act_grad_h is not None else torch.empty((T, M), dtype=torch.float32, device=X.device)
     bc = None if bias is None else _c(bias.detach())
+    hc = None if act_grad_h is None else _c(act_grad_h).reshape(-1, M)
+    act_out = torch.empty((T, M), dtype=torch.float32, device=X.device) if act_forward else None
+    out_bytes = (14.0 if act_forward else 10.0 if hc is not None else 4.0) * T * M
     with _on_device(like) as lib:
         ws = _ws(lib.te_gemm_x6_workspace_bytes(T, K, M), like)
         x_bytes = (6.0 if x_planes is not None else 10.0) * T * K
@@ -412,7 +464,7 @@
         for_rule = xs is None and keep_abs is not None and rule_takes_abs_planes(T, K, M)
         if for_rule and not X6_SIGNED_PLANES:
             x_bytes += 6.0 * T * K
-        with _timed(timer_name, 12.0 * T * K * M, x_bytes + 6.0 * K * M + 4.0 * T * M):
+        with _timed(timer_name, 12.0 * T * K * M, x_bytes + 6.0 * K * M + out_bytes):
             if for_rule:
                 nb = lib.te_linear_x6_planes_bytes(T, K)
                 if X6_SIGNED_PLANES:
@@ -425,9 +477,20 @@
                     _lib.check(lib.te_linear_x6_split_dual_f32(_ptr(Xc), T, K, _ptr(xs), _ptr(xa), nb, _stream(Xc)),
                                "te_linear_x6_split_dual_f32")
                     post_x_abs_planes(keep_abs, X, T, K, xa)
-            _lib.check(lib.te_gemm_x6_f32(_ptr(Xc) if Xc is not None else None, _ptr(xs), _ptr(w_planes), _ptr(bc), _ptr(out),
-                                          T, K, M, (X6_TILE | X6_FLAGS) & ~0x3c00, _ptr(x6_status(X.device)), _ptr(ws),
-                                          ws.numel(), _stream(like)), "te_gemm_x6_f32")
+            flags, status = (X6_TILE | X6_FLAGS) & ~0x3c00, x6_status(X.device)
+            if act_forward or hc is not None:
+                nb = lib.te_linear_x6_planes_bytes(T, M)
+                act_planes = _ws(nb, like)
+                _lib.check(lib.te_gemm_x6_act_f32(_ptr(Xc) if Xc is not None else None, _ptr(xs), _ptr(w_planes), _ptr(bc),
+                                                  _ptr(out), _ptr(act_out), _ptr(act_planes), nb, _ptr(hc), T, K, M, flags,
+                                                  _ptr(status), _ptr(ws), ws.numel(), _stream(like)), "te_gemm_x6_act_f32")
+            else:
+                _lib.check(lib.te_gemm_x6_f32(_ptr(Xc) if Xc is not None else None, _ptr(xs), _ptr(w_planes), _ptr(bc), _ptr(out),
+                                              T, K, M, flags, _ptr(status), _ptr(ws), ws.numel(), _stream(like)), "te_gemm_x6_f32")
+    if hc is not None:
+        return act_planes
+    if act_forward:
+        return out.reshape(*lead, M), act_out.reshape(*lead, M), act_planes
     return out.reshape(*lead, M)
 
 
@@ -898,7 +961,11 @@
     return bool(X6_FUSE_GELU and x.dim() >= 2 and x.shape[-1] >= 16 and x.shape[-1] % 16 == 0)
 
 
-def gelu_forward_planes(x: Tensor, planes_abs: bool = True):
+def gelu_forward_planes(x: Tensor, planes_abs: bool = True, posted: Optional[dict] = None):
+    if posted is not None:
+        hit = take_act(posted, x)
+        if hit is not None and not planes_abs:
+            return hit[0], hit[1], None
     x = _c(x)
     K = x.shape[-1]
     T = x.numel() // K
@@ -911,7 +978,11 @@
     return y, xs, xa
 
 
-def gelu_backward_planes(dy: Tensor, x: Tensor) -> Tensor:
+def gelu_backward_planes(dy: Tensor, x: Tensor, posted: Optional[dict] = None) -> Tensor:
+    if posted is not None:
+        planes = take_dy_planes(posted, dy)
+        if planes is not None:
+            return planes
     dy, x = _c(dy), _c(x)
     K = x.shape[-1]
     T = x.numel() // K
diff --git a/transformer-explainability_amd/producers.py b/transformer-explainability_amd/producers.py
--- a/transformer-explainability_amd/producers.py
+++ b/transformer-explainability_amd/producers.py
@@ -51,12 +51,14 @@
 class _Gelu(torch.autograd.Function):
 
     @staticmethod
-    def forward(ctx, x, feeds, source):
+    def forward(ctx, x, feeds, source, mail):
         ctx.save_for_backward(x)
-        ctx.source = source
+        ctx.source, ctx.mail = source, mail
         if feeds is not None:
-            y, xs, xa = ops.gelu_forward_planes(x, not ops.X6_SIGNED_PLANES)
+            y, xs, xa = ops.gelu_forward_planes(x, not ops.X6_SIGNED_PLANES, mail)
             ops.post_x_planes(feeds, y, xs, xa)
+            if source is not None and mail is not None and ops.act_epilogue_on("bwd"):
+                ops.post_act_grad(feeds, y, x, mail)
             return y
         return ops.gelu_forward(x)
 
@@ -64,15 +66,23 @@
     def backward(ctx, dy):
         (x,) = ctx.saved_tensors
         if ctx.source is not None:
-            return ops.post_dy_planes(ctx.source, ops.gelu_backward_planes(dy, x), x), None, None
-        return ops.gelu_backward(dy, x), None, None
+            handed = ops.dy_planes_posted(ctx.mail, dy)
+            planes = ops.gelu_backward_planes(dy, x, ctx.mail)
+            return ops.post_dy_planes(ctx.source, planes, x, dy if handed else None), None, None, None
+        return ops.gelu_backward(dy, x), None, None, None
 
 
 class _Linear(torch.autograd.Function):
 
     @staticmethod
-    def forward(ctx, x, weight, bias, cache, fwd_x6, bwd_x6):
+    def forward(ctx, x, weight, bias, cache, fwd_x6, bwd_x6, act_mail):
         ctx.weight, ctx.cache, ctx.bwd_x6 = weight, cache, bwd_x6
+        ctx.act_grad = ops.take_act_grad(cache, x) if bwd_x6 else None
+        if fwd_x6 and act_mail is not None:
+            h, a, planes = ops.gemm_x6(x, ops.x6_matrix_planes(weight, False, cache), bias, weight.shape[0], "linear_forward_x6",
+                                       keep_abs=cache, act_forward=True)
+            ops.post_act(act_mail, h, a, planes)
+            return h
         if fwd_x6:
             return ops.gemm_x6(x, ops.x6_matrix_planes(weight, False, cache), bias, weight.shape[0], "linear_forward_x6",
                                keep_abs=cache)
@@ -81,12 +91,17 @@
     @staticmethod
     def backward(ctx, dy):
         w = ctx.weight
-        if ctx.bwd_x6:
+        if ctx.bwd_x6 and ctx.act_grad is not None:
+            h, act_mail = ctx.act_grad
+            planes = ops.gemm_x6(dy, ops.x6_matrix_planes(w, True, ctx.cache), None, w.shape[1], "linear_backward_x6",
+                                 x_planes=ops.take_dy_planes(ctx.cache, dy), act_grad_h=h)
+            dx = ops.post_dy_planes(act_mail, planes, h)
+        elif ctx.bwd_x6:
             dx = ops.gemm_x6(dy, ops.x6_matrix_planes(w, True, ctx.cache), None, w.shape[1], "linear_backward_x6",
                              x_planes=ops.take_dy_planes(ctx.cache, dy))
         else:
             dx = torch.matmul(dy, w)
-        return dx, None, None, None, None, None
+        return dx, None, None, None, None, None, None
 
 
 def linear_plan(x: torch.Tensor, lin):
@@ -108,8 +123,8 @@
     return None if t is None else t.detach()
 
 
-def linear(x, lin, cache, plan):
-    out = _Linear.apply(x, _d(lin.weight), _d(lin.bias), cache, plan[0], plan[1])
+def linear(x, lin, cache, plan, act_mail=None):
+    out = _Linear.apply(x, _d(lin.weight), _d(lin.bias), cache, plan[0], plan[1], act_mail if plan[0] else None)
     if plan[1]:
         out._te_bwd_x6_cache = cache
     return out
@@ -123,7 +138,13 @@
     return _ResidualLayerNorm.apply(x, _d(norm.weight), _d(norm.bias), norm.eps)
 
 
-def gelu(x, consumer=None, consumer_cache=None):
+def act_epilogue_wanted(act, consumer, T: int, K: int) -> bool:
+    return bool(ops.act_epilogue_on("fwd") and ops.X6_FUSE_GELU and ops.X6_SIGNED_PLANES and K >= 16 and K % 16 == 0
+                and getattr(act, "approximate", "none") == "none" and not act.training
+                and consumer is not None and takes_producer_planes(consumer, T, K))
+
+
+def gelu(x, consumer=None, consumer_cache=None, mail=None):
     feeds = source = None
     if ops.gelu_planes_supported(x):
         K = x.shape[-1]
@@ -133,4 +154,6 @@
             source = getattr(x, "_te_bwd_x6_cache", None)
     if feeds is None and consumer_cache is not None:
         ops.drop_x_planes(consumer_cache)
-    return _Gelu.apply(x, feeds, source)
+    if feeds is None and mail is not None:
+        mail.pop("act_from_product", None)
+    return _Gelu.apply(x, feeds, source, mail)
diff --git a/transformer-explainability_amd/rules.py b/transformer-explainability_amd/rules.py
--- a/transformer-explainability_amd/rules.py
+++ b/transformer-explainability_amd/rules.py
@@ -89,11 +89,16 @@
         self.__dict__["_te_feeds"] = (linear,)
         return self
 
+    def follows(self, linear):
+        linear.__dict__["_te_act"] = (self,)
+        return self
+
     def forward(self, x):
         from . import producers
         if getattr(self, "approximate", "none") == "none" and not self.training and producers.gelu_usable(x):
             nxt = self.__dict__.get("_te_feeds", (None,))[0]
-            return producers.gelu(x, nxt, x6_cache(nxt) if isinstance(nxt, Linear) else None)
+            return producers.gelu(x, nxt, x6_cache(nxt) if isinstance(nxt, Linear) else None, x6_cache(self))
+        x6_cache(self).pop("act_from_product", None)
         return super().forward(x)
 
     def attnlrp(self, G, eps):
@@ -160,7 +165,11 @@
         if not plan[0]:
             ops.drop_x_planes(x6_cache(self), with_abs=True)
         if plan[0] or plan[1]:
-            return producers.linear(x, self, x6_cache(self), plan)
+            act = self.__dict__.get("_te_act", (None,))[0]
+            nxt = None if act is None else act.__dict__.get("_te_feeds", (None,))[0]
+            fused = (plan[0] and isinstance(act, GELU) and isinstance(nxt, Linear)
+                     and producers.act_epilogue_wanted(act, nxt, x.numel() // self.in_features, self.out_features))
+            return producers.linear(x, self, x6_cache(self), plan, x6_cache(act) if fused else None)
         return super().forward(x)
 
     def relprop(self, R, alpha):
diff --git a/transformer-explainability_amd/vit.py b/transformer-explainability_amd/vit.py
--- a/transformer-explainability_amd/vit.py
+++ b/transformer-explainability_amd/vit.py
@@ -166,6 +166,8 @@
             self.drop = L.Dropout(drop)
             if hasattr(self.act, "feeds"):
                 self.act.feeds(self.fc2)
+            if hasattr(self.act, "follows"):
+                self.act.follows(self.fc1)
 
         def forward(self, x):
             return self.drop(self.fc2(self.drop(self.act(self.fc1(x)))))
```

Result: no change. 1029 (median of 6 runs) (+0.3%).
